# ThomasZiegler/RS-aware-differential-SfM

Measured on AMD Instinct MI355X. Metric: Mpixels/sec RS depth+pose solve, 1280x720 pair, higher is better.
Workload: dtype f64

## Files before the change

### include/rsdsfm.h

```cpp
#ifndef RSDSFM_H
#define RSDSFM_H

#include <stddef.h>
#include <stdint.h>

#ifdef __cplusplus
extern "C" {
#endif

#define RSDSFM_OK 0
#define RSDSFM_ERR_INVALID (-1)
#define RSDSFM_ERR_HIP (-2)
#define RSDSFM_ERR_NO_DEVICE (-3)
#define RSDSFM_ERR_NUMERIC (-4)
#define RSDSFM_ERR_PENDING (-5)
#define RSDSFM_ERR_PEER (-6)

#define RSDSFM_DEPTH_CLOSED_FORM 0
#define RSDSFM_DEPTH_CERES_LM 1

#define RSDSFM_K_COMPAT 0
#define RSDSFM_K_FIXED 1

#define RSDSFM_FLOW_COMPAT_RANK 0
#define RSDSFM_FLOW_GATHERED 1

#define RSDSFM_BACKPROJECT_RS 0
#define RSDSFM_BACKPROJECT_GS 1

#define RSDSFM_Q5_COMPAT 0
#define RSDSFM_Q5_FIXED 1

#define RSDSFM_TERM_GRADIENT 0
#define RSDSFM_TERM_PARAMETER 1
#define RSDSFM_TERM_FUNCTION 2
#define RSDSFM_TERM_MAX_ITER 3
#define RSDSFM_TERM_FAILURE 4
#define RSDSFM_TERM_MIN_RADIUS 5

typedef struct rsdsfm_ctx rsdsfm_ctx;

typedef struct rsdsfm_lm_summary {
    int32_t num_iterations;
    int32_t num_successful_steps;
    int32_t num_unsuccessful_steps;
    int32_t termination;
    double initial_cost;
    double final_cost;
    double final_radius;
} rsdsfm_lm_summary;

typedef struct rsdsfm_ransac_out {
    int64_t num_inliers;
    int32_t best_trial;
    int32_t _pad;
    double w[3], v[3], k;
    double inlier_error;
    int64_t* inlier_idx;
    double* inliers;
    double* alpha;
    double* alpha_k;
    uint8_t* mask;
    double* inv_depth;
    int64_t* trial_count;
    double* trial_err;
    double* trial_vel;
    int32_t* trial_steps;
} rsdsfm_ransac_out;

int rsdsfm_create(rsdsfm_ctx** ctx, int device, void* stream_or_null);
void rsdsfm_destroy(rsdsfm_ctx* ctx);
const char* rsdsfm_last_error(const rsdsfm_ctx* ctx);
const char* rsdsfm_version(void);
int rsdsfm_fused_arithmetic(void);
int rsdsfm_synchronize(rsdsfm_ctx* ctx);
int rsdsfm_set_depth_variant(rsdsfm_ctx* ctx, int variant);
int rsdsfm_set_ransac_speculation(rsdsfm_ctx* ctx, int k0);
int rsdsfm_set_ransac_math(rsdsfm_ctx* ctx, int mode);
int rsdsfm_ransac_restarts(rsdsfm_ctx* ctx, int64_t* count);
int rsdsfm_set_lm_arithmetic(rsdsfm_ctx* ctx, int mode);
int rsdsfm_lma_restarts(rsdsfm_ctx* ctx, int64_t* count, int32_t* last_guards_or_null);
int rsdsfm_refine_restarts(rsdsfm_ctx* ctx, int64_t* runs, int64_t* restarts, int64_t* resolves_or_null, int32_t* last_guard_or_null);
int rsdsfm_set_refine_arithmetic(rsdsfm_ctx* ctx, int mode);
int rsdsfm_lma_count_only(rsdsfm_ctx* ctx, int64_t* runs, int64_t* lazy_runs_or_null);
int rsdsfm_depth_restarts(rsdsfm_ctx* ctx, int64_t* count);
int rsdsfm_set_refine_stage(rsdsfm_ctx* ctx, int mode);
int rsdsfm_set_profiling(rsdsfm_ctx* ctx, int on);
int rsdsfm_profile_last_ms(rsdsfm_ctx* ctx, const char* what, double* ms);
const char* rsdsfm_kernel_name(const char* entry_point);

int rsdsfm_get_alpha(rsdsfm_ctx* ctx, const double* flow_px2n, int64_t n, double h, double gamma, double* alpha_n);
int rsdsfm_get_alpha_k(rsdsfm_ctx* ctx, const double* q_px2n, const double* flow_px2n, int64_t n, double h,
                       double gamma, double* alpha_k_n);
int rsdsfm_calculate_velocities(rsdsfm_ctx* ctx, const double* q_18xT, const double* u_18xT,
                                const double* alpha_9xT, const double* alpha_k_9xT, int32_t count,
                                int use_alpha_k, int k_sign_mode, double* w_3xT, double* v_3xT, double* k_T);
int rsdsfm_estimate_inverse_depths(rsdsfm_ctx* ctx, const double* q2n, const double* u2n, int64_t n,
                                   const double v[3], const double w[3], double k, const double* alpha_n,
                                   const double* alpha_k_n, int depth_mode, double* inv_depth_n,
                                   rsdsfm_lm_summary* summary_or_null);
int rsdsfm_ransac(rsdsfm_ctx* ctx, const double* q2n, const double* u2n, const double* alpha_n,
                  const double* alpha_k_n, int64_t n, int use_alpha_k, int32_t iterations, double tolerance,
                  const int32_t* samples_9xT_or_null, uint64_t seed, int depth_mode, int k_sign_mode,
                  rsdsfm_ransac_out* out);
int rsdsfm_refine(rsdsfm_ctx* ctx, const double* flow2n, int64_t n_flow, int64_t m, const double* inliers_3m,
                  const double* alpha_m, const double* alpha_k_m, const int64_t* inlier_idx_or_null,
                  const double v_in[3], const double w_in[3], double k_in, int const_acceleration,
                  int flow_index_mode, double* inliers_out_3m, double v_out[3], double w_out[3], double* k_out,
                  rsdsfm_lm_summary* summary_or_null);
int rsdsfm_last_ransac_tag(rsdsfm_ctx* ctx, uint64_t* tag, int64_t* cache_hits_or_null);
int rsdsfm_refine_from_ransac(rsdsfm_ctx* ctx, uint64_t ransac_tag, const double* flow2n, int64_t n_flow, int64_t m, const double* inliers_3m,
                              const double* alpha_m, const double* alpha_k_m, const int64_t* inlier_idx_or_null, const double v_in[3],
                              const double w_in[3], double k_in, int const_acceleration, int flow_index_mode, double* inliers_out_3m,
                              double v_out[3], double w_out[3], double* k_out, rsdsfm_lm_summary* summary_or_null);
#define RSDSFM_REFINE_TRACE_COLS 8
#define RSDSFM_TRACE_REJECTED 0.0
#define RSDSFM_TRACE_ACCEPTED 1.0
#define RSDSFM_TRACE_INVALID 2.0
#define RSDSFM_TRACE_PARAMETER_TOL 3.0
#define RSDSFM_TRACE_FUNCTION_TOL 4.0
#define RSDSFM_TRACE_ACCEPTED_GRADIENT_TOL 5.0
int rsdsfm_set_refine_trace(rsdsfm_ctx* ctx, int32_t rows);
int rsdsfm_get_refine_trace(rsdsfm_ctx* ctx, double* trace_rows_x_8, int32_t rows);
int rsdsfm_flatten(rsdsfm_ctx* ctx, const double* flow_img_rows_cols_2, int32_t rows, int32_t cols, double fx,
                   double fy, double cx, double cy, double gamma, double flow_threshold, double* q2n,
                   double* u2n, double* alpha_n, double* alpha_k_n, int64_t* n_out);
int rsdsfm_depth_map(rsdsfm_ctx* ctx, double* inliers_3m_inout, int64_t m, double v_inout[3], double fx,
                     double fy, double cx, double cy, int32_t rows, int32_t cols,
                     double* depth_map_colmajor, int32_t* xs_or_null, int32_t* ys_or_null, int* flipped);
int rsdsfm_pose_table(rsdsfm_ctx* ctx, const double v[3], const double w[3], double k, double gamma,
                      int32_t rows, double* R_rows9, double* t_rows3);

int rsdsfm_estimate_inverse_depths_dev(rsdsfm_ctx* ctx, const double* d_q2n, const double* d_u2n, int64_t n,
                                       const double v[3], const double w[3], double k, const double* d_alpha_n,
                                       const double* d_alpha_k_n, int depth_mode, double* d_inv_depth_n);
int rsdsfm_flatten_dev(rsdsfm_ctx* ctx, const double* d_flow_img, int32_t rows, int32_t cols, double fx, double fy,
                       double cx, double cy, double gamma, double flow_threshold, double* d_q2n, double* d_u2n,
                       double* d_alpha_n, double* d_alpha_k_n, int64_t* n_out);
int rsdsfm_depth_map_dev(rsdsfm_ctx* ctx, double* d_inliers_3m_inout, int64_t m, double v_inout[3], double fx, double fy,
                         double cx, double cy, int32_t rows, int32_t cols, double* d_depth_map_colmajor,
                         int32_t* d_xs_or_null, int32_t* d_ys_or_null, int* flipped);
int rsdsfm_pose_table_dev(rsdsfm_ctx* ctx, const double v[3], const double w[3], double k, double gamma, int32_t rows,
                          double* d_R_rows9, double* d_t_rows3);
typedef struct rsdsfm_frame_params {
    int32_t ransac_trials;
    int32_t use_acceleration_mode;
    int32_t use_refinement;
    int32_t depth_mode;
    int32_t k_sign_mode;
    int32_t flow_index_mode;
    int32_t use_global_shutter_mode;
    int32_t struct_bytes;
    double ransac_tol;
    double flow_threshold;
    uint64_t seed;
} rsdsfm_frame_params;

void rsdsfm_frame_params_init(rsdsfm_frame_params* params);

typedef struct rsdsfm_frame_result {
    int64_t n_points, num_inliers;
    int32_t best_trial, flipped;
    double ransac_w[3], ransac_v[3], ransac_k;
    double w[3], v[3], k;
// ... 182 lines not shown
```

### rs-aware-differential-sfm_amd/__init__.py

```python
import ctypes as C
import os
import sys

import numpy as np

from . import dist, pipeline, synth

_HERE = os.path.dirname(os.path.abspath(__file__))
LIB_PATH = os.environ.get("RSDSFM_LIB") or os.path.join(_HERE, "librsdsfm_hip.so")
LIB_PATH_FUSED = os.path.join(_HERE, "librsdsfm_hip_fused.so")
HEADER_PATH = os.path.join(os.path.dirname(_HERE), "include", "rsdsfm.h")

OK = 0
ERR_PENDING = -5
DEPTH_CLOSED_FORM, DEPTH_CERES_LM = 0, 1
K_COMPAT, K_FIXED = 0, 1
FLOW_COMPAT_RANK, FLOW_GATHERED = 0, 1
REFINE_TRACE_COLS = 8
TRACE_REJECTED, TRACE_ACCEPTED, TRACE_INVALID, TRACE_PARAMETER_TOL, TRACE_FUNCTION_TOL, TRACE_ACCEPTED_GRADIENT_TOL = 0.0, 1.0, 2.0, 3.0, 4.0, 5.0
TERMINATION = {0: "gradient", 1: "parameter", 2: "function", 3: "max_iter", 4: "failure", 5: "min_radius"}

_libs = {}


# ... 134 lines not shown
    return np.ascontiguousarray(a, dtype=np.float64)


def _p(a):
    return None if a is None else a.ctypes.data_as(C.c_void_p)


def _v3(a):
    return (C.c_double * 3)(*[float(x) for x in a])


def _dp(ptr):
    return C.c_void_p(int(ptr))


class Solver:

    def __init__(self, device=0, stream=None, arith="reference"):
        self.lib = load_library(arith=arith)
        self.arith = arith
        self._ctx = C.c_void_p()
        rc = self.lib.rsdsfm_create(C.byref(self._ctx), int(device), C.c_void_p(stream) if stream else None)
        if rc != OK:
            self._ctx = None
            raise RsdsfmError("rsdsfm_create(device=%d) failed with %d (no usable gfx950 device? there is no CPU fallback)" % (device, rc))

    def close(self):
        if getattr(self, "_ctx", None):
            self.lib.rsdsfm_destroy(self._ctx)
            self._ctx = None

    def __del__(self):
        try:
            self.close()
        except Exception:
            pass

    def __enter__(self):
        return self

    def __exit__(self, *a):
        self.close()

    def _check(self, rc, what):
        if rc != OK:
            msg = self.lib.rsdsfm_last_error(self._ctx)
            raise RsdsfmError("%s failed (%d): %s" % (what, rc, msg.decode() if msg else ""))

    def set_depth_variant(self, variant):
        self._check(self.lib.rsdsfm_set_depth_variant(self._ctx, int(variant)), "rsdsfm_set_depth_variant")

    def set_profiling(self, on):
        self._check(self.lib.rsdsfm_set_profiling(self._ctx, int(bool(on))), "rsdsfm_set_profiling")

    def profile_last_ms(self, what="ransac_lm_round0"):
        ms = C.c_double()
        self._check(self.lib.rsdsfm_profile_last_ms(self._ctx, what.encode(), C.byref(ms)), "rsdsfm_profile_last_ms")
        return ms.value

    def set_refine_stage(self, mode):
        self._check(self.lib.rsdsfm_set_refine_stage(self._ctx, int(mode)), "rsdsfm_set_refine_stage")

    def set_ransac_speculation(self, k0):
        self._check(self.lib.rsdsfm_set_ransac_speculation(self._ctx, int(k0)), "rsdsfm_set_ransac_speculation")

    def set_ransac_math(self, mode):
        self._check(self.lib.rsdsfm_set_ransac_math(self._ctx, int(mode)), "rsdsfm_set_ransac_math")

    def set_lm_arithmetic(self, mode):
        self._check(self.lib.rsdsfm_set_lm_arithmetic(self._ctx, int(mode)), "rsdsfm_set_lm_arithmetic")

    def set_refine_arithmetic(self, mode):
        self._check(self.lib.rsdsfm_set_refine_arithmetic(self._ctx, int(mode)), "rsdsfm_set_refine_arithmetic")

    def refine_restarts(self):
        n, r, sv, g = C.c_int64(0), C.c_int64(0), C.c_int64(0), C.c_int32(0)
        self._check(self.lib.rsdsfm_refine_restarts(self._ctx, C.byref(n), C.byref(r), C.byref(sv), C.byref(g)), "rsdsfm_refine_restarts")
        return dict(runs=n.value, restarts=r.value, resolves=sv.value, last_guard=g.value)

    def lma_restarts(self):
        n, g = C.c_int64(0), C.c_int32(0)
        self._check(self.lib.rsdsfm_lma_restarts(self._ctx, C.byref(n), C.byref(g)), "rsdsfm_lma_restarts")
        return int(n.value), int(g.value)

    def lma_count_only(self):
        a, b = C.c_int64(0), C.c_int64(0)
        self._check(self.lib.rsdsfm_lma_count_only(self._ctx, C.byref(a), C.byref(b)), "rsdsfm_lma_count_only")
        return int(a.value), int(b.value)

    def ransac_restarts(self):
        n = C.c_int64()
        self._check(self.lib.rsdsfm_ransac_restarts(self._ctx, C.byref(n)), "rsdsfm_ransac_restarts")
        return n.value

    def depth_restarts(self):
        n = C.c_int64()
        self._check(self.lib.rsdsfm_depth_restarts(self._ctx, C.byref(n)), "rsdsfm_depth_restarts")
        return int(n.value)

    def synchronize(self):
        self._check(self.lib.rsdsfm_synchronize(self._ctx), "rsdsfm_synchronize")

    def get_alpha(self, flow_px, h, gamma):
        flow_px = _f64(flow_px)
        n = flow_px.shape[0]
        out = np.empty(n)
        self._check(self.lib.rsdsfm_get_alpha(self._ctx, _p(flow_px), C.c_int64(n), C.c_double(h), C.c_double(gamma), _p(out)), "rsdsfm_get_alpha")
        return out

    def get_alpha_k(self, q_px, flow_px, h, gamma):
        q_px, flow_px = _f64(q_px), _f64(flow_px)
        n = flow_px.shape[0]
        out = np.empty(n)
        self._check(self.lib.rsdsfm_get_alpha_k(self._ctx, _p(q_px), _p(flow_px), C.c_int64(n), C.c_double(h), C.c_double(gamma), _p(out)), "rsdsfm_get_alpha_k")
        return out

    def calculate_velocities(self, q, u, alpha, alpha_k, use_alpha_k=False, k_sign_mode=K_COMPAT):
        q, u, alpha, alpha_k = _f64(q), _f64(u), _f64(alpha), _f64(alpha_k)
        single = q.ndim == 2
        T = 1 if single else q.shape[0]
        w, v, k = np.empty((T, 3)), np.empty((T, 3)), np.empty(T)
        self._check(self.lib.rsdsfm_calculate_velocities(self._ctx, _p(q), _p(u), _p(alpha), _p(alpha_k), C.c_int32(T), int(use_alpha_k), int(k_sign_mode), _p(w), _p(v), _p(k)), "rsdsfm_calculate_velocities")
        return (w[0], v[0], float(k[0])) if single else (w, v, k)

    def ransac(self, q, u, alpha, alpha_k, use_alpha_k, iterations, tolerance, samples=None, seed=0, depth_mode=DEPTH_CERES_LM, k_sign_mode=K_COMPAT, outputs=None):
        q, u, alpha, alpha_k = _f64(q), _f64(u), _f64(alpha), _f64(alpha_k)
        n, T = q.shape[0], int(iterations)
        smp = None if samples is None else np.ascontiguousarray(samples, dtype=np.int32).reshape(-1)
        reuse = outputs is not None
        if reuse and outputs.get("_shape") == (n, T):
            bufs = outputs["_bufs"]
        else:
            bufs = dict(
                inlier_idx=np.zeros(n, dtype=np.int64), inliers=np.zeros((n, 3)), alpha=np.zeros(n), alpha_k=np.zeros(n),
                mask=np.zeros(n, dtype=np.uint8), inv_depth=np.zeros(n), trial_count=np.zeros(max(T, 1), dtype=np.int64),
                trial_err=np.zeros(max(T, 1)), trial_vel=np.zeros((max(T, 1), 7)), trial_steps=np.zeros(max(T, 1), dtype=np.int32),
            )
            if reuse:
                outputs["_shape"], outputs["_bufs"] = (n, T), bufs
        out = RansacOut()
        for name, arr in bufs.items():
            if not reuse or "only" not in outputs or name in outputs["only"]:
                setattr(out, name, arr.ctypes.data)
        self._check(self.lib.rsdsfm_ransac(self._ctx, _p(q), _p(u), _p(alpha), _p(alpha_k), C.c_int64(n), int(use_alpha_k), C.c_int32(T), C.c_double(tolerance), _p(smp), C.c_uint64(seed), int(depth_mode), int(k_sign_mode), C.byref(out)), "rsdsfm_ransac")
        m = int(out.num_inliers)
        tag, hits = C.c_uint64(0), C.c_int64(0)
        self._check(self.lib.rsdsfm_last_ransac_tag(self._ctx, C.byref(tag), C.byref(hits)), "rsdsfm_last_ransac_tag")
        return dict(
            tag=int(tag.value),
            num_inliers=m, best_trial=int(out.best_trial), w=np.array(out.w[:]), v=np.array(out.v[:]), k=float(out.k),
            inlier_error=float(out.inlier_error), inlier_idx=bufs["inlier_idx"][:m] if reuse else bufs["inlier_idx"][:m].copy(),
            inliers=bufs["inliers"][:m] if reuse else bufs["inliers"][:m].copy(), alpha=bufs["alpha"][:m] if reuse else bufs["alpha"][:m].copy(),
            alpha_k=bufs["alpha_k"][:m] if reuse else bufs["alpha_k"][:m].copy(), mask=bufs["mask"], inv_depth=bufs["inv_depth"],
            trial_count=bufs["trial_count"][:T], trial_err=bufs["trial_err"][:T], trial_vel=bufs["trial_vel"][:T],
            trial_steps=bufs["trial_steps"][:T],
        )

    def estimate_inverse_depths(self, q, u, v, w, k, alpha, alpha_k, mode=DEPTH_CERES_LM):
        q, u, alpha, alpha_k = _f64(q), _f64(u), _f64(alpha), _f64(alpha_k)
        n = q.shape[0]
        rho = np.empty(n)
        sm = LmSummary()
        self._check(self.lib.rsdsfm_estimate_inverse_depths(self._ctx, _p(q), _p(u), C.c_int64(n), _v3(v), _v3(w), C.c_double(k), _p(alpha), _p(alpha_k), int(mode), _p(rho), C.byref(sm)), "rsdsfm_estimate_inverse_depths")
        return rho, sm.as_dict()

    def estimate_inverse_depth(self, q, v, w, flow, k, alpha, alpha_k, mode=DEPTH_CERES_LM):
# ... 852 lines not shown
```

### rs-aware-differential-sfm_amd/csrc/capi.hip

```cpp
#include <string.h>

#include <algorithm>
#include <new>
#include <vector>

#include <chrono>
#include <thread>

#include "rsdsfm_internal.hpp"

namespace rsdsfm {

int fail(Ctx* c, int code, const char* msg) {
    if (c) c->err = msg;
    return code;
}

int ensure_stage(Ctx* c, size_t bytes) {
    c->stage_gen += 1;
    if (bytes <= c->stage_bytes) return RSDSFM_OK;
    RSDSFM_HIP_CHECK(c, hipStreamSynchronize(c->stream));
    if (c->d_stage) RSDSFM_HIP_CHECK(c, hipFree(c->d_stage));
    c->d_stage = nullptr;
    c->stage_bytes = 0;
// ... 241 lines not shown
    if (rows < 0 || rows > 4096) return fail(c, RSDSFM_ERR_INVALID, "refine trace: 0 <= rows <= 4096");
    if (rows != c->refine_trace_rows) {
        RSDSFM_HIP_CHECK(c, hipStreamSynchronize(c->stream));
        if (c->d_refine_trace) RSDSFM_HIP_CHECK(c, hipFree(c->d_refine_trace));
        c->d_refine_trace = nullptr;
        c->refine_trace_rows = 0;
        if (rows > 0) {
            RSDSFM_HIP_CHECK(c, hipMalloc((void**)&c->d_refine_trace, (size_t)rows * kRefineTraceCols * sizeof(double)));
            c->refine_trace_rows = rows;
        }
    }
    if (c->d_refine_trace)
        RSDSFM_HIP_CHECK(c, hipMemsetAsync(c->d_refine_trace, 0xFF, (size_t)rows * kRefineTraceCols * sizeof(double), c->stream));
    return RSDSFM_OK;
}

int rsdsfm_get_refine_trace(rsdsfm_ctx* ctx, double* out, int32_t rows) {
    CTX_OR_FAIL(ctx);
    if (!out || rows < 1) return fail(c, RSDSFM_ERR_INVALID, "refine trace: null output or rows < 1");
    if (!c->d_refine_trace) return fail(c, RSDSFM_ERR_INVALID, "no refine trace: call rsdsfm_set_refine_trace(ctx, rows) before the refinement");
    if (rows > c->refine_trace_rows) return fail(c, RSDSFM_ERR_INVALID, "refine trace: more rows requested than rsdsfm_set_refine_trace reserved");
    RSDSFM_HIP_CHECK(c, hipMemcpyAsync(out, c->d_refine_trace, (size_t)rows * kRefineTraceCols * sizeof(double), hipMemcpyDeviceToHost, c->stream));
    RSDSFM_HIP_CHECK(c, hipStreamSynchronize(c->stream));
    return RSDSFM_OK;
}

int rsdsfm_set_ransac_speculation(rsdsfm_ctx* ctx, int k0) {
    CTX_OR_FAIL(ctx);
    if (k0 != 0 && k0 != 2 && k0 != KMAX) return fail(c, RSDSFM_ERR_INVALID, "ransac speculation depth must be 0 (automatic, default), 2 or 3");
    c->ransac_k0 = k0;
    return RSDSFM_OK;
}

int rsdsfm_set_ransac_math(rsdsfm_ctx* ctx, int mode) {
    CTX_OR_FAIL(ctx);
    if (mode < 0 || mode > 1) return fail(c, RSDSFM_ERR_INVALID, "ransac math: 0 = in-range function cores with restart (default), 1 = standard functions");
    c->ransac_math_mode = mode;
    return RSDSFM_OK;
}

int rsdsfm_ransac_restarts(rsdsfm_ctx* ctx, int64_t* count) {
    CTX_OR_FAIL(ctx);
    if (!count) return fail(c, RSDSFM_ERR_INVALID, "ransac restarts: null output");
    int64_t total = c->ransac_restarts;
    for (rsdsfm_ctx* lane : c->lanes) total += lane->c.ransac_restarts;
    *count = total;
    return RSDSFM_OK;
}

int rsdsfm_set_lm_arithmetic(rsdsfm_ctx* ctx, int mode) {
    CTX_OR_FAIL(ctx);
    if (mode < 0 || mode > 2)
        return fail(c, RSDSFM_ERR_INVALID, "LM arithmetic: 0 = analytic trajectory with guards (default), 1 = iterate by iterate, 2 = 0 with the frame solve's count-only pass forced");
    c->lm_arithmetic = mode == 1 ? 1 : 0;
    c->lma_count_only_force = mode == 2;
    c->lma_hold = c->lma_unique_run = 0;
    dist_reset_hold(c);
    for (rsdsfm_ctx* lane : c->lanes)
        lane->c.lm_arithmetic = c->lm_arithmetic, lane->c.lma_count_only_force = c->lma_count_only_force, lane->c.lma_hold = lane->c.lma_unique_run = 0;
    return RSDSFM_OK;
}

int rsdsfm_lma_count_only(rsdsfm_ctx* ctx, int64_t* runs, int64_t* lazy_runs) {
    CTX_OR_FAIL(ctx);
    if (!runs) return fail(c, RSDSFM_ERR_INVALID, "lma count only: null output");
    int64_t a = c->lma_count_only_runs, b = c->lma_lazy_runs;
    for (rsdsfm_ctx* lane : c->lanes) a += lane->c.lma_count_only_runs, b += lane->c.lma_lazy_runs;
    *runs = a;
    if (lazy_runs) *lazy_runs = b;
    return RSDSFM_OK;
}

int rsdsfm_lma_restarts(rsdsfm_ctx* ctx, int64_t* count, int32_t* last_guards) {
    CTX_OR_FAIL(ctx);
    if (!count) return fail(c, RSDSFM_ERR_INVALID, "lma restarts: null output");
    int64_t total = c->lma_restarts;
    int guards = c->lma_last_guard;
    for (rsdsfm_ctx* lane : c->lanes) total += lane->c.lma_restarts, guards |= lane->c.lma_last_guard;
    *count = total;
    if (last_guards) *last_guards = guards;
    return RSDSFM_OK;
}

int rsdsfm_set_refine_arithmetic(rsdsfm_ctx* ctx, int mode) {
    CTX_OR_FAIL(ctx);
    if (mode != 0 && mode != 1) return fail(c, RSDSFM_ERR_INVALID, "refine arithmetic: 0 = radius-factorised (default), 1 = iterate by iterate");
    c->refine_arithmetic = mode;
    for (rsdsfm_ctx* lane : c->lanes) lane->c.refine_arithmetic = mode;
    return RSDSFM_OK;
}

int rsdsfm_refine_restarts(rsdsfm_ctx* ctx, int64_t* runs, int64_t* restarts, int64_t* resolves_or_null, int32_t* last_guard_or_null) {
    CTX_OR_FAIL(ctx);
    if (!runs || !restarts) return fail(c, RSDSFM_ERR_INVALID, "refine restarts: null output");
    int64_t n = c->refine_rf_runs, r = c->refine_rf_restarts, s = c->refine_rf_resolves;
    int guard = c->refine_rf_last_guard;
    for (rsdsfm_ctx* lane : c->lanes) {
        n += lane->c.refine_rf_runs, r += lane->c.refine_rf_restarts, s += lane->c.refine_rf_resolves;
        if (lane->c.refine_rf_last_guard) guard = lane->c.refine_rf_last_guard;
    }
    *runs = n, *restarts = r;
    if (resolves_or_null) *resolves_or_null = s;
    if (last_guard_or_null) *last_guard_or_null = guard;
    return RSDSFM_OK;
}

int rsdsfm_depth_restarts(rsdsfm_ctx* ctx, int64_t* count) {
    CTX_OR_FAIL(ctx);
    if (!count) return fail(c, RSDSFM_ERR_INVALID, "depth restarts: null output");
    *count = c->depth_restarts;
    return RSDSFM_OK;
}

int rsdsfm_set_true_flow_search(rsdsfm_ctx* ctx, int mode) {
    CTX_OR_FAIL(ctx);
    if (mode < 0 || mode > 2) return fail(c, RSDSFM_ERR_INVALID, "true-flow search mode: 0 = automatic, 1 = exhaustive, 2 = interval-pruned");
    c->true_flow_exhaustive = mode;
    return RSDSFM_OK;
}

const char* rsdsfm_kernel_name(const char* entry_point) {
    if (!entry_point) return "";
    if (!strcmp(entry_point, "estimate_inverse_depths_lm")) return RSDSFM_FUSED ? "depth_lm_kernel<1, false>" : "depth_lm_kernel<1, true>";
    if (!strcmp(entry_point, "estimate_inverse_depths_closed_form")) return "depth_closed_form_kernel";
    return "";
}

int rsdsfm_estimate_inverse_depths_dev(rsdsfm_ctx* ctx, const double* d_q, const double* d_u, int64_t n,
                                       const double v[3], const double w[3], double k, const double* d_alpha,
                                       const double* d_alpha_k, int depth_mode, double* d_rho) {
    CTX_OR_FAIL(ctx);
    if (n < 0 || !v || !w) return fail(c, RSDSFM_ERR_INVALID, "bad arguments");
    if (n > 0 && (!d_q || !d_u || !d_alpha || !d_alpha_k || !d_rho)) return fail(c, RSDSFM_ERR_INVALID, "null device pointer");
    Pose pose;
    memcpy(pose.v, v, sizeof(pose.v));
    memcpy(pose.w, w, sizeof(pose.w));
    pose.k = k;
    if (depth_mode == RSDSFM_DEPTH_CLOSED_FORM) return depth_closed_form_launch(c, d_q, d_u, d_alpha, d_alpha_k, n, pose, d_rho);
    if (depth_mode != RSDSFM_DEPTH_CERES_LM) return fail(c, RSDSFM_ERR_INVALID, "unknown depth_mode");
    if (c->depth_variant == 2) {
        int rcf = depth_lm_fused_launch(c, d_q, d_u, d_alpha, d_alpha_k, n, pose, d_rho);
        if (rcf != RSDSFM_OK) return rcf;
        rcf = depth_lm_launch(c, d_q, d_u, d_alpha, d_alpha_k, n, pose, d_rho, 1);
        c->lm_issued_k = 2;
        c->lm_issued_d = 1;
        return rcf;
    }
    if (depth_lma_allowed(c, n)) {
        Ctx* cs1[1] = {c};
        const double *q1[1] = {d_q}, *u1[1] = {d_u}, *a1[1] = {d_alpha}, *ak1[1] = {d_alpha_k};
        double* r1[1] = {d_rho};
        int rc0 = depth_lma_batch_launch(cs1, 1, q1, u1, a1, ak1, &n, &pose, r1);
        c->lm_issued_k = 1;
        c->lm_issued_d = 1;
        return rc0;
    }
    if (c->depth_variant == 0) {
        int rc0 = depth_lm_launch(c, d_q, d_u, d_alpha, d_alpha_k, n, pose, d_rho, 0, true);
        if (rc0 != RSDSFM_OK) return rc0;
        rc0 = depth_lm_decide_apply_launch(c, d_q, d_u, d_alpha, d_alpha_k, n, pose, d_rho);
        c->lm_issued_k = 1;
        c->lm_issued_d = 1;
        return rc0;
    }
    int rc = depth_lm_launch(c, d_q, d_u, d_alpha, d_alpha_k, n, pose, d_rho, 0);
    if (rc != RSDSFM_OK) return rc;
// ... 254 lines not shown
```

### rs-aware-differential-sfm_amd/csrc/frame_host.hip

```cpp
#include <stdlib.h>
#include <string.h>

#include <atomic>

#include <algorithm>
#include <new>

#include "rsdsfm_internal.hpp"
#include "sequence_host.hpp"

namespace rsdsfm {

static std::atomic<int> g_frames_in_flight[64];
int frames_in_flight(const Ctx* c) { return g_frames_in_flight[c->device & 63].load(std::memory_order_relaxed); }

int alpha_ones_launch(Ctx* c, double* d_alpha, int64_t n);
int flatten_device(Ctx* c, const double* d_img, int32_t rows, int32_t cols, int32_t col0, double fx, double fy, double cx, double cy, double gamma,
                   double thr, double* d_q, double* d_u, double* d_alpha, double* d_alpha_k, int64_t* n_out);

struct FrameRun {
    rsdsfm_frame_job job;
    rsdsfm_frame_params prm;
    size_t N = 0;
    int64_t n = 0;
// ... 86 lines not shown
    F->d_in_a = fa.take<double>(N);
    F->d_in_ak = fa.take<double>(N);
    F->d_inl = fa.take<double>(3 * N);
    F->d_inl_ref = fa.take<double>(3 * N);
    F->d_idx = fa.take<int64_t>(N);
    F->d_mask = fa.take<uint8_t>(N);
    F->d_ys = fa.take<int32_t>(N);
    F->d_zpartials = fa.take<double>(1024);
    F->d_zheader = fa.take<double>(8);
    F->d_refine_ws = fa.take<char>(refine_workspace_bytes(c, (int64_t)N, true));
    int64_t* d_flat_counts = fa.take<int64_t>(ncells);
    int64_t* d_flat_offsets = fa.take<int64_t>(ncells + 2048);

    int rc = ensure_pinned(c, ransac_pinned_bytes(prm->ransac_trials));
    if (rc != RSDSFM_OK) return rc;
    int64_t n = (int64_t)N;
    F->side_flatten = false;
    if (c->frame_dense_hint) {
        *count_host(c) = -1;
        int side = prm->ransac_trials > 0 ? c->frame_side_flatten : 0;
        if (side == 3 && prm->ransac_trials > c->num_cus * 2) side = 0;
        F->dense_in_launch = false;
        if (side) {
            F->side_flatten = true;
            F->direct = Minimal9Direct();
            F->direct.img = J.d_flow_img, F->direct.rows = rows, F->direct.cols = cols, F->direct.alpha_ones = prm->use_global_shutter_mode ? 1 : 0;
            F->direct.fx = fx, F->direct.fy = fy, F->direct.cx = cx, F->direct.cy = cy, F->direct.gamma = gamma;
        }
        if (side == 3) {
            if (!c->d_flat_counters) {
                RSDSFM_HIP_CHECK(c, hipMalloc(reinterpret_cast<void**>(&c->d_flat_counters), 2 * sizeof(unsigned long long)));
                RSDSFM_HIP_CHECK(c, hipMemsetAsync(c->d_flat_counters, 0, 2 * sizeof(unsigned long long), c->stream));
            }
            F->dense = DenseFlatten();
            F->dense.thr = prm->flow_threshold;
            F->dense.d_q = F->d_q, F->dense.d_u = F->d_u, F->dense.d_alpha = F->d_a, F->dense.d_alpha_k = F->d_ak;
            F->dense.d_counters = c->d_flat_counters;
            F->dense.total_out = count_host(c);
            F->dense_in_launch = true;
        } else if (side == 2) {
            F->join = [c, F, d_flat_counts, d_flat_offsets]() -> int {
                const rsdsfm_frame_job& J2 = F->job;
                int rc2 = flatten_launch(c, J2.d_flow_img, J2.rows, J2.cols, 0, J2.fx, J2.fy, J2.cx, J2.cy, J2.gamma, F->prm.flow_threshold, F->d_q, F->d_u, F->d_a,
                                         F->d_ak, d_flat_counts, d_flat_offsets, count_host(c), nullptr);
                if (rc2 == RSDSFM_OK && F->prm.use_global_shutter_mode) rc2 = alpha_ones_launch(c, F->d_a, (int64_t)F->N);
                return rc2;
            };
        } else if (side == 1) {
            rc = ensure_side_stream(c);
            if (rc != RSDSFM_OK) return rc;
            RSDSFM_HIP_CHECK(c, hipEventRecord(c->ev_fork, c->stream));
            RSDSFM_HIP_CHECK(c, hipStreamWaitEvent(c->aux_stream, c->ev_fork, 0));
            {
                StreamSwap on_side(c, c->aux_stream);
                rc = flatten_launch(c, J.d_flow_img, rows, cols, 0, fx, fy, cx, cy, gamma, prm->flow_threshold, F->d_q, F->d_u, F->d_a, F->d_ak,
                                    d_flat_counts, d_flat_offsets, count_host(c), nullptr);
                if (rc == RSDSFM_OK && prm->use_global_shutter_mode) rc = alpha_ones_launch(c, F->d_a, n);
            }
            if (rc != RSDSFM_OK) return rc;
            RSDSFM_HIP_CHECK(c, hipEventRecord(c->ev_join, c->aux_stream));
            F->join = [c]() -> int {
                RSDSFM_HIP_CHECK(c, hipStreamWaitEvent(c->stream, c->ev_join, 0));
                return RSDSFM_OK;
            };
        } else {
            rc = flatten_enqueue(c, J.d_flow_img, rows, cols, fx, fy, cx, cy, gamma, prm->flow_threshold, F->d_q, F->d_u, F->d_a, F->d_ak, count_host(c));
            if (rc != RSDSFM_OK) return rc;
        }
    } else {
        rc = flatten_device(c, J.d_flow_img, rows, cols, 0, fx, fy, cx, cy, gamma, prm->flow_threshold, F->d_q, F->d_u, F->d_a, F->d_ak, &n);
        if (rc != RSDSFM_OK) return rc;
        *count_host(c) = n;
    }
    if (prm->use_global_shutter_mode && !F->side_flatten) {
        rc = alpha_ones_launch(c, F->d_a, n);
        if (rc != RSDSFM_OK) return rc;
    }
    F->n = n;
    memset(&F->ro, 0, sizeof(F->ro));
    F->ro.inlier_idx = F->d_idx;
    F->ro.inliers = F->d_inl;
    F->ro.alpha = F->d_in_a;
    F->ro.alpha_k = F->d_in_ak;
    F->ro.mask = F->d_mask;
    F->m_known = -1;
    F->tail = [c, F](const RefineBuffers& B) -> int {
        const rsdsfm_frame_job& J2 = F->job;
        const RefineState* st = B.state;
        const int64_t m_arg = F->m_known >= 0 ? F->m_known : F->n;
        const int64_t* m_dev = F->m_known >= 0 ? nullptr : &st->m;
        PoseTableOut pt;
        if (J2.d_R_rows9_or_null && J2.d_t_rows3_or_null)
            pt.R = J2.d_R_rows9_or_null, pt.t = J2.d_t_rows3_or_null, pt.rows = J2.rows, pt.gamma = J2.gamma, pt.wk_dev = st->p + 3;
        if (B.claim.on)
            return depth_map_decided_launch(c, F->d_inl_ref, m_arg, F->d_zpartials, refine_finish_grid(c, B), B, J2.d_depth_map_colmajor, F->d_zheader,
                                            header_host(c), st->p, m_dev, &pt);
        return depth_map_slab_launch(c, F->d_inl_ref, m_arg, F->d_zpartials, refine_finish_grid(c, B), m_arg, nullptr, J2.fx, J2.fy, J2.cx, J2.cy, J2.rows,
                                     0, J2.cols, J2.d_depth_map_colmajor, nullptr, F->d_ys, F->d_zheader, header_host(c), st->p, m_dev, &pt);
    };
    F->claim = FinishClaim();
    if (c->frame_tail == 0) {
        F->claim.on = true;
        F->claim.fx = J.fx, F->claim.fy = J.fy, F->claim.cx = J.cx, F->claim.cy = J.cy;
        F->claim.rows = rows, F->claim.cols = cols;
        F->claim.ys = F->d_ys;
    }
    F->spec_tail = [c, F](const RansacBest* d_best) -> int {
        return refine_begin(c, F->d_u, F->n, F->n, F->d_inl, F->d_in_a, F->d_in_ak, F->d_idx, nullptr, nullptr, 0.0, F->prm.use_acceleration_mode,
                            F->prm.flow_index_mode, F->d_inl_ref, &F->tail, d_best, F->d_refine_ws, &F->refine, state_host(c), F->d_zpartials, false,
                            &F->claim);
    };
    F->refinement_enqueued = false;
    F->ahead = prm->use_refinement && c->ransac_spec_miss < 2;
    F->open = true;
    g_frames_in_flight[c->device & 63].fetch_add(1, std::memory_order_relaxed);
    F->counted = true;
    F->rc_begin = ransac_begin(c, F->d_q, F->d_u, F->d_a, F->d_ak, n, prm->use_acceleration_mode, prm->ransac_trials, prm->ransac_tol, nullptr, J.seed,
                               prm->depth_mode, prm->k_sign_mode, &F->ro, prm->use_refinement ? &F->spec_tail : nullptr, &F->refinement_enqueued, &F->ransac,
                               F->side_flatten ? &F->direct : nullptr, F->side_flatten && !F->dense_in_launch ? &F->join : nullptr,
                               F->dense_in_launch ? &F->dense : nullptr, F->ahead, true,
                               F->claim.on && prm->use_refinement ? refine_flag_words(F->d_refine_ws) : nullptr);
    return RSDSFM_OK;
}

int frame_finish(Ctx* c, FrameRun* F, rsdsfm_frame_result* res) {
    if (!F->open) return fail(c, RSDSFM_ERR_INVALID, "no frame solve in flight");
    F->open = false;
    FrameInFlightEnd in_flight_end_{c, F};
    const rsdsfm_frame_job& J = F->job;
    const rsdsfm_frame_params* prm = &F->prm;
    memset(res, 0, sizeof(*res));
    int rc = F->rc_begin;
    if (rc == RSDSFM_OK) rc = ransac_finish(c, &F->ransac);
    if (rc != RSDSFM_OK) RSDSFM_HIP_CHECK(c, hipStreamSynchronize(c->stream));
    if (F->side_flatten && c->aux_stream) RSDSFM_HIP_CHECK(c, hipStreamSynchronize(c->aux_stream));
    int64_t n = F->n;
    if (*count_host(c) < 0) {
        c->frame_dense_hint = 1;
        return rc != RSDSFM_OK ? rc : fail(c, RSDSFM_ERR_NUMERIC, "frame solve: the point count did not arrive");
    }
    bool counted = true;
    if (*count_host(c) != n) {
        if (F->dense_in_launch) {
            int64_t n_real = 0;
            rc = flatten_device(c, J.d_flow_img, J.rows, J.cols, 0, J.fx, J.fy, J.cx, J.cy, J.gamma, prm->flow_threshold, F->d_q, F->d_u, F->d_a, F->d_ak, &n_real);
            if (rc == RSDSFM_OK && prm->use_global_shutter_mode) rc = alpha_ones_launch(c, F->d_a, n_real);
            if (rc != RSDSFM_OK) return rc;
            *count_host(c) = n_real;
        }
        n = *count_host(c);
        F->n = n;
        F->refinement_enqueued = false;
        counted = false;
        rc = ransac_begin(c, F->d_q, F->d_u, F->d_a, F->d_ak, n, prm->use_acceleration_mode, prm->ransac_trials, prm->ransac_tol, nullptr, J.seed,
                          prm->depth_mode, prm->k_sign_mode, &F->ro, prm->use_refinement ? &F->spec_tail : nullptr, &F->refinement_enqueued, &F->ransac, nullptr, nullptr,
                          nullptr, F->ahead, true,
                               F->claim.on && prm->use_refinement ? refine_flag_words(F->d_refine_ws) : nullptr);
        if (rc == RSDSFM_OK) rc = ransac_finish(c, &F->ransac);
        counted = rc == RSDSFM_OK;
    }
    c->frame_dense_hint = n == (int64_t)F->N ? 1 : 0;
    if (rc != RSDSFM_OK) return rc;
    if (counted) ransac_commit_hints(c, F->ransac);
    const rsdsfm_ransac_out& ro = F->ro;
    res->n_points = n;
    res->num_inliers = ro.num_inliers;
    res->best_trial = ro.best_trial;
// ... 67 lines not shown
    if (!p) return;
    memset(p, 0, sizeof(*p));
    p->ransac_trials = 5;
    p->use_acceleration_mode = 0;
    p->use_refinement = 1;
    p->depth_mode = RSDSFM_DEPTH_CERES_LM;
    p->k_sign_mode = RSDSFM_K_COMPAT;
    p->flow_index_mode = RSDSFM_FLOW_COMPAT_RANK;
    p->use_global_shutter_mode = 0;
    p->struct_bytes = (int32_t)sizeof(rsdsfm_frame_params);
    p->ransac_tol = 0.05;
    p->flow_threshold = 1e-10;
    p->seed = 1;
}

int rsdsfm_solve_frame_dev(rsdsfm_ctx* ctx, const double* d_flow_img, int32_t rows, int32_t cols, double fx, double fy, double cx,
                           double cy, double gamma, const rsdsfm_frame_params* prm, double* d_depth_map, double* d_R_rows9,
                           double* d_t_rows3, rsdsfm_frame_result* res) {
    if (!ctx) return RSDSFM_ERR_INVALID;
    Ctx* c = &ctx->c;
    DeviceGuard device_guard_(c);
    if (!prm || !res) return fail(c, RSDSFM_ERR_INVALID, "bad arguments");
    FrameRun* F = frame_run_of(c);
    if (!F) return fail(c, RSDSFM_ERR_INVALID, "out of host memory");
    F->prm = *prm;
    F->job = rsdsfm_frame_job{d_flow_img, rows, cols, fx, fy, cx, cy, gamma, d_depth_map, d_R_rows9, d_t_rows3, prm->seed};
    int rc = frame_begin(c, F);
    if (rc != RSDSFM_OK) return rc;
    return frame_finish(c, F, res);
}

int rsdsfm_set_sequence_lanes(rsdsfm_ctx* ctx, int32_t lanes) {
    if (!ctx) return RSDSFM_ERR_INVALID;
    Ctx* c = &ctx->c;
    DeviceGuard device_guard_(c);
    if (lanes < 0 || lanes > 16) return fail(c, RSDSFM_ERR_INVALID, "lanes must be 0 (default) .. 16");
    c->seq_lanes = lanes;
    return RSDSFM_OK;
}

int rsdsfm_set_frame_tail(rsdsfm_ctx* ctx, int mode) {
    if (!ctx) return RSDSFM_ERR_INVALID;
    if (mode < 0 || mode > 1) return fail(&ctx->c, RSDSFM_ERR_INVALID, "mode must be 0 (short launch tail) or 1 (stage-by-stage launches)");
    ctx->c.frame_tail = mode;
    return RSDSFM_OK;
}

int rsdsfm_set_frame_side_flatten(rsdsfm_ctx* ctx, int mode) {
    if (!ctx) return RSDSFM_ERR_INVALID;
    if (mode < 0 || mode > 3) return fail(&ctx->c, RSDSFM_ERR_INVALID, "mode must be 0 (flatten first), 1 (flatten on a second stream), 2 (flatten behind the minimal solver) or 3 (flatten inside the solver's launch)");
    ctx->c.frame_side_flatten = mode;
    return RSDSFM_OK;
}

}

namespace rsdsfm {

int sequence_lane_count(const Ctx* c, int count) { return std::max(1, std::min<int>(count, c->seq_lanes > 0 ? c->seq_lanes : kSequenceLanesDefault)); }

int solve_frames_run(Ctx* c, const rsdsfm_frame_job* jobs, int32_t count, const rsdsfm_frame_params* prm, rsdsfm_frame_result* results, const PairHook* hook) {
    const int L = sequence_lane_count(c, count);
    while ((int)c->lanes.size() < L - 1) {
        rsdsfm_ctx* lane = nullptr;
        int rc = rsdsfm_create(&lane, c->device, nullptr);
        if (rc != RSDSFM_OK) return fail(c, rc, "could not create a sequence lane");
        c->lanes.push_back(lane);
    }
    auto lane_ctx = [&](int l) -> Ctx* { return l == 0 ? c : &c->lanes[(size_t)l - 1]->c; };
    if (L > 1) {
        if (!c->ev_seq) RSDSFM_HIP_CHECK(c, hipEventCreateWithFlags(&c->ev_seq, hipEventDisableTiming));
        RSDSFM_HIP_CHECK(c, hipEventRecord(c->ev_seq, c->stream));
    }
    for (int l = 1; l < L; ++l) {
        Ctx* lc = lane_ctx(l);
        RSDSFM_HIP_CHECK(c, hipStreamWaitEvent(lc->stream, c->ev_seq, 0));
        lc->ransac_k0 = c->ransac_k0;
        lc->ransac_math_mode = c->ransac_math_mode;
        lc->lm_arithmetic = c->lm_arithmetic;
        lc->refine_arithmetic = c->refine_arithmetic;
        lc->lma_count_only_force = c->lma_count_only_force;
        lc->frame_side_flatten = c->frame_side_flatten;
        lc->frame_tail = c->frame_tail;
        lc->refine_stage_mode = c->refine_stage_mode;
    }
    for (int l = 0; l < L; ++l) lane_ctx(l)->refine_stage_separate = L > 1;
    int first_error = RSDSFM_OK;
    int in_flight[16];
    for (int l = 0; l < 16; ++l) in_flight[l] = -1;
    auto finish_lane = [&](int l) {
        const int i = in_flight[l];
        if (i < 0) return;
        in_flight[l] = -1;
        Ctx* lc = lane_ctx(l);
        int rc = frame_finish(lc, static_cast<FrameRun*>(lc->frame_run), &results[i]);
        if (rc != RSDSFM_OK && first_error == RSDSFM_OK) {
            first_error = rc;
            if (lc != c) c->err = "pair " + std::to_string(i) + ": " + lc->err;
        }
        if (rc == RSDSFM_OK && hook && first_error == RSDSFM_OK) {
            rc = (*hook)(lc, i, static_cast<FrameRun*>(lc->frame_run)->job, results[i]);
            if (rc != RSDSFM_OK) {
                first_error = rc;
                c->err = "pair " + std::to_string(i) + ": " + std::string(lc->err);
            }
        }
    };
    for (int i = 0; i < count && first_error == RSDSFM_OK; ++i) {
        const int l = i % L;
        finish_lane(l);
        if (first_error != RSDSFM_OK) break;
        Ctx* lc = lane_ctx(l);
        FrameRun* F = frame_run_of(lc);
        if (!F) {
            first_error = fail(c, RSDSFM_ERR_INVALID, "out of host memory");
            break;
        }
        F->prm = *prm;
        F->job = jobs[i];
        int rc = frame_begin(lc, F);
        if (rc != RSDSFM_OK) {
            first_error = rc;
            if (lc != c) c->err = "pair " + std::to_string(i) + ": " + lc->err;
            break;
        }
        in_flight[l] = i;
    }
    for (;;) {
        int best = -1;
        for (int l = 0; l < L; ++l)
            if (in_flight[l] >= 0 && (best < 0 || in_flight[l] < in_flight[best])) best = l;
        if (best < 0) break;
        finish_lane(best);
    }
    for (int l = 0; l < L; ++l) lane_ctx(l)->refine_stage_separate = false;
    return first_error;
}

}

extern "C" {

int rsdsfm_solve_frames_dev(rsdsfm_ctx* ctx, const rsdsfm_frame_job* jobs, int32_t count, const rsdsfm_frame_params* prm, rsdsfm_frame_result* results) {
    if (!ctx) return RSDSFM_ERR_INVALID;
    Ctx* c = &ctx->c;
    DeviceGuard device_guard_(c);
    if (count < 0 || !prm || (count > 0 && (!jobs || !results))) return fail(c, RSDSFM_ERR_INVALID, "bad arguments");
    if (count == 0) return RSDSFM_OK;
    return solve_frames_run(c, jobs, count, prm, results, nullptr);
}

int rsdsfm_set_refine_stage(rsdsfm_ctx* ctx, int mode) {
    if (!ctx) return RSDSFM_ERR_INVALID;
    Ctx* c = &ctx->c;
    if (mode < 0 || mode > 2) return fail(c, RSDSFM_ERR_INVALID, "refine stage: 0 (automatic), 1 (in the next pass's prologue) or 2 (a launch of its own)");
    c->refine_stage_mode = mode;
    return RSDSFM_OK;
}

}
```

### rs-aware-differential-sfm_amd/csrc/lma_stages.hpp

```cpp
#pragma once

#include "lma_common.hpp"

namespace rsdsfm {

constexpr int kLB = 256;

struct PixIn {
    double x, y, ux, uy, al, ak;
};
__device__ __forceinline__ PixIn load_pix(const double2* __restrict__ q, const double2* __restrict__ u, const double* __restrict__ alpha,
                                          const double* __restrict__ alpha_k, unsigned i) {
    const unsigned o16 = i << 4, o8 = i << 3;
    const double2 qq = *reinterpret_cast<const double2*>(reinterpret_cast<const char*>(q) + o16);
    const double2 uu = *reinterpret_cast<const double2*>(reinterpret_cast<const char*>(u) + o16);
    PixIn p;
    p.x = qq.x, p.y = qq.y, p.ux = uu.x, p.uy = uu.y;
    p.al = *reinterpret_cast<const double*>(reinterpret_cast<const char*>(alpha) + o8);
    p.ak = *reinterpret_cast<const double*>(reinterpret_cast<const char*>(alpha_k) + o8);
    return p;
}

__device__ __forceinline__ void lma_rows_stage(const double* __restrict__ partials, int nblocks, int T, int t, const double2* __restrict__ q,
                                               const double2* __restrict__ u, const double* __restrict__ alpha, const double* __restrict__ alpha_k,
                                               const Pose& pose, const LmaCand& cd, const int* __restrict__ irr_count,
                                               const int* __restrict__ irr_list, double* s_row) {
    __shared__ double s_red3[768];
    __shared__ int s_list[kLmaListCap], s_sorted[kLmaListCap];
    constexpr int LBATCH = 64;
    __shared__ double s_x[LBATCH][2 + 5 * kLmaKP + 2 * kLmaNC + 2 + 1];
    const int tid = threadIdx.x;
    const int raw = irr_count[t];
    {
        static_assert(768 % kLmaSlots == 0 && 768 % kLB == 0, "the stride keeps every thread on its slots");
        const double* __restrict__ base = partials + (int64_t)t * nblocks * kLmaSlots;
        const int total = nblocks * kLmaSlots;
        double acc[3] = {0.0, 0.0, 0.0};
        bool mx[3];
#pragma unroll
        for (int m = 0; m < 3; ++m) mx[m] = ((tid + kLB * m) % kLmaSlots) == kLmaG;
        constexpr int UB = 20;
        for (int f0 = 0; f0 < total; f0 += UB * 768) {
            double vv[UB][3];
#pragma unroll
            for (int j = 0; j < UB; ++j)
#pragma unroll
                for (int m = 0; m < 3; ++m) {
                    const int f = f0 + j * 768 + m * kLB + tid;
                    vv[j][m] = f < total ? base[f] : 0.0;
                }
#pragma unroll
            for (int j = 0; j < UB; ++j)
#pragma unroll
                for (int m = 0; m < 3; ++m) acc[m] = mx[m] ? fmax(acc[m], vv[j][m]) : acc[m] + vv[j][m];
        }
#pragma unroll
        for (int m = 0; m < 3; ++m) s_red3[m * kLB + tid] = acc[m];
        __syncthreads();
        if (tid < kLmaSlots) {
            double r = s_red3[tid];
            for (int e = tid + kLmaSlots; e < 768; e += kLmaSlots) r = tid == kLmaG ? fmax(r, s_red3[e]) : r + s_red3[e];
            if (tid < 6) s_row[tid] = r;
            else s_row[kLmaRowScore + (tid - 6)] = r;
        }
        if (tid >= 6 && tid < kLmaRowScore) s_row[tid] = 0.0;
    }
    const int nl = min(raw, kLmaListCap);
    for (int i = tid; i < nl; i += kLB) s_list[i] = irr_list[(int64_t)t * kLmaListCap + i];
    __syncthreads();
    for (int i = tid; i < nl; i += kLB) {
        const int mine = s_list[i];
        int rank = 0;
        for (int j = 0; j < nl; ++j) rank += s_list[j] < mine ? 1 : 0;
        s_sorted[rank] = mine;
    }
    __syncthreads();
    if (tid == 0 && raw > kLmaListCap) s_row[7] = 1.0;
    if (nl == 0) return;
    const double two_over = 2.0 / (2.0 + pose.k);
    const LmaPlan& plan = cd.plan;
    constexpr int XW = 2 + 5 * kLmaKP + 2 * kLmaNC + 2;
    for (int base = 0; base < nl; base += LBATCH) {
        const int e = base + tid;
        double* xr = s_x[tid < LBATCH ? tid : 0];
        if (tid >= LBATCH) {
        } else if (e < nl) {
            const int64_t i = s_sorted[e];
            const double2 qq = q[i], uu = u[i];
            PixIn px;
            px.x = qq.x, px.y = qq.y, px.ux = uu.x, px.uy = uu.y, px.al = alpha[i], px.ak = alpha_k[i];
            const LmaPx v = lma_pixel(px.x, px.y, px.ux, px.uy, px.al, px.ak, pose, two_over);
            LmxWalk wk;
            lmx_walk(px.x, px.y, px.ux, px.uy, px.al, px.ak, pose, two_over, plan, kLmaKP, wk);
            xr[0] = v.clamped ? wk.c0 : 0.0;
            xr[1] = v.clamped ? wk.g0 : 0.0;
#pragma unroll
            for (int k = 0; k < kLmaKP; ++k) {
                xr[2 + 5 * k + 0] = v.clamped ? wk.m[k] : 0.0;
                xr[2 + 5 * k + 1] = v.clamped ? wk.s2[k] : 0.0;
                xr[2 + 5 * k + 2] = v.clamped ? wk.c[k] : 0.0;
                xr[2 + 5 * k + 3] = v.clamped ? wk.x2[k] : 0.0;
                xr[2 + 5 * k + 4] = v.clamped ? wk.g[k] : 0.0;
            }
#pragma unroll
            for (int c = 0; c < kLmaNC; ++c) {
                double dc = 0.0, de = 0.0;
                if (c < cd.nc) {
                    bool in_a;
                    double err_a;
                    lma_score(v, cd.phi2[c], cd.tol2, in_a, err_a);
                    const double ex = point_error(px.x, px.y, px.ux, px.uy, px.al, px.ak, pose, two_over, wk.rho[cd.steps[c]]);
                    const bool in_x = ex < cd.tol;
                    dc = (in_x ? 1.0 : 0.0) - (in_a ? 1.0 : 0.0);
                    de = cd.count_only ? 0.0 : (in_x ? ex : 0.0) - err_a;
                }
                xr[2 + 5 * kLmaKP + 2 * c] = dc;
                xr[2 + 5 * kLmaKP + 2 * c + 1] = de;
            }
            xr[XW - 2] = v.clamped ? v.a : 0.0;
            xr[XW - 1] = v.clamped ? 1.0 : 0.0;
        } else {
            for (int j = 0; j < XW; ++j) xr[j] = 0.0;
        }
        __syncthreads();
        if (tid < XW) {
            const int cntb = min(LBATCH, nl - base);
            const bool is_max = tid == 1 || (tid >= 2 && tid < 2 + 5 * kLmaKP && ((tid - 2) % 5) == 4);
            double r = 0.0;
            for (int j = 0; j < cntb; ++j) r = is_max ? fmax(r, s_x[j][tid]) : r + s_x[j][tid];
            if (tid < 2) s_row[kLmaRowX0 + tid] = is_max ? fmax(s_row[kLmaRowX0 + tid], r) : s_row[kLmaRowX0 + tid] + r;
            else if (tid < 2 + 5 * kLmaKP) s_row[kLmaRowXk + (tid - 2)] = is_max ? fmax(s_row[kLmaRowXk + (tid - 2)], r) : s_row[kLmaRowXk + (tid - 2)] + r;
            else if (tid < XW - 2) s_row[kLmaRowScore + (tid - 2 - 5 * kLmaKP)] += r;
            else if (tid == XW - 2) s_row[0] -= r;
            else {
                s_row[3] -= r;
                s_row[6] += r;
            }
        }
        __syncthreads();
    }
}

__device__ __forceinline__ bool lma_band(double x, double thr) { return fabs(x - thr) <= kLmaBand * fabs(thr); }

__device__ __forceinline__ int lma_decide(const double* row, int64_t n, const LmaCand& cd, const LmaPlan& plan, bool nan_pose, LmScal& st, double* hist, bool& scored,
                                          double& count, double& err, double* phi_out = nullptr) {
    const double A = row[0], B = row[1], C = row[2], D = row[3], E = row[4], G = row[5];
    const bool listed_walk = row[6] != 0.0;
    int fallback = 0;
    if (row[7] != 0.0) fallback = 8;
    if (__builtin_isinf(A) || __builtin_isinf(B) || __builtin_isinf(C) || __builtin_isinf(D) || __builtin_isinf(E) || __builtin_isinf(G)) fallback = 1;
    st.status = 1;
    st.restart = 0;
    st.n_hist = 0;
    st.K = 0;
    st.write_which = 0;
    st.iteration = 0;
    st.num_successful = 0;
    st.num_unsuccessful = 0;
    st.invalid_run = 0;
    st.termination = -1;
    st.rho_holds = -1;
    st.launches = 1;
    st.next_launch = 1;
    st.predict = 0;
    st.radius = kInitialRadius;
    st.decrease_factor = 2.0;
    double phi = 1.0;
    double XC = row[kLmaRowX0], Xg = row[kLmaRowX0 + 1];
    double cost = 0.5 * ((A + B) + XC), x_norm = sqrt((double)n);
    double gmax = fmax(G, Xg);
    st.initial_cost = cost;
    bool on_plan = true;
    if (lma_band(gmax, kGradientTol)) fallback = 2;
    if (n == 0 || gmax <= kGradientTol) st.termination = RSDSFM_TERM_GRADIENT;
    while (st.termination < 0 && !fallback) {
        if (st.iteration >= kMaxIter) {
            st.termination = RSDSFM_TERM_MAX_ITER;
            break;
        }
        if (st.radius <= kMinRadius) {
            st.termination = RSDSFM_TERM_MIN_RADIUS;
            break;
        }
        st.iteration += 1;
        const int kk = st.n_hist;
        on_plan = on_plan && kk < kLmaKP && st.radius == plan.radius[kk];
        if (listed_walk && !on_plan && B == B) {
            fallback = 9;
            break;
        }
        double psi, phic;
        if (on_plan) psi = plan.psi[kk], phic = plan.phi[kk + 1];
        else lma_phi_step(st.radius, phi, psi, phic);
        const double p2 = phi * phi, pc2 = phic * phic;
        const double* xk = row + kLmaRowXk + 5 * (kk < kLmaKP ? kk : 0);
        const double XM = listed_walk ? xk[0] : 0.0, XS = listed_walk ? xk[1] : 0.0, XCc = listed_walk ? xk[2] : 0.0;
        const double XX = listed_walk ? xk[3] : 0.0, Xgc = listed_walk ? xk[4] : 0.0;
        const double model_change = __builtin_fma(B * p2, psi * (1.0 - 0.5 * psi), XM);
        const double stepsq = __builtin_fma(C * p2, psi * psi, XS);
        if (!(model_change > 0.0)) {
            if (model_change == model_change) {
                fallback = 3;
                break;
            }
            st.num_unsuccessful += 1;
            st.invalid_run += 1;
            if (st.invalid_run >= kMaxInvalid) {
                st.termination = RSDSFM_TERM_FAILURE;
                break;
            }
            st.radius *= 0.5;
            continue;
        }
        if (model_change < 1e-25 * cost) {
            fallback = 3;
            break;
        }
        st.invalid_run = 0;
        const double step_norm = sqrt(stepsq);
        const double ptol = kParameterTol * (x_norm + kParameterTol);
        if (lma_band(step_norm, ptol)) {
            fallback = 4;
            break;
        }
        if (step_norm <= ptol) {
            st.termination = RSDSFM_TERM_PARAMETER;
            break;
        }
        const double cost_change = 0.5 * __builtin_fma(B, p2 - pc2, XC - XCc);
        if (lma_band(fabs(cost_change), kFunctionTol * cost)) {
            fallback = 5;
            break;
        }
        if (fabs(cost_change) <= kFunctionTol * cost) {
            st.termination = RSDSFM_TERM_FUNCTION;
            break;
        }
        const double rel = cost_change / model_change;
        if (!(rel > 0.95)) {
            fallback = 6;
            break;
        }
        hist[st.n_hist] = st.radius;
        st.n_hist += 1;
        phi = phic;
        XC = XCc;
        Xg = Xgc;
        cost = 0.5 * (__builtin_fma(B, pc2, A) + XC);
        x_norm = sqrt(__builtin_fma(C, pc2, __builtin_fma(2.0 * E, phi, D)) + XX);
        gmax = fmax(G * phi, Xg);
        st.radius = radius_accept(st.radius, rel);
        st.decrease_factor = 2.0;
        st.num_successful += 1;
        if (lma_band(gmax, kGradientTol)) {
            fallback = 2;
            break;
        }
        if (gmax <= kGradientTol) st.termination = RSDSFM_TERM_GRADIENT;
    }
    st.cost = cost;
    st.rho_holds = -1;
    if (phi_out) *phi_out = phi;
    scored = false;
    count = err = 0.0;
    if (fallback) return fallback;
    if (nan_pose) {
        scored = true;
        return 0;
    }
    const double phi2 = phi * phi;
    for (int c = 0; c < cd.nc; ++c)
        if (cd.steps[c] == st.n_hist && cd.phi2[c] == phi2) {
            count = row[kLmaRowScore + 2 * c];
            err = row[kLmaRowScore + 2 * c + 1];
            scored = true;
        }
    return 0;
}

}
```

### rs-aware-differential-sfm_amd/csrc/ransac_host.hip

```cpp
#include <stdio.h>
#include <stdlib.h>
#include <string.h>

#include <algorithm>
#include <vector>

#include "rsdsfm_internal.hpp"

namespace rsdsfm {

namespace {


inline uint64_t splitmix64(uint64_t& state) {
    uint64_t z = (state += 0x9E3779B97F4A7C15ULL);
    z = (z ^ (z >> 30)) * 0xBF58476D1CE4E5B9ULL;
    z = (z ^ (z >> 27)) * 0x94D049BB133111EBULL;
    return z ^ (z >> 31);
}

void sample_indices(int64_t n, int T, uint64_t seed, std::vector<int32_t>& out) {
    struct Slot {
        int64_t key;
        int32_t val;
        uint32_t gen;
    };
    thread_local std::vector<Slot> table;
    thread_local uint32_t gen = 0;
    size_t cap = 64;
    while (cap < (size_t)T * 18 * 4) cap <<= 1;
    if (table.size() != cap || gen == 0xFFFFFFFFu) {
        table.assign(cap, Slot{-1, 0, 0});
        gen = 0;
    }
    gen += 1;
    Slot* tb = table.data();
    const uint32_t g = gen;
    auto slot = [&](int64_t i) -> size_t {
        size_t h = (size_t)(((uint64_t)i * 0x9E3779B97F4A7C15ull) >> 20) & (cap - 1);
        while (tb[h].gen == g && tb[h].key != i) h = (h + 1) & (cap - 1);
        return h;
    };
    auto get = [&](int64_t i) -> int32_t {
        const size_t h = slot(i);
        return tb[h].gen == g ? tb[h].val : (int32_t)i;
    };
    auto put = [&](int64_t i, int32_t v) {
        const size_t h = slot(i);
        tb[h].key = i;
        tb[h].val = v;
        tb[h].gen = g;
    };
    out.resize((size_t)T * 9);
    uint64_t st = seed;
    for (int t = 0; t < T; ++t) {
        int64_t n_temp = n;
        for (int j = 0; j < 9; ++j) {
            const int64_t r = (int64_t)(splitmix64(st) % (uint64_t)n_temp);
            const int32_t a = get(n_temp - 1), b = get(r);
            put(n_temp - 1, b);
            put(r, a);
            out[(size_t)t * 9 + j] = b;
            n_temp--;
        }
    }
}

}

void sample_indices(int64_t n, int T, uint64_t seed, int32_t* out) {
    std::vector<int32_t> v;
    sample_indices(n, T, seed, v);
    if (!v.empty()) memcpy(out, v.data(), sizeof(int32_t) * v.size());
}

size_t ransac_pinned_bytes(int T) {
    const size_t Tn = (size_t)std::max(T, 1);
    return sizeof(RansacBest) + 8 * sizeof(int) + sizeof(double) * 2 * Tn + sizeof(double) * 8 * Tn + sizeof(LmState) * Tn + 64 +
           sizeof(int32_t) * Tn * 9 + kPinnedTail;
}

namespace {

enum RansacPc { kPcStart = 0, kPcBatchBegin, kPcRoundEnqueue, kPcRoundWait, kPcAfterRounds, kPcScore, kPcFinal, kPcFinalWait, kPcDone };

int lma_start_over(Ctx* c, RansacRun& R, int guards) {
    R.analytic = false;
    R.lma_restarted = true;
    R.lma_guard |= guards;
    R.tie_margin = -kLmaTie;
    R.not_one_step = 0;
    R.final_done = R.spec_scored = R.tail_enqueued = R.spec_final = false;
    RSDSFM_HIP_CHECK(c, hipMemsetAsync(R.zero_begin, 0, R.zero_bytes, c->stream));
    R.b0 = 0;
    R.pc = kPcBatchBegin;
    return RSDSFM_OK;
}

int ransac_advance(Ctx* c, RansacRun& R, bool yield_at_wait) {
    rsdsfm_ransac_out* out = R.out;
    const int T = R.T, Tn = R.Tn, batch = R.batch, depth_mode = R.depth_mode;
    const int64_t n = R.n;
    const double tol = R.tol;
    int rc = RSDSFM_OK;
    for (;;) {
        switch (R.pc) {
            case kPcStart: {
                const bool zero_in_minimal9 = T > 0 && R.zero_bytes % 8 == 0 && (reinterpret_cast<uintptr_t>(R.zero_begin) & 7) == 0;
                if (!zero_in_minimal9) RSDSFM_HIP_CHECK(c, hipMemsetAsync(R.zero_begin, 0, R.zero_bytes, c->stream));
                if (T > 0) {
                    memcpy(R.h_samples_pinned, R.samples.data(), sizeof(int32_t) * (size_t)T * 9);
                    Minimal9Direct dir = R.direct ? *R.direct : Minimal9Direct();
                    R.core_epoch = 0;
                    if (R.core_math && depth_mode == RSDSFM_DEPTH_CERES_LM && T <= c->num_cus * 2 && c->d_core_flag) {
                        c->core_epoch = c->core_epoch >= 0x3fffffff ? 1 : c->core_epoch + 1;
                        dir.core_flag = c->d_core_flag;
                        dir.core_epoch = R.core_epoch = c->core_epoch;
                    }
                    if (R.direct && R.dense && T <= c->num_cus * 2)
                        rc = minimal9_flatten_launch(c, R.h_samples_pinned, T, R.use_alpha_k, R.k_sign_mode, R.d_hyp, zero_in_minimal9 ? R.zero_begin : nullptr,
                                                     zero_in_minimal9 ? R.zero_bytes : 0, dir, R.dense->thr, R.dense->d_q, R.dense->d_u, R.dense->d_alpha,
                                                     R.dense->d_alpha_k, R.dense->d_counters, R.dense->total_out);
                    else
                        rc = minimal9_launch(c, R.d_q, R.d_u, R.d_a, R.d_ak, R.h_samples_pinned, T, R.use_alpha_k, R.k_sign_mode, R.d_hyp,
                                             zero_in_minimal9 ? R.zero_begin : nullptr, zero_in_minimal9 ? R.zero_bytes : 0, &dir);
                    if (rc != RSDSFM_OK) return rc;
                    if (R.after_minimal9) {
                        rc = (*R.after_minimal9)();
                        if (rc != RSDSFM_OK) return rc;
                    }
                }
                R.b0 = 0;
                R.pc = kPcBatchBegin;
                break;
            }
            case kPcBatchBegin: {
                if (R.b0 >= T) {
                    R.pc = kPcFinal;
                    break;
                }
                R.B = std::min(batch, T - R.b0);
                R.need_score = true;
                if (depth_mode == RSDSFM_DEPTH_CERES_LM) {
                    if (R.b0 > 0)
                        RSDSFM_HIP_CHECK(c, hipMemsetAsync(R.d_flags, 0, (size_t)(reinterpret_cast<char*>(R.d_irr_count + R.batch) - reinterpret_cast<char*>(R.d_flags)), c->stream));
                    R.round = 0;
                    R.pc = kPcRoundEnqueue;
                } else {
                    R.pc = kPcScore;
                }
                break;
            }
            case kPcRoundEnqueue: {
                const int b0 = R.b0, B = R.B, round = R.round;
                bool flags_via_pick = false;
                if (round > 4 * kMaxIter) return fail(c, RSDSFM_ERR_NUMERIC, "LM state machines did not terminate");
                if (R.analytic && round == 0) {
                    rc = ransac_lma_launch(c, R.d_q, R.d_u, R.d_a, R.d_ak, n, R.d_hyp + (size_t)b0 * 8, B, R.d_states + b0, R.d_partials, R.d_flags,
                                           R.d_scored + b0, R.d_tcount + b0, R.d_terr + b0, tol, R.lma_cand, 2, R.d_irr_count, R.d_irr_list, R.d_unscored,
                                           nullptr, R.core_epoch ? c->d_core_flag : nullptr, R.core_epoch, R.count_only);
                } else {
                    rc = ransac_lm_round_launch(c, R.d_q, R.d_u, R.d_a, R.d_ak, n, R.d_hyp + (size_t)b0 * 8, B, R.d_states + b0, R.d_partials, R.d_flags,
                                                R.d_scored + b0, R.d_tcount + b0, R.d_terr + b0, round, tol, R.k0, R.fused_base, R.core_math,
                                                R.core_epoch ? c->d_core_flag : nullptr, R.core_epoch, R.d_unscored);
                }
                if (rc != RSDSFM_OK) return rc;
                if (round == 0 && B == T) {
                    const PickLazy lazy = R.count_only ? PickLazy{R.d_scored, R.d_unscored, R.d_flags + 1} : PickLazy();
                    if (c->ransac_score_idle < kScoreIdleLimit) {
                        if (R.count_only) {
                            rc = ransac_pick_launch(c, R.d_tcount, R.d_terr, T, R.d_hyp, R.d_best, nullptr, R.d_flags, nullptr, 0, nullptr, 0, 0, nullptr, 0.0, lazy);
                            if (rc != RSDSFM_OK) return rc;
                        }
                        rc = ransac_score_launch(c, R.d_q, R.d_u, R.d_a, R.d_ak, n, R.d_hyp, T, R.d_states, depth_mode, tol, R.d_scored, R.d_partials,
                                                 R.d_tcount, R.d_terr, R.d_unscored, R.d_flags + 1);
                        if (rc != RSDSFM_OK) return rc;
                        R.spec_scored = true;
                    }
                    rc = ransac_pick_launch(c, R.d_tcount, R.d_terr, T, R.d_hyp, R.d_best, R.h_best, R.d_flags, R.h_running, R.spec_scored ? 1 : 0,
                                            nullptr, 0, 0, nullptr, R.tie_margin, lazy);
                    if (rc != RSDSFM_OK) return rc;
                    flags_via_pick = true;
                    rc = ransac_final_launch(c, R.d_q, R.d_u, R.d_a, R.d_ak, n, R.d_best, R.d_states, depth_mode, tol, R.d_rho, R.d_mask, R.d_bcounts,
                                             R.d_boffs, out->inlier_idx, out->inliers, out->alpha, out->alpha_k, R.h_best, R.refine_flag_words);
                    if (rc != RSDSFM_OK) return rc;
                    R.final_done = true;
                    R.spec_final = true;
                    if (R.spec_tail && R.tail_ahead) {
                        rc = (*R.spec_tail)(R.d_best);
                        if (rc != RSDSFM_OK) return rc;
                        R.tail_enqueued = true;
                    }
                }
                if (!flags_via_pick) RSDSFM_HIP_CHECK(c, hipMemcpyAsync(R.h_running, R.d_flags, sizeof(int) * 8, hipMemcpyDeviceToHost, c->stream));
                R.pc = kPcRoundWait;
                if (yield_at_wait) return RSDSFM_OK;
                break;
            }
            case kPcRoundWait: {
                yield_at_wait = false;
                if (int rcs = sync_stream(c, "ransac_finish line 244")) return rcs;
                const int* h_running = R.h_running;
                if (R.round == 0 && R.analytic && (h_running[3] & 16) != 0) R.lma_guard |= h_running[3] >> 8;
                if (R.round == 0 && R.analytic && (h_running[3] & 6) != 0 && !((h_running[3] & 1) && R.core_math)) {
                    rc = lma_start_over(c, R, (h_running[3] >> 8) | ((h_running[3] & 4) ? (1 << 7) : 0));
                    if (rc != RSDSFM_OK) return rc;
                    break;
                }
                if (R.round == 0 && R.core_math && (h_running[3] & 1) != 0) {
                    R.core_math = false;
                    R.restarted = true;
                    R.not_one_step = 0;
                    R.final_done = R.spec_scored = R.tail_enqueued = R.spec_final = false;
                    R.dense = nullptr;
                    R.after_minimal9 = nullptr;
                    R.pc = kPcStart;
                    break;
                }
                if (R.round == 0) {
                    R.not_one_step += h_running[2];
                    if (R.b0 == 0) {
                        int best = 0;
                        for (int a2 = 1; a2 <= 3; ++a2)
                            if (h_running[4 + a2] > (best ? h_running[4 + best] : 0)) best = a2;
                        if (best) R.fused_base_next = best;
                        int second = 0;
                        for (int a2 = 1; a2 <= 3; ++a2)
                            if (a2 != best && h_running[4 + a2] > (second ? h_running[4 + second] : 0)) second = a2;
                        if (best) {
                            R.lma_cand_next[0] = best;
                            R.lma_cand_next[1] = second ? second : (best > 1 ? best - 1 : 2);
                        }
                    }
                }
                if (h_running[0] == 0) {
                    R.pc = kPcAfterRounds;
                } else {
                    R.final_done = false;
                    R.round += 1;
                    R.pc = kPcRoundEnqueue;
                }
                break;
            }
            case kPcAfterRounds: {
                R.need_score = R.h_running[1] > 0;
                if (R.B == T) R.score_hint_next = R.need_score ? 1 : 0;
                if (R.need_score && R.final_done && R.spec_scored && !R.h_best->lazy_pending) R.need_score = false;
                if (R.need_score) R.final_done = false;
                R.pc = kPcScore;
                break;
            }
            case kPcScore: {
                if (R.need_score) {
                    rc = ransac_score_launch(c, R.d_q, R.d_u, R.d_a, R.d_ak, n, R.d_hyp + (size_t)R.b0 * 8, R.B, R.d_states + R.b0, depth_mode, tol,
                                             depth_mode == RSDSFM_DEPTH_CERES_LM ? R.d_scored + R.b0 : nullptr, R.d_partials, R.d_tcount + R.b0,
                                             R.d_terr + R.b0, depth_mode == RSDSFM_DEPTH_CERES_LM ? R.d_unscored : nullptr, R.d_flags + 1);
                    if (rc != RSDSFM_OK) return rc;
                }
                R.b0 += batch;
                R.pc = kPcBatchBegin;
                break;
            }
            case kPcFinal: {
                if (!R.final_done) {
                    R.tail_enqueued = false;
                    R.spec_final = false;
                    rc = ransac_pick_launch(c, R.d_tcount, R.d_terr, T, R.d_hyp, R.d_best, R.h_best, nullptr, nullptr, 0, nullptr, 0, 0, nullptr, R.tie_margin,
                                            R.count_only ? PickLazy{R.d_scored, R.d_unscored, R.d_flags + 1} : PickLazy());
                    if (rc != RSDSFM_OK) return rc;
                    rc = ransac_final_launch(c, R.d_q, R.d_u, R.d_a, R.d_ak, n, R.d_best, R.d_states, depth_mode, tol, R.d_rho, R.d_mask, R.d_bcounts,
                                             R.d_boffs, out->inlier_idx, out->inliers, out->alpha, out->alpha_k, R.h_best, R.refine_flag_words);
                    if (rc != RSDSFM_OK) return rc;
                }
                if (R.spec_tail && !R.tail_enqueued) {
                    rc = (*R.spec_tail)(R.d_best);
                    if (rc != RSDSFM_OK) return rc;
                    R.tail_enqueued = true;
                }
                if (T > 0 && out->trial_count) RSDSFM_HIP_CHECK(c, hipMemcpyAsync(R.h_tcount, R.d_tcount, sizeof(double) * T, hipMemcpyDeviceToHost, c->stream));
                if (T > 0 && out->trial_err) RSDSFM_HIP_CHECK(c, hipMemcpyAsync(R.h_terr, R.d_terr, sizeof(double) * T, hipMemcpyDeviceToHost, c->stream));
                if (T > 0 && out->trial_vel) RSDSFM_HIP_CHECK(c, hipMemcpyAsync(R.h_hyp, R.d_hyp, sizeof(double) * 8 * T, hipMemcpyDeviceToHost, c->stream));
                if (T > 0 && out->trial_steps && depth_mode == RSDSFM_DEPTH_CERES_LM)
                    RSDSFM_HIP_CHECK(c, hipMemcpyAsync(R.h_states, R.d_states, sizeof(LmState) * T, hipMemcpyDeviceToHost, c->stream));
                R.pc = kPcFinalWait;
                if (yield_at_wait) return RSDSFM_OK;
                break;
            }
            case kPcFinalWait: {
                if (int rcs = sync_stream(c, "ransac_finish line 345")) return rcs;
                const RansacBest* h_best = R.h_best;
#ifdef RSDSFM_DEBUG_HOOKS
                if (getenv("RSDSFM_RANSAC_DEBUG")) fprintf(stderr, "[ransac] final wait: lazy_pending %d undecided %d flags %d %d %d %d hist %d %d %d %d spec_scored %d spec_final %d tail %d idle %d\n", h_best->lazy_pending, h_best->undecided, R.h_running[0], R.h_running[1], R.h_running[2], R.h_running[3], R.h_running[4], R.h_running[5], R.h_running[6], R.h_running[7], (int)R.spec_scored, (int)R.spec_final, (int)R.tail_enqueued, c->ransac_score_idle);
#endif
                if (R.count_only && h_best->lazy_pending) {
                    if (++R.lazy_rounds > T + 2) return fail(c, RSDSFM_ERR_NUMERIC, "lazy error sums did not settle");
                    R.final_done = R.tail_enqueued = R.spec_final = false;
                    R.need_score = true;
                    R.score_hint_next = 1;
                    R.b0 = 0;
                    R.B = T;
                    R.pc = kPcScore;
                    break;
                }
                if (R.analytic && h_best->lma_tie) {
                    rc = lma_start_over(c, R, 1 << 7);
                    if (rc != RSDSFM_OK) return rc;
                    break;
                }
                R.lma_tie_seen = h_best->lma_tie != 0;
                R.shared_best = h_best->shared_best;
                if (h_best->num_inliers != h_best->num_inliers_scan) {
                    if (R.analytic) {
                        rc = lma_start_over(c, R, 1 << 10);
                        if (rc != RSDSFM_OK) return rc;
                        break;
                    }
                    return fail(c, RSDSFM_ERR_NUMERIC, "inlier count mismatch between scoring and compaction");
                }
                out->num_inliers = h_best->num_inliers;
                out->best_trial = h_best->best_trial;
                memcpy(out->w, &h_best->hyp[0], 3 * sizeof(double));
                memcpy(out->v, &h_best->hyp[3], 3 * sizeof(double));
                out->k = h_best->hyp[6];
                out->inlier_error = h_best->inlier_error;
                for (int t = 0; t < T; ++t) {
                    if (out->trial_count) out->trial_count[t] = (int64_t)R.h_tcount[t];
                    if (out->trial_err) out->trial_err[t] = R.h_terr[t];
                    if (out->trial_vel) memcpy(out->trial_vel + (size_t)7 * t, R.h_hyp + (size_t)8 * t, 7 * sizeof(double));
                    if (out->trial_steps) out->trial_steps[t] = depth_mode == RSDSFM_DEPTH_CERES_LM ? R.h_states[t].num_successful : 1;
                }
                if (R.spec_tail_held) *R.spec_tail_held = R.tail_enqueued;
                R.hints_ready = true;
                R.pc = kPcDone;
                (void)Tn;
                return RSDSFM_OK;
            }
            default:
                return RSDSFM_OK;
        }
    }
}

}

void ransac_commit_hints(Ctx* c, const RansacRun& R) {
    if (!R.hints_ready || R.depth_mode != RSDSFM_DEPTH_CERES_LM || R.T <= 0) return;
    if (R.fused_base_next) c->ransac_fused_base = R.fused_base_next;
    if (R.score_hint_next >= 0) c->ransac_score_idle = R.score_hint_next ? 0 : std::min(c->ransac_score_idle + 1, kScoreIdleLimit);
    c->ransac_not_one_step = R.not_one_step;
    c->ransac_spec_miss = R.spec_final ? 0 : std::min(c->ransac_spec_miss + 1, 2);
    if (R.count_only) c->lma_count_only_runs += 1, c->lma_lazy_runs += (R.lazy_rounds > 0 || R.shared_best > 1) ? 1 : 0;
    if (R.lazy_rounds > 0 || R.shared_best > 1) c->lma_unique_run = 0;
    else if (R.shared_best == 1) c->lma_unique_run = std::min(c->lma_unique_run + 1, 2);
    if (R.lma_guard) c->lma_last_guard = R.lma_guard, c->lma_handed_over += 1;
    if (R.lma_restarted) {
        c->lma_hold = 16;
        c->lma_restarts += 1;
        c->lma_last_guard = R.lma_guard;
    } else if (c->lma_hold > 0 && !R.analytic) {
        c->lma_hold = R.lma_tie_seen ? 16 : c->lma_hold - 1;
    }
    if (R.restarted) {
        c->ransac_standard_math = 16;
        c->ransac_restarts += 1;
    } else if (c->ransac_standard_math > 0) {
        c->ransac_standard_math -= 1;
    }
}

int ransac_begin(Ctx* c, const double* d_q, const double* d_u, const double* d_a, const double* d_ak, int64_t n, int use_alpha_k, int T,
                 double tol, const int32_t* h_samples, uint64_t seed, int depth_mode, int k_sign_mode, rsdsfm_ransac_out* out,
                 const RansacSpecTail* spec_tail, bool* spec_tail_held, RansacRun* run, const Minimal9Direct* direct,
                 const std::function<int()>* after_minimal9, const DenseFlatten* dense, bool tail_ahead, bool count_only, int* refine_flag_words) {
    RansacRun& R = *run;
    R = RansacRun();
    R.tail_ahead = tail_ahead;
    R.core_math = c->ransac_math_mode == 0 && c->ransac_standard_math == 0;
    R.analytic = depth_mode == RSDSFM_DEPTH_CERES_LM && T > 0 && c->lm_arithmetic == 0 && c->lma_hold == 0;
    R.tie_margin = depth_mode != RSDSFM_DEPTH_CERES_LM || c->lm_arithmetic != 0 ? 0.0 : (R.analytic ? kLmaTie : -kLmaTie);
    R.lma_cand[0] = c->lma_cand[0], R.lma_cand[1] = c->lma_cand[1];
    R.count_only = count_only && R.analytic && T <= kRansacBatch && (c->lma_unique_run >= 2 || c->lma_count_only_force);
    if (R.count_only) R.tie_margin = 0.0;
    R.refine_flag_words = refine_flag_words;
    if (spec_tail_held) *spec_tail_held = false;
    if (!out) return fail(c, RSDSFM_ERR_INVALID, "null out");
    if (n < 9) return fail(c, RSDSFM_ERR_INVALID, "ransac needs at least 9 points (the reference would compute rand() % 0)");
    if (T < 0) return fail(c, RSDSFM_ERR_INVALID, "negative iterations");
    if (depth_mode != RSDSFM_DEPTH_CLOSED_FORM && depth_mode != RSDSFM_DEPTH_CERES_LM) return fail(c, RSDSFM_ERR_INVALID, "unknown depth_mode");
    if (n > (int64_t)INT32_MAX) return fail(c, RSDSFM_ERR_INVALID, "n exceeds the int32 sample index range");
    if (T > 0) {
        if (h_samples) {
            R.samples.assign(h_samples, h_samples + (size_t)T * 9);
            for (int32_t s : R.samples)
                if (s < 0 || s >= n) return fail(c, RSDSFM_ERR_INVALID, "sample index out of range");
        } else {
            sample_indices(n, T, seed, R.samples);
        }
    }
    const int Tn = std::max(T, 1);
    const int batch = std::min(Tn, kRansacBatch);
    const size_t partials_doubles = std::max<size_t>((size_t)ransac_lm_partials_doubles(c, n, batch), (size_t)ransac_lma_partials_doubles(c, n, batch));
    size_t need = Arena::need(sizeof(double) * Tn * 8) + Arena::need(sizeof(int) * batch) + Arena::need(sizeof(int) * ransac_lma_list_ints(batch)) +
                  Arena::need(sizeof(LmState) * Tn) + Arena::need(sizeof(double) * partials_doubles) +
                  Arena::need(sizeof(int) * 8) + 2 * Arena::need(sizeof(int) * Tn) + 2 * Arena::need(sizeof(double) * Tn) + Arena::need(sizeof(RansacBest)) +
                  2 * Arena::need(sizeof(int64_t) * 2048) + Arena::need(sizeof(double) * (size_t)n) + Arena::need((size_t)n) + 4096;
    int rc = ensure_ws(c, need);
    if (rc != RSDSFM_OK) return rc;
    Arena ws(c->d_ws);
    R.d_hyp = ws.take<double>((size_t)Tn * 8);
    R.zero_begin = ws.base + ws.off;
    R.d_states = ws.take<LmState>(Tn);
    R.d_scored = ws.take<int>(Tn);
    R.d_flags = ws.take<int>(8);
    R.d_irr_count = ws.take<int>(batch);
    R.zero_bytes = (size_t)((ws.base + ws.off) - R.zero_begin);
    R.d_irr_list = ws.take<int>(ransac_lma_list_ints(batch));
    R.d_unscored = ws.take<int>(batch);
    R.d_partials = ws.take<double>(partials_doubles);
    R.d_tcount = ws.take<double>(Tn);
    R.d_terr = ws.take<double>(Tn);
    R.d_best = ws.take<RansacBest>(1);
    R.d_bcounts = ws.take<int64_t>(2048);
    R.d_boffs = ws.take<int64_t>(2048);
    R.d_rho = out->inv_depth ? out->inv_depth : ws.take<double>((size_t)n);
    R.d_mask = out->mask ? out->mask : ws.take<uint8_t>((size_t)n);

    rc = ensure_pinned(c, ransac_pinned_bytes(T));
    if (rc != RSDSFM_OK) return rc;
    if (!c->d_core_flag) {
        RSDSFM_HIP_CHECK(c, hipMalloc(reinterpret_cast<void**>(&c->d_core_flag), 64));
        RSDSFM_HIP_CHECK(c, hipMemsetAsync(c->d_core_flag, 0, 64, c->stream));
    }
    char* hp = static_cast<char*>(c->h_pinned);
    R.h_best = reinterpret_cast<RansacBest*>(hp);
    R.h_running = reinterpret_cast<int*>(hp + sizeof(RansacBest));
    R.h_tcount = reinterpret_cast<double*>(hp + sizeof(RansacBest) + 32);
    R.h_terr = R.h_tcount + Tn;
    R.h_hyp = R.h_terr + Tn;
    R.h_states = reinterpret_cast<LmState*>(R.h_hyp + (size_t)8 * Tn);
    R.h_samples_pinned = reinterpret_cast<int32_t*>(R.h_states + Tn);

    R.d_q = d_q, R.d_u = d_u, R.d_a = d_a, R.d_ak = d_ak;
    R.n = n, R.T = T, R.Tn = Tn, R.batch = batch, R.tol = tol, R.depth_mode = depth_mode, R.use_alpha_k = use_alpha_k, R.k_sign_mode = k_sign_mode;
    R.out = out, R.spec_tail = spec_tail, R.spec_tail_held = spec_tail_held;
    R.direct = direct, R.after_minimal9 = after_minimal9, R.dense = dense;
    R.k0 = c->ransac_k0 != 0 ? c->ransac_k0 : (c->ransac_not_one_step == 0 ? 2 : (int)KMAX);
    R.fused_base = R.k0 == 2 ? 1 : std::min(std::max(c->ransac_fused_base, 1), (int)KMAX);
    R.pc = kPcStart;
    return ransac_advance(c, R, true);
}

int ransac_finish(Ctx* c, RansacRun* run) { return ransac_advance(c, *run, false); }

int ransac_device(Ctx* c, const double* d_q, const double* d_u, const double* d_a, const double* d_ak, int64_t n,
                  int use_alpha_k, int T, double tol, const int32_t* h_samples, uint64_t seed, int depth_mode,
                  int k_sign_mode, rsdsfm_ransac_out* out, const RansacSpecTail* spec_tail, bool* spec_tail_held) {
    RansacRun run;
    int rc = ransac_begin(c, d_q, d_u, d_a, d_ak, n, use_alpha_k, T, tol, h_samples, seed, depth_mode, k_sign_mode, out, spec_tail, spec_tail_held,
                          &run, nullptr, nullptr);
    if (rc == RSDSFM_OK) rc = ransac_finish(c, &run);
    if (rc == RSDSFM_OK) ransac_commit_hints(c, run);
    return rc;
}

}

using namespace rsdsfm;

extern "C" {

int rsdsfm_calculate_velocities(rsdsfm_ctx* ctx, const double* q, const double* u, const double* alpha, const double* alpha_k,
                                int32_t count, int use_alpha_k, int k_sign_mode, double* w, double* v, double* k) {
    if (!ctx) return RSDSFM_ERR_INVALID;
    Ctx* c = &ctx->c;
    DeviceGuard device_guard_(c);
    if (count < 0 || (count > 0 && (!q || !u || !alpha || !alpha_k || !w || !v || !k))) return fail(c, RSDSFM_ERR_INVALID, "bad arguments");
    if (count == 0) return RSDSFM_OK;
    const size_t T = (size_t)count;
    int rc = ensure_stage(c, 2 * Arena::need(144 * T) + 2 * Arena::need(72 * T) + Arena::need(64 * T));
    if (rc != RSDSFM_OK) return rc;
    Arena sa(c->d_stage);
    double* d_q = sa.take<double>(18 * T);
    double* d_u = sa.take<double>(18 * T);
    double* d_a = sa.take<double>(9 * T);
    double* d_ak = sa.take<double>(9 * T);
    double* d_h = sa.take<double>(8 * T);
    RSDSFM_HIP_CHECK(c, hipMemcpyAsync(d_q, q, 144 * T, hipMemcpyHostToDevice, c->stream));
    RSDSFM_HIP_CHECK(c, hipMemcpyAsync(d_u, u, 144 * T, hipMemcpyHostToDevice, c->stream));
    RSDSFM_HIP_CHECK(c, hipMemcpyAsync(d_a, alpha, 72 * T, hipMemcpyHostToDevice, c->stream));
    RSDSFM_HIP_CHECK(c, hipMemcpyAsync(d_ak, alpha_k, 72 * T, hipMemcpyHostToDevice, c->stream));
    rc = minimal9_launch(c, d_q, d_u, d_a, d_ak, nullptr, count, use_alpha_k, k_sign_mode, d_h);
    if (rc != RSDSFM_OK) return rc;
    std::vector<double> h(8 * T);
    RSDSFM_HIP_CHECK(c, hipMemcpyAsync(h.data(), d_h, 64 * T, hipMemcpyDeviceToHost, c->stream));
    RSDSFM_HIP_CHECK(c, hipStreamSynchronize(c->stream));
    int worst = 0;
    for (size_t t = 0; t < T; ++t) {
        memcpy(w + 3 * t, &h[8 * t], 3 * sizeof(double));
        memcpy(v + 3 * t, &h[8 * t + 3], 3 * sizeof(double));
        k[t] = h[8 * t + 6];
        if (h[8 * t + 7] != 0.0) worst = (int)h[8 * t + 7];
    }
    if (worst != 0) return fail(c, RSDSFM_ERR_NUMERIC, worst == -1 ? "no real eigenvalue k for at least one hypothesis" : "singular system in the k estimation");
    return RSDSFM_OK;
}

int rsdsfm_ransac_dev(rsdsfm_ctx* ctx, const double* d_q, const double* d_u, const double* d_alpha, const double* d_alpha_k,
                      int64_t n, int use_alpha_k, int32_t iterations, double tolerance, const int32_t* samples, uint64_t seed,
// ... 76 lines not shown
```

### rs-aware-differential-sfm_amd/csrc/ransac_kernels.hip

```cpp
#include <algorithm>

#include "device_math.hpp"
#include "lm_common.hpp"
#include "rsdsfm_internal.hpp"

namespace rsdsfm {

namespace {

constexpr int kRB = 256;
constexpr int kRP = RSDSFM_FUSED ? 5 : 6;
constexpr int kFused = 1;
constexpr int kTiledFusedBase = 2;
constexpr int NSR = NS + 2 * kFused;
constexpr int kNSum = NSR - (KMAX + 1);
constexpr int kTStride = 65;

template <int K0>
struct R0Shape {
    static constexpr int NSk = 3 + 5 * K0;
    static constexpr int F = kFused;
    static constexpr int nsum = NSk - (K0 + 1) + 2 * F;
};
static_assert(R0Shape<KMAX>::nsum == kNSum, "full shape uses every sum slot");

template <int BIDX, bool CORE = false>
struct ScoreHook {
    double x, y, ux, uy, al, ak, two_over, tol;
    const Pose* pose;
    double* sc;
    uint32_t* worst = nullptr;
    __device__ __forceinline__ void operator()(int j, double rho, const PixelModel& m) const {
        if (j == BIDX) {
#if RSDSFM_FUSED
            (void)m;
            const double e = point_error(x, y, ux, uy, al, ak, *pose, two_over, rho);
#else
            const double e = CORE ? point_error_from_model_core(m, rho, *worst) : point_error_from_model(m, rho);
#endif
            if (e < tol) {
                sc[0] += 1.0;
                sc[1] += e;
            }
        }
    }
};

struct Tile {
    double x[kRP], y[kRP], ux[kRP], uy[kRP], al[kRP], ak[kRP];
    bool ok[kRP];
};

__device__ __forceinline__ void load_tile(Tile& t, const double2* __restrict__ q, const double2* __restrict__ u,
                                          const double* __restrict__ alpha, const double* __restrict__ alpha_k,
                                          int64_t base, int64_t n) {
#pragma unroll
    for (int j = 0; j < kRP; ++j) {
        const int64_t i = base + threadIdx.x + (int64_t)j * kRB;
        t.ok[j] = i < n;
        const int64_t ii = t.ok[j] ? i : n - 1;
        const double2 qq = q[ii], uu = u[ii];
        t.x[j] = qq.x;
        t.y[j] = qq.y;
        t.ux[j] = uu.x;
        t.uy[j] = uu.y;
        t.al[j] = alpha[ii];
        t.ak[j] = alpha_k[ii];
    }
}

__device__ __forceinline__ bool is_nan_bits(double x) {
    const uint32_t h = (uint32_t)__double2hiint(x) & 0x7FFFFFFFu;
    return h > 0x7FF00000u || (h == 0x7FF00000u && __double2loint(x) != 0);
}
__device__ __forceinline__ bool pose_has_nan(const Pose& p) {
    return ((int)is_nan_bits(p.w[0]) | (int)is_nan_bits(p.w[1]) | (int)is_nan_bits(p.w[2]) | (int)is_nan_bits(p.v[0]) | (int)is_nan_bits(p.v[1]) |
            (int)is_nan_bits(p.v[2]) | (int)is_nan_bits(p.k)) != 0;
}

#define RSDSFM_LOAD_POSE(pose, hyp, t)                       \
    Pose pose;                                               \
    {                                                        \
        const double* h_ = (hyp) + (int64_t)(t) * 8;          \
        pose.w[0] = h_[0], pose.w[1] = h_[1], pose.w[2] = h_[2]; \
        pose.v[0] = h_[3], pose.v[1] = h_[4], pose.v[2] = h_[5]; \
        pose.k = h_[6];                                      \
// ... 517 lines not shown
        rows[(int64_t)t * 2 + 1] = ((s_red[0][1] + s_red[1][1]) + s_red[2][1]) + s_red[3][1];
    }
}

__device__ __forceinline__ void pick_best_trial(const double* __restrict__ trial_count, const double* __restrict__ trial_err, int T,
                                                int lane, int& bi, double& best_count, double& best_err) {
    best_count = -1.0, best_err = 0.0;
    bi = -1;
    for (int t0 = 0; t0 < T; t0 += 64) {
        const int t = t0 + lane;
        const double cl = t < T ? trial_count[t] : 0.0, el = t < T ? trial_err[t] : 0.0;
        const int nt = T - t0 < 64 ? T - t0 : 64;
        for (int j = 0; j < nt; ++j) {
            const double c = lane_value(cl, j), e = lane_value(el, j);
            if (c > best_count || (c == best_count && e < best_err)) {
                best_count = c;
                best_err = e;
                bi = t0 + j;
            }
        }
    }
}

__global__ __launch_bounds__(64) void ransac_pick_kernel(const double* __restrict__ trial_count, const double* __restrict__ trial_err, int T,
                                                        const double* __restrict__ hyp, RansacBest* best, RansacBest* best_host,
                                                        const int* __restrict__ flags, int* __restrict__ flags_host, int scored_ahead,
                                                        const double* __restrict__ cnt_rt = nullptr, int cnt_stride = 0, int nranks = 0,
                                                        int64_t* __restrict__ m_all = nullptr, double tie_margin = 0.0, PickLazy lazy = PickLazy()) {
    if (blockIdx.x != 0) return;
    const int lane = threadIdx.x;
    int undecided = (flags && (flags[0] != 0 || (flags[1] > 0 && !scored_ahead) || flags[3] != 0)) ? 1 : 0;
    double best_count, best_err;
    int bi;
    pick_best_trial(trial_count, trial_err, T, lane, bi, best_count, best_err);
    int tie = 0;
    if (tie_margin != 0.0 && bi >= 0 && best_count > 0.0 && !(flags && (flags[0] != 0 || (flags[1] > 0 && !scored_ahead)))) {
        const double tm = fabs(tie_margin);
        for (int t0 = 0; t0 < T; t0 += 64) {
            const int t = t0 + lane;
            const bool hit = t < T && t != bi && trial_count[t] == best_count && fabs(trial_err[t] - best_err) <= tm * best_count;
            if (__builtin_amdgcn_ballot_w64(hit) != 0) tie = 1;
        }
    }
    if (tie_margin > 0.0) undecided |= tie;
    int pending = 0, list_n = 0, ns = 0;
    if (bi >= 0 && best_count > 0.0 && !(flags && (flags[0] != 0 || (flags[1] > 0 && !scored_ahead) || flags[3] != 0))) {
        int nco = 0;
        for (int t0 = 0; t0 < T; t0 += 64) {
            const int t = t0 + lane;
            const bool hit = t < T && trial_count[t] == best_count;
            ns += __builtin_popcountll(__builtin_amdgcn_ballot_w64(hit));
            nco += __builtin_popcountll(__builtin_amdgcn_ballot_w64(hit && lazy.scored && lazy.scored[t] == 2));
        }
        if (ns > 1 && nco > 0) {
            int base = 0;
            for (int t0 = 0; t0 < T; t0 += 64) {
                const int t = t0 + lane;
                const bool co = t < T && trial_count[t] == best_count && lazy.scored[t] == 2;
                const unsigned long long mk = __builtin_amdgcn_ballot_w64(co);
                if (co) {
                    lazy.list[base + __builtin_popcountll(mk & ((1ull << lane) - 1ull))] = t;
                    lazy.scored[t] = 0;
                }
                base += __builtin_popcountll(mk);
            }
            if (lane == 0) *lazy.list_count = nco;
            pending = 1;
            list_n = nco;
            undecided = 1;
        }
    }
    if (flags_host && lane < 8) flags_host[lane] = (lane == 1 && pending) ? list_n : (flags[lane] | ((lane == 3 && tie && tie_margin > 0.0) ? 4 : 0));
    if (m_all)
        for (int r = lane; r < nranks; r += 64) m_all[r] = bi >= 0 ? (int64_t)cnt_rt[(int64_t)r * cnt_stride + bi] : 0;
    const double h = (lane < 8 && bi >= 0) ? hyp[(int64_t)bi * 8 + lane] : 0.0;
    if (lane < 8) best->hyp[lane] = h;
    if (lane < 8 && best_host) best_host->hyp[lane] = h;
    if (lane == 0) {
        best->best_trial = bi;
        best->undecided = undecided;
        best->lma_tie = tie;
        best->lazy_pending = pending;
        best->shared_best = ns;
        best->num_inliers = bi >= 0 ? (int64_t)best_count : 0;
        best->inlier_error = best_err;
        if (best_host) {
            best_host->best_trial = bi;
            best_host->undecided = undecided;
            best_host->lma_tie = tie;
            best_host->lazy_pending = pending;
            best_host->shared_best = ns;
            best_host->num_inliers = bi >= 0 ? (int64_t)best_count : 0;
            best_host->inlier_error = best_err;
        }
    }
}

__global__ __launch_bounds__(kRB) void ransac_final_kernel(const double2* __restrict__ q, const double2* __restrict__ u,
                                                          const double* __restrict__ alpha,
                                                          const double* __restrict__ alpha_k, int64_t n, int64_t chunk,
                                                          const RansacBest* __restrict__ best,
                                                          const LmState* __restrict__ states, int depth_mode, double tol,
                                                          double* __restrict__ rho_out, uint8_t* __restrict__ mask_out,
                                                          int64_t* __restrict__ block_counts) {
    __shared__ LmPlanLds plan;
    __shared__ int s_cnt[kRB / 64];
    const int tid = threadIdx.x, lane = tid & 63, wv = tid >> 6;
    if (best->undecided) return;
    const int bt = best->best_trial;
    Pose pose;
    pose.w[0] = best->hyp[0], pose.w[1] = best->hyp[1], pose.w[2] = best->hyp[2];
    pose.v[0] = best->hyp[3], pose.v[1] = best->hyp[4], pose.v[2] = best->hyp[5];
    pose.k = best->hyp[6];
    if (depth_mode == RSDSFM_DEPTH_CERES_LM && bt >= 0) {
        if (tid == 0) {
            plan.n_hist = states[bt].n_hist;
            plan.K = 0;
            plan.write_which = 0;
        }
        if (tid < kMaxIter) plan.inv_hist[tid] = 1.0 / states[bt].hist[tid];
    }
    __syncthreads();
    const double two_over = 2.0 / (2.0 + pose.k);
    const int64_t i0 = (int64_t)blockIdx.x * chunk;
    const int64_t i1 = (i0 + chunk < n) ? i0 + chunk : n;
    int count = 0;
    for (int64_t i = i0 + tid; i < i1; i += kRB) {
        double2 qq = q[i], uu = u[i];
        const double al = alpha[i], ak = alpha_k[i];
        bool in = false;
        double rho = 0.0;
        if (bt >= 0) {
            rho = hyp_rho(qq.x, qq.y, uu.x, uu.y, al, ak, pose, two_over, depth_mode, plan);
            in = point_error(qq.x, qq.y, uu.x, uu.y, al, ak, pose, two_over, rho) < tol;
        }
        rho_out[i] = rho;
        mask_out[i] = in ? 1 : 0;
        count += in ? 1 : 0;
    }
    for (int off = 32; off >= 1; off >>= 1) count += __shfl_xor(count, off, 64);
    if (lane == 0) s_cnt[wv] = count;
    __syncthreads();
    if (tid == 0) {
        int c = 0;
        for (int w2 = 0; w2 < kRB / 64; ++w2) c += s_cnt[w2];
        block_counts[blockIdx.x] = c;
    }
}

__global__ __launch_bounds__(256) void ransac_scan_kernel(const int64_t* __restrict__ block_counts, int nblocks,
                                                         int64_t* __restrict__ block_offsets, RansacBest* best, RansacBest* best_host) {
    __shared__ int64_t s_part[256];
    const int tid = threadIdx.x;
    const int per = (nblocks + 255) / 256;
    int64_t sum = 0;
    for (int j = 0; j < per; ++j) {
        const int b = tid * per + j;
        if (b < nblocks) sum += block_counts[b];
    }
    s_part[tid] = sum;
    __syncthreads();
    if (tid == 0) {
        int64_t run = 0;
        for (int i = 0; i < 256; ++i) {
            int64_t v = s_part[i];
            s_part[i] = run;
            run += v;
        }
        best->num_inliers_scan = run;
        if (best_host) best_host->num_inliers_scan = run;
    }
    __syncthreads();
    int64_t run = s_part[tid];
    for (int j = 0; j < per; ++j) {
        const int b = tid * per + j;
        if (b < nblocks) {
            block_offsets[b] = run;
            run += block_counts[b];
        }
    }
}

__global__ __launch_bounds__(kRB) void ransac_scatter_kernel(const double2* __restrict__ q, const double* __restrict__ alpha,
                                                            const double* __restrict__ alpha_k, int64_t n, int64_t chunk,
                                                            const double* __restrict__ rho, const uint8_t* __restrict__ mask,
                                                            const int64_t* __restrict__ block_counts, RansacBest* best,
                                                            RansacBest* best_host, int64_t* __restrict__ inlier_idx, double* __restrict__ inliers,
                                                            double* __restrict__ out_alpha, double* __restrict__ out_alpha_k,
                                                            int* __restrict__ zero_words = nullptr) {
    __shared__ int s_wave[kRB / 64];
    __shared__ int64_t s_base;
    if (zero_words && blockIdx.x == 0 && threadIdx.x < (int)(kRefineStateBlockTail / sizeof(int))) zero_words[threadIdx.x] = 0;
    __shared__ int64_t s_pre[kRB / 64], s_all[kRB / 64];
    const int tid = threadIdx.x, lane = tid & 63, wv = tid >> 6;
    const int undecided = best->undecided;
    const int64_t i0 = (int64_t)blockIdx.x * chunk;
    const int64_t i1 = (i0 + chunk < n) ? i0 + chunk : n;
    {
        int64_t pre = 0, all = 0;
        for (int b = tid; b < (int)gridDim.x; b += kRB) {
            const int64_t cnt = block_counts[b];
            all += cnt;
            if (b < (int)blockIdx.x) pre += cnt;
        }
#pragma unroll
        for (int off = 32; off > 0; off >>= 1) {
            pre += __shfl_down(pre, off);
            all += __shfl_down(all, off);
        }
        if (lane == 0) s_pre[wv] = pre, s_all[wv] = all;
        __syncthreads();
        if (tid == 0) {
            int64_t p2 = 0, a2 = 0;
            for (int w2 = 0; w2 < kRB / 64; ++w2) p2 += s_pre[w2], a2 += s_all[w2];
            s_base = p2;
            if (blockIdx.x == 0 && !undecided) {
                best->num_inliers_scan = a2;
                if (best_host) best_host->num_inliers_scan = a2;
            }
        }
    }
    if (undecided) return;
    __syncthreads();
    for (int64_t start = i0; start < i1; start += kRB) {
        const int64_t i = start + tid;
        const bool in = (i < i1) && mask[i] != 0;
        const unsigned long long bal = __ballot(in);
        const int prefix = __popcll(bal & ((1ull << lane) - 1ull));
        if (lane == 0) s_wave[wv] = __popcll(bal);
        __syncthreads();
        int woff = 0, total = 0;
#pragma unroll
        for (int w2 = 0; w2 < kRB / 64; ++w2) {
            const int c = s_wave[w2];
            if (w2 < wv) woff += c;
            total += c;
        }
        if (in) {
            const int64_t o = s_base + woff + prefix;
            double2 qq = q[i];
            if (inlier_idx) inlier_idx[o] = i;
            if (inliers) {
                inliers[3 * o + 0] = qq.x;
                inliers[3 * o + 1] = qq.y;
                inliers[3 * o + 2] = 1.0 / rho[i];
            }
            if (out_alpha) out_alpha[o] = alpha[i];
            if (out_alpha_k) out_alpha_k[o] = alpha_k[i];
        }
        __syncthreads();
        if (tid == 0) s_base += total;
        __syncthreads();
    }
}

int ransac_pixel_grid(const Ctx* c, int64_t n) {
    const int64_t tiles = (n + (int64_t)kRB * kRP - 1) / ((int64_t)kRB * kRP);
    int64_t g = tiles < 1 ? 1 : tiles;
    const int64_t cap = (int64_t)c->num_cus * 4;
    if (g > cap) {
        const int64_t iters = (g + cap - 1) / cap;
        g = (g + iters - 1) / iters;
    }
    return (int)g;
}

static int ransac_lm_groups(const Ctx* c, int grid, int T) {
    const int slots = c->num_cus * 2;
    int g = (8 * slots + grid - 1) / grid;
    g = std::min(g, T / 8);
    return std::max(g, 1);
}

int ransac_lm_partials_doubles(const Ctx* c, int64_t n, int batch) { return ransac_pixel_grid(c, n) * batch * NSR; }

static int lm_launch(Ctx* c, const dim3& g2, int k0, const double* q, const double* u, const double* a, const double* ak, int64_t n,
                     const double* hyp, int T, const LmState* states, double* partials, int round, double tol, int* flags, int fused_base,
                     bool core_math, const int* m9_flag, int m9_epoch, unsigned long long* clk = nullptr) {
    const double2* q2 = reinterpret_cast<const double2*>(q);
    const double2* u2 = reinterpret_cast<const double2*>(u);
    const size_t lds = sizeof(double) * T * NSR;
    const int tiles = (int)g2.x, groups = (int)g2.y;
    const dim3 g1((unsigned)(((tiles + 7) / 8) * 8 * groups));
    const int clk_bid = !clk ? -1 : groups > 1 ? (((tiles + 7) / 8) / 2) * 8 * (groups - 1) : tiles / 2;
#define RSDSFM_LM_LAUNCH(R0, K0, BASE, CORE) \
    hipLaunchKernelGGL((ransac_lm_kernel<R0, K0, BASE, CORE>), g1, dim3(kRB), lds, c->stream, q2, u2, a, ak, n, hyp, T, states, partials, round, tol, flags, tiles, groups, m9_flag, m9_epoch, clk, clk_bid)
    const bool core = core_math && flags != nullptr && !RSDSFM_FUSED;
    (void)core;
#if RSDSFM_FUSED
#define RSDSFM_LM_LAUNCH2(R0, K0, BASE) RSDSFM_LM_LAUNCH(R0, K0, BASE, false)
#else
#define RSDSFM_LM_LAUNCH2(R0, K0, BASE)                 \
    do {                                                \
        if (core) RSDSFM_LM_LAUNCH(R0, K0, BASE, true); \
        else RSDSFM_LM_LAUNCH(R0, K0, BASE, false);     \
    } while (0)
#endif
    if (round != 0)
        RSDSFM_LM_LAUNCH(false, KMAX, 0, false);
    else if (k0 == 2)
        RSDSFM_LM_LAUNCH2(true, 2, 1);
    else if (fused_base == 1)
        RSDSFM_LM_LAUNCH2(true, KMAX, 1);
    else if (fused_base == 3)
        RSDSFM_LM_LAUNCH2(true, KMAX, 3);
    else
        RSDSFM_LM_LAUNCH2(true, KMAX, 2);
#undef RSDSFM_LM_LAUNCH2
#undef RSDSFM_LM_LAUNCH
    RSDSFM_HIP_CHECK(c, hipGetLastError());
    return RSDSFM_OK;
}

int ransac_lm_round_launch(Ctx* c, const double* q, const double* u, const double* a, const double* ak, int64_t n,
                           const double* hyp, int T, LmState* states, double* partials, int* flags, int* scored,
                           double* trial_count, double* trial_err, int round, double tol, int k0, int fused_base, bool core_math,
                           const int* m9_core_flag, int m9_core_epoch, int* unscored_list) {
    const int grid = ransac_pixel_grid(c, n);
    const dim3 g2(grid, ransac_lm_groups(c, grid, T));
    if (k0 != 2) k0 = KMAX;
    if (fused_base < 1 || fused_base > k0) fused_base = std::min(2, k0);
    const bool prof = c->profile && round == 0 && c->ev_prof[0] && c->ev_prof[1];
    if (prof) RSDSFM_HIP_CHECK(c, hipEventRecord(c->ev_prof[0], c->stream));
    int rc = lm_launch(c, g2, k0, q, u, a, ak, n, hyp, T, states, partials, round, tol, flags, fused_base, core_math, round == 0 ? m9_core_flag : nullptr, m9_core_epoch,
                       prof ? c->d_clk_probe : nullptr);
    if (rc != RSDSFM_OK) return rc;
    if (prof) {
        RSDSFM_HIP_CHECK(c, hipEventRecord(c->ev_prof[1], c->stream));
        c->prof_pending = true;
        c->prof_what = 0;
    }
    hipLaunchKernelGGL(ransac_decide_kernel, dim3(T), dim3(256), 0, c->stream, partials, grid, T, 1, states, n, round, k0, flags, flags + 2, scored,
                       trial_count, trial_err, fused_base, flags + 4, unscored_list);
    RSDSFM_HIP_CHECK(c, hipGetLastError());
    return RSDSFM_OK;
// ... 23 lines not shown
    int rc = lm_launch(c, g2, KMAX, q, u, a, ak, n, hyp, T, states, partials, round, tol, core ? core_flags : nullptr, kTiledFusedBase, core,
                       core ? m9_flag : nullptr, m9_epoch);
    if (rc != RSDSFM_OK) return rc;
    hipLaunchKernelGGL(ransac_lm_rows_kernel, dim3(T), dim3(256), 0, c->stream, partials, grid, T, states, round, rows,
                       static_cast<const int*>(core ? core_flags : nullptr));
    RSDSFM_HIP_CHECK(c, hipGetLastError());
    return RSDSFM_OK;
}

int ransac_rows_payload_doubles(int T, bool core_trailer) { return T * NSR + (core_trailer ? 2 : 0); }

int ransac_decide_rows_launch(Ctx* c, const double* rows_all, int nranks, int T, LmState* states, int64_t n_total, int round,
                              int* flags, int* scored, double* trial_count, double* trial_err, bool core_trailer, double* cnt_rt, int cnt_stride) {
    if (cnt_rt && nranks > 256) return fail(c, RSDSFM_ERR_INVALID, "more than 256 ranks");
    RSDSFM_HIP_CHECK(c, hipMemsetAsync(flags, 0, sizeof(int), c->stream));
    hipLaunchKernelGGL(ransac_decide_kernel, dim3(T), dim3(256), 0, c->stream, rows_all, nranks, T, 0, states, n_total, round, (int)KMAX, flags,
                       static_cast<int*>(nullptr), scored, trial_count, trial_err, kTiledFusedBase, static_cast<int*>(nullptr),
                       static_cast<int*>(nullptr), core_trailer ? T * NSR / 2 + 1 : 0, cnt_rt, cnt_stride);
    RSDSFM_HIP_CHECK(c, hipGetLastError());
    return RSDSFM_OK;
}

int ransac_score_rows_launch(Ctx* c, const double* q, const double* u, const double* a, const double* ak, int64_t n,
                             const double* hyp, int T, const LmState* states, int depth_mode, double tol, const int* scored,
                             double* partials, double* rows) {
    const int grid = ransac_pixel_grid(c, n);
    const int groups = ransac_lm_groups(c, grid, T);
    hipLaunchKernelGGL(ransac_score_kernel, dim3(((grid + 7) / 8) * 8 * groups), dim3(kRB), sizeof(double) * T * 2, c->stream,
                       reinterpret_cast<const double2*>(q), reinterpret_cast<const double2*>(u), a, ak, n, hyp, T, states,
                       depth_mode, tol, scored, partials, grid, groups, static_cast<const int*>(nullptr), static_cast<const int*>(nullptr));
    RSDSFM_HIP_CHECK(c, hipGetLastError());
    hipLaunchKernelGGL(ransac_score_rows_kernel, dim3(T), dim3(256), 0, c->stream, partials, grid, T, scored, rows);
    RSDSFM_HIP_CHECK(c, hipGetLastError());
    return RSDSFM_OK;
}

int ransac_score_merge_launch(Ctx* c, const double* rows_all, int nranks, int T, const int* scored, double* trial_count,
                              double* trial_err, double* cnt_rt, int cnt_stride) {
    if (cnt_rt && nranks > 256) return fail(c, RSDSFM_ERR_INVALID, "more than 256 ranks");
    hipLaunchKernelGGL(ransac_reduce_scores_kernel, dim3(T), dim3(256), 0, c->stream, rows_all, nranks, T, scored, trial_count,
                       trial_err, cnt_rt, cnt_stride);
    RSDSFM_HIP_CHECK(c, hipGetLastError());
    return RSDSFM_OK;
}

int ransac_rows_doubles() { return NSR; }

int ransac_pick_launch(Ctx* c, const double* trial_count, const double* trial_err, int T, const double* hyp, RansacBest* best,
                       RansacBest* best_host, const int* d_flags, int* h_flags, int scored_ahead, const double* cnt_rt, int cnt_stride,
                       int nranks, int64_t* m_all, double tie_margin, PickLazy lazy) {
    hipLaunchKernelGGL(ransac_pick_kernel, dim3(1), dim3(64), 0, c->stream, trial_count, trial_err, T, hyp, best, best_host, d_flags, h_flags, scored_ahead,
                       cnt_rt, cnt_stride, nranks, m_all, tie_margin, lazy);
    RSDSFM_HIP_CHECK(c, hipGetLastError());
    return RSDSFM_OK;
}

int ransac_final_launch(Ctx* c, const double* q, const double* u, const double* a, const double* ak, int64_t n,
                        RansacBest* best, const LmState* states, int depth_mode, double tol, double* rho, uint8_t* mask,
                        int64_t* block_counts, int64_t* block_offsets, int64_t* inlier_idx, double* inliers,
                        double* out_alpha, double* out_alpha_k, RansacBest* best_host, int* zero_words) {
    int64_t blocks = (n + kRB - 1) / kRB;
    if (blocks < 1) blocks = 1;
    const int64_t cap = 2048;
    int64_t chunk = kRB;
    if (blocks > cap) {
        chunk = ((blocks + cap - 1) / cap) * kRB;
        blocks = (n + chunk - 1) / chunk;
    }
    hipLaunchKernelGGL(ransac_final_kernel, dim3((int)blocks), dim3(kRB), 0, c->stream, reinterpret_cast<const double2*>(q),
                       reinterpret_cast<const double2*>(u), a, ak, n, chunk, best, states, depth_mode, tol, rho, mask,
                       block_counts);
    RSDSFM_HIP_CHECK(c, hipGetLastError());
    if (inlier_idx || inliers || out_alpha || out_alpha_k) {
        hipLaunchKernelGGL(ransac_scatter_kernel, dim3((int)blocks), dim3(kRB), 0, c->stream, reinterpret_cast<const double2*>(q),
                           a, ak, n, chunk, rho, mask, block_counts, best, best_host, inlier_idx, inliers, out_alpha, out_alpha_k, zero_words);
    } else {
        if (zero_words) RSDSFM_HIP_CHECK(c, hipMemsetAsync(zero_words, 0, kRefineStateBlockTail, c->stream));
        hipLaunchKernelGGL(ransac_scan_kernel, dim3(1), dim3(256), 0, c->stream, block_counts, (int)blocks, block_offsets, best, best_host);
    }
    RSDSFM_HIP_CHECK(c, hipGetLastError());
    return RSDSFM_OK;
}

}
```

### rs-aware-differential-sfm_amd/csrc/ransac_lma_kernels.hip

```cpp
#include <stdlib.h>

#include <algorithm>

#include "lma_common.hpp"
#include "lma_stages.hpp"
#include "rsdsfm_internal.hpp"

namespace rsdsfm {

namespace {

__device__ __forceinline__ bool is_nan_bits2(double x) {
    const uint32_t h = (uint32_t)__double2hiint(x) & 0x7FFFFFFFu;
    return h > 0x7FF00000u || (h == 0x7FF00000u && __double2loint(x) != 0);
}
__device__ __forceinline__ Pose load_pose(const double* __restrict__ hyp, int t) {
    const double* h_ = hyp + (int64_t)t * 8;
    Pose p;
    p.w[0] = h_[0], p.w[1] = h_[1], p.w[2] = h_[2];
    p.v[0] = h_[3], p.v[1] = h_[4], p.v[2] = h_[5];
    p.k = h_[6];
    return p;
}
__device__ __forceinline__ bool pose_nan(const Pose& p) {
// ... 24 lines not shown
    const int len = (int)min(chunk, n - p0);
    const double2* __restrict__ qb = q + p0;
    const double2* __restrict__ ub = u + p0;
    const double* __restrict__ ab = alpha + p0;
    const double* __restrict__ akb = alpha_k + p0;
    double A = 0.0, B = 0.0, C = 0.0, D = 0.0, E = 0.0, G = 0.0;
    int cnt[NC];
    double es[NC];
#pragma unroll
    for (int c = 0; c < NC; ++c) cnt[c] = 0, es[c] = 0.0;
    if (active) {
        const Pose pose = load_pose(hyp, t);
        const double two_over = 2.0 / (2.0 + pose.k);
        auto pixel = [&](const PixIn& px) -> bool {
            const LmaPx v = lma_pixel(px.x, px.y, px.ux, px.uy, px.al, px.ak, pose, two_over);
            A += v.a;
            B += v.ge;
            C = __builtin_fma(v.e0, v.e0, C);
            D = __builtin_fma(v.rhos, v.rhos, D);
            E = __builtin_fma(v.rhos, v.e0, E);
            G = lma_max_abs(G, v.g);
            const double m = lma_margin(v, cd);
            bool listed = v.clamped;
#pragma unroll
            for (int c = 0; c < NC; ++c) {
                const double e2 = __builtin_fma(v.ge, cd.phi2[c], v.a);
                const bool in = e2 < cd.tol2;
                listed = listed || (fabs(e2 - cd.tol2) <= m);
                cnt[c] += in ? 1 : 0;
                if (ERR) {
                    const double err = sqrt_core(lma_max_pos(e2, kLmaSqrtMin));
                    es[c] = __builtin_fma(err, __hiloint2double((in && e2 >= kLmaSqrtMin) ? 0x3FF00000 : 0, 0), es[c]);
                }
            }
            return listed;
        };
        auto push = [&](unsigned i) {
            const int pos = atomicAdd(&irr_count[t], 1);
            if (pos < kLmaListCap) irr_list[(int64_t)t * kLmaListCap + pos] = (int)(p0 + (int64_t)i);
        };
        const int rounds = len / P;
        unsigned i = (unsigned)slot;
        const unsigned uP = (unsigned)P;
        PixIn pa, pb;
        int r = 0;
        if (rounds > 0) pa = load_pix(qb, ub, ab, akb, i);
        for (; r + 1 < rounds; r += 2, i += 2 * uP) {
            pb = load_pix(qb, ub, ab, akb, i + uP);
            const bool la = pixel(pa);
            pa = load_pix(qb, ub, ab, akb, r + 2 < rounds ? i + 2 * uP : i);
            const bool lb = pixel(pb);
            if (la || lb) {
                if (la) push(i);
                if (lb) push(i + uP);
            }
        }
        if (r < rounds) {
            if (pixel(pa)) push(i);
            i += uP;
        }
        if (i < (unsigned)len && pixel(load_pix(qb, ub, ab, akb, i))) push(i);
    }
    s_part[g][0] = A, s_part[g][1] = B, s_part[g][2] = C, s_part[g][3] = D, s_part[g][4] = E, s_part[g][kLmaG] = G;
#pragma unroll
    for (int c = 0; c < kLmaNC; ++c) {
        s_part[g][6 + 2 * c] = c < NC ? (double)cnt[c < NC ? c : 0] : 0.0;
        s_part[g][7 + 2 * c] = c < NC ? es[c < NC ? c : 0] : 0.0;
    }
    __syncthreads();
    for (int o = g; o < Tl * kLmaSlots; o += kLB) {
        const int tt = o / kLmaSlots, sl = o - tt * kLmaSlots;
        double r = s_part[tt][sl];
        for (int s = 1; s < P; ++s) r = sl == kLmaG ? fmax(r, s_part[s * Tg + tt][sl]) : r + s_part[s * Tg + tt][sl];
        partials[((int64_t)(t0 + tt) * nwg + bid) * kLmaSlots + sl] = r;
    }
    if ((int)blockIdx.x == clk_bid && g == 0) {
        clk_probe[2] = __builtin_amdgcn_s_memtime();
        clk_probe[3] = __builtin_amdgcn_s_memrealtime();
    }
}

__device__ __forceinline__ void lma_publish(int t, const LmScal& st, const double* hist_l, int fallback, bool scored, double count, double err,
                                            LmState* states, int* flags, int* __restrict__ scored_out, double* __restrict__ trial_count,
                                            double* __restrict__ trial_err, int* steps_hist, int* __restrict__ unscored_list, int* guard_word, bool count_only) {
    LmState* state = states + t;
    if (fallback) {
        LmScal f = {};
        f.status = 0;
        f.K = KMAX;
        f.termination = -1;
        f.rho_holds = -1;
        f.launches = 0;
        f.next_launch = 1;
        f.radius = kInitialRadius;
        f.decrease_factor = 2.0;
        double r = kInitialRadius;
        for (int j = 0; j < KMAX; ++j) {
            f.cand[j] = r;
            r = radius_accept(r, 1.0);
        }
        *static_cast<LmScal*>(state) = f;
        atomicAdd(&flags[0], 1);
        atomicOr(&flags[3], 16 | (1 << (8 + fallback)));
        (void)guard_word;
        return;
    }
    *static_cast<LmScal*>(state) = st;
    for (int j = 0; j < st.n_hist && j < kMaxIter; ++j) state->hist[j] = hist_l[j];
    if (steps_hist) atomicAdd(&steps_hist[st.n_hist < 1 ? 0 : (st.n_hist > 3 ? 3 : st.n_hist)], 1);
    if (scored) {
        trial_count[t] = count;
        trial_err[t] = err;
        scored_out[t] = count_only ? 2 : 1;
    } else {
        const int pos = atomicAdd(&flags[1], 1);
        if (unscored_list) unscored_list[pos] = t;
    }
}

__global__ __launch_bounds__(kLB) void ransac_lma_rows_decide_kernel(const double* __restrict__ partials, int nblocks, int T, const double2* __restrict__ q,
                                                                    const double2* __restrict__ u, const double* __restrict__ alpha,
                                                                    const double* __restrict__ alpha_k, int64_t n, const double* __restrict__ hyp,
                                                                    const LmaCand cd, const int* __restrict__ irr_count, const int* __restrict__ irr_list,
                                                                    LmState* states, int* flags, int* __restrict__ scored_out, double* __restrict__ trial_count,
                                                                    double* __restrict__ trial_err, int* __restrict__ unscored_list, int* guard_word,
                                                                    const int* __restrict__ m9_core_flag, int m9_core_epoch) {
    __shared__ double s_row[kLmaRow];
    const int t = blockIdx.x;
    if (t == 0 && threadIdx.x == 0 && m9_core_flag && *m9_core_flag == m9_core_epoch) atomicOr(&flags[3], 1);
    lma_rows_stage(partials, nblocks, T, t, q, u, alpha, alpha_k, load_pose(hyp, t), cd, irr_count, irr_list, s_row);
    __syncthreads();
    if (threadIdx.x == 0) {
        LmScal st;
        double hist_l[kMaxIter];
        bool scored;
        double count, err;
        const Pose pose = load_pose(hyp, t);
        const int fb = lma_decide(s_row, n, cd, cd.plan, pose_nan(pose), st, hist_l, scored, count, err);
        lma_publish(t, st, hist_l, fb, scored, count, err, states, flags, scored_out, trial_count, trial_err, flags + 4, unscored_list, guard_word, cd.count_only != 0);
    }
}

__global__ __launch_bounds__(kLB) void ransac_lma_rows_kernel(const double* __restrict__ partials, int nblocks, int T, const double2* __restrict__ q,
                                                             const double2* __restrict__ u, const double* __restrict__ alpha,
                                                             const double* __restrict__ alpha_k, const double* __restrict__ hyp, const LmaCand cd,
                                                             const int* __restrict__ irr_count, const int* __restrict__ irr_list, double* __restrict__ rows) {
    __shared__ double s_row[kLmaRow];
    const int t = blockIdx.x;
    lma_rows_stage(partials, nblocks, T, t, q, u, alpha, alpha_k, load_pose(hyp, t), cd, irr_count, irr_list, s_row);
    __syncthreads();
    if (threadIdx.x < kLmaRow) rows[(int64_t)t * kLmaRow + threadIdx.x] = s_row[threadIdx.x];
}

__global__ __launch_bounds__(64) void ransac_lma_decide_kernel(const double* __restrict__ rows_all, int nranks, int64_t rank_stride, int T, int64_t n_total,
                                                              const double* __restrict__ hyp, const LmaCand cd, LmState* states, int* flags,
                                                              int* __restrict__ scored_out, double* __restrict__ trial_count,
                                                              double* __restrict__ trial_err, int* __restrict__ unscored_list, int* guard_word,
                                                              double* __restrict__ cnt_rt, int cnt_stride, const int* __restrict__ m9_core_flag, int m9_core_epoch) {
    const int t = blockIdx.x * 64 + threadIdx.x;
    if (t == 0 && m9_core_flag && *m9_core_flag == m9_core_epoch) atomicOr(&flags[3], 1);
    if (t >= T) return;
    double row[kLmaRow];
    for (int j = 0; j < kLmaRow; ++j) {
        const bool is_max = j == kLmaG || j == kLmaRowX0 + 1 || (j >= kLmaRowXk && j < kLmaRowScore && ((j - kLmaRowXk) % 5) == 4) || j == 7;
        double r = rows_all[(int64_t)t * kLmaRow + j];
        for (int rk = 1; rk < nranks; ++rk) {
            const double x = rows_all[rk * rank_stride + (int64_t)t * kLmaRow + j];
            r = is_max ? fmax(r, x) : r + x;
        }
        row[j] = r;
    }
    LmScal st;
    double hist_l[kMaxIter];
    bool scored;
    double count, err;
    const Pose pose = load_pose(hyp, t);
    const int fb = lma_decide(row, n_total, cd, cd.plan, pose_nan(pose), st, hist_l, scored, count, err);
    lma_publish(t, st, hist_l, fb, scored, count, err, states, flags, scored_out, trial_count, trial_err, nullptr, unscored_list, guard_word, cd.count_only != 0);
    if (cnt_rt && scored && !fb) {
        int cc = -1;
        for (int c = 0; c < cd.nc; ++c)
            if (cd.steps[c] == st.n_hist) cc = c;
        for (int rk = 0; rk < nranks; ++rk) cnt_rt[(int64_t)rk * cnt_stride + t] = cc >= 0 ? rows_all[rk * rank_stride + (int64_t)t * kLmaRow + kLmaRowScore + 2 * cc] : 0.0;
    }
}

LmaCand lma_candidates(const int* steps, int nc, double tol, bool count_only = false) {
    LmaCand cd;
    const LmaPlan plan = lma_plan();
    cd.plan = plan;
    cd.nc = std::min(std::max(nc, 1), (int)kLmaNC);
    for (int c = 0; c < kLmaNC; ++c) {
        const int s = c < cd.nc ? std::min(std::max(steps[c], 1), kLmaKP - 1) : 1;
        cd.steps[c] = s;
        cd.phi2[c] = plan.phi[s] * plan.phi[s];
    }
    cd.tol = tol;
    cd.tol2 = tol * tol;
    cd.c1 = std::max(0.5 * kLmaEta * tol, kLmaMarginFloor);
    cd.c1x2 = 2.0 * cd.c1;
    cd.count_only = count_only ? 1 : 0;
    return cd;
}

int ransac_lma_group_size(int T, int* groups_out) {
    int best_ng = 1;
    double best_u = 0.0;
    for (int ng = 1; ng <= 8 && ng <= T; ++ng) {
        const int tg = (T + ng - 1) / ng, ngu = (T + tg - 1) / tg;
        const double u = (double)T * (kLB / tg) / ((double)ngu * kLB);
        if (u > best_u + 1e-9) best_u = u, best_ng = ng;
        if (u >= 0.9) {
            best_ng = ng;
            break;
        }
    }
    const int tg = (T + best_ng - 1) / best_ng;
    if (groups_out) *groups_out = (T + tg - 1) / tg;
    return tg;
}

int ransac_lma_grid(const Ctx* c, int64_t n, int T, int64_t* chunk_out, int blocks_per_cu) {
    const int P = std::max(1, kLB / std::max(T, 1));
    if (n <= 0) {
        *chunk_out = P;
        return 1;
    }
    int64_t g = (n + (int64_t)P * 8 - 1) / ((int64_t)P * 8);
    g = std::max<int64_t>(1, std::min<int64_t>(g, (int64_t)c->num_cus * std::max(1, std::min(blocks_per_cu, 8))));
    int64_t chunk = (n + g - 1) / g;
    chunk = ((chunk + P - 1) / P) * P;
    g = std::max<int64_t>(1, (n + chunk - 1) / chunk);
    *chunk_out = chunk;
    return (int)g;
}
int64_t ransac_lma_partials_doubles(const Ctx* c, int64_t n, int batch) {
    const int64_t gmax = std::min<int64_t>((int64_t)c->num_cus * 8, std::max<int64_t>(1, (n + 7) / 8));
    return gmax * batch * kLmaSlots;
}
size_t ransac_lma_list_ints(int batch) { return (size_t)batch * kLmaListCap; }

static int lma_pass_launch(Ctx* c, const double* q, const double* u, const double* a, const double* ak, int64_t n, const double* hyp, int T,
                           const LmaCand& cd, double* partials, int* irr_count, int* irr_list, int* grid_out, unsigned long long* clk = nullptr) {
    static int occ_tab[2][kLmaNC + 1] = {{0, 0, 0, 0}, {0, 0, 0, 0}};
    const int nc = std::min(std::max(cd.nc, 1), (int)kLmaNC);
    int* occ = occ_tab[cd.count_only ? 1 : 0];
    if (occ[nc] == 0) {
        int nb = 0;
        const void* fn = cd.count_only ? (nc == 1 ? reinterpret_cast<const void*>(&ransac_lma_kernel<1, false>) : nc == 2 ? reinterpret_cast<const void*>(&ransac_lma_kernel<2, false>) : reinterpret_cast<const void*>(&ransac_lma_kernel<3, false>))
                                       : (nc == 1 ? reinterpret_cast<const void*>(&ransac_lma_kernel<1, true>) : nc == 2 ? reinterpret_cast<const void*>(&ransac_lma_kernel<2, true>) : reinterpret_cast<const void*>(&ransac_lma_kernel<3, true>));
        if (hipOccupancyMaxActiveBlocksPerMultiprocessor(&nb, fn, kLB, 0) != hipSuccess || nb < 1) nb = 4;
        occ[nc] = nb;
    }
    int64_t chunk;
    static const int grid_override = getenv("RSDSFM_LMA_BLOCKS_PER_CU") ? atoi(getenv("RSDSFM_LMA_BLOCKS_PER_CU")) : 0;
    int groups = 1;
    const int Tg = ransac_lma_group_size(T, &groups);
    const int per_cu = std::max(1, (grid_override > 0 ? grid_override : occ[nc]));
    int nwg = ransac_lma_grid(c, n, Tg, &chunk, per_cu);
    if (groups > 1) {
        const int64_t cap = std::max<int64_t>(1, (int64_t)c->num_cus * std::min(per_cu, 8) / groups);
        if (nwg > cap) {
            const int P = std::max(1, kLB / Tg);
            chunk = (n + cap - 1) / cap;
            chunk = ((chunk + P - 1) / P) * P;
            nwg = (int)std::max<int64_t>(1, (n + chunk - 1) / chunk);
        }
    }
    const int grid = nwg * groups;
    *grid_out = nwg;
    const double2* q2 = reinterpret_cast<const double2*>(q);
    const double2* u2 = reinterpret_cast<const double2*>(u);
    const int clk_bid = clk ? grid / 2 : -1;
#define RSDSFM_LMA_LAUNCH(NC, ERR) \
    hipLaunchKernelGGL((ransac_lma_kernel<NC, ERR>), dim3(grid), dim3(kLB), 0, c->stream, q2, u2, a, ak, n, hyp, T, cd, partials, irr_count, irr_list, chunk, clk, clk_bid, Tg, nwg)
    if (cd.count_only) {
        if (cd.nc == 1) RSDSFM_LMA_LAUNCH(1, false);
        else if (cd.nc == 2) RSDSFM_LMA_LAUNCH(2, false);
        else RSDSFM_LMA_LAUNCH(3, false);
    } else if (cd.nc == 1) RSDSFM_LMA_LAUNCH(1, true);
    else if (cd.nc == 2) RSDSFM_LMA_LAUNCH(2, true);
    else RSDSFM_LMA_LAUNCH(3, true);
#undef RSDSFM_LMA_LAUNCH
    RSDSFM_HIP_CHECK(c, hipGetLastError());
    return RSDSFM_OK;
}

int ransac_lma_launch(Ctx* c, const double* q, const double* u, const double* a, const double* ak, int64_t n, const double* hyp, int T,
                      LmState* states, double* partials, int* flags, int* scored, double* trial_count, double* trial_err, double tol,
                      const int* cand_steps, int ncand, int* irr_count, int* irr_list, int* unscored_list, int* guard_word, const int* m9_core_flag,
                      int m9_core_epoch, bool count_only) {
    if (T < 1 || T > kLB) return fail(c, RSDSFM_ERR_INVALID, "hypothesis batch of the analytic pass exceeds 256");
    const LmaCand cd = lma_candidates(cand_steps, ncand, tol, count_only);
    int grid = 0;
    const bool prof = c->profile && c->ev_prof[0] && c->ev_prof[1];
    if (prof) RSDSFM_HIP_CHECK(c, hipEventRecord(c->ev_prof[0], c->stream));
    int rc = lma_pass_launch(c, q, u, a, ak, n, hyp, T, cd, partials, irr_count, irr_list, &grid, prof ? c->d_clk_probe : nullptr);
    if (rc != RSDSFM_OK) return rc;
    if (prof) {
        RSDSFM_HIP_CHECK(c, hipEventRecord(c->ev_prof[1], c->stream));
        c->prof_pending = true;
        c->prof_what = 0;
    }
    hipLaunchKernelGGL(ransac_lma_rows_decide_kernel, dim3(T), dim3(kLB), 0, c->stream, partials, grid, T, reinterpret_cast<const double2*>(q),
                       reinterpret_cast<const double2*>(u), a, ak, n, hyp, cd, irr_count, irr_list, states, flags, scored, trial_count, trial_err,
                       unscored_list, guard_word, m9_core_flag, m9_core_epoch);
    RSDSFM_HIP_CHECK(c, hipGetLastError());
    return RSDSFM_OK;
}

int ransac_lma_rows_doubles() { return kLmaRow; }
int ransac_lma_rows_launch(Ctx* c, const double* q, const double* u, const double* a, const double* ak, int64_t n, const double* hyp, int T,
                           double* partials, double tol, const int* cand_steps, int ncand, int* irr_count, int* irr_list, double* rows) {
    if (T < 1 || T > kLB) return fail(c, RSDSFM_ERR_INVALID, "hypothesis batch of the analytic pass exceeds 256");
    const LmaCand cd = lma_candidates(cand_steps, ncand, tol);
    int grid = 0;
    int rc = lma_pass_launch(c, q, u, a, ak, n, hyp, T, cd, partials, irr_count, irr_list, &grid);
    if (rc != RSDSFM_OK) return rc;
    hipLaunchKernelGGL(ransac_lma_rows_kernel, dim3(T), dim3(kLB), 0, c->stream, partials, grid, T, reinterpret_cast<const double2*>(q),
                       reinterpret_cast<const double2*>(u), a, ak, hyp, cd, irr_count, irr_list, rows);
    RSDSFM_HIP_CHECK(c, hipGetLastError());
    return RSDSFM_OK;
}
int ransac_lma_decide_rows_launch(Ctx* c, const double* rows_all, int nranks, int64_t rank_stride, int T, int64_t n_total, const double* hyp,
                                  LmState* states, int* flags, int* scored, double* trial_count, double* trial_err, double tol, const int* cand_steps,
                                  int ncand, int* unscored_list, int* guard_word, double* cnt_rt, int cnt_stride, const int* m9_core_flag, int m9_core_epoch) {
    const LmaCand cd = lma_candidates(cand_steps, ncand, tol);
    hipLaunchKernelGGL(ransac_lma_decide_kernel, dim3((T + 63) / 64), dim3(64), 0, c->stream, rows_all, nranks, rank_stride, T, n_total, hyp, cd, states,
                       flags, scored, trial_count, trial_err, unscored_list, guard_word, cnt_rt, cnt_stride, m9_core_flag, m9_core_epoch);
    RSDSFM_HIP_CHECK(c, hipGetLastError());
    return RSDSFM_OK;
}

}
```

### rs-aware-differential-sfm_amd/csrc/rsdsfm_internal.hpp

```cpp
#pragma once

#include <hip/hip_runtime.h>
#include <stdint.h>

#include <functional>
#include <string>
#include <vector>

#include "../../include/rsdsfm.h"

namespace rsdsfm {

constexpr int kMaxIter = 50;
constexpr int kRefineTraceCols = RSDSFM_REFINE_TRACE_COLS;
constexpr double kInitialRadius = 1e4;
constexpr double kMaxRadius = 1e16;
constexpr double kMinRadius = 1e-32;
constexpr double kMinRelDecrease = 1e-3;
constexpr double kMinLmDiag = 1e-6;
constexpr double kMaxLmDiag = 1e32;
constexpr double kFunctionTol = 1e-6;
constexpr double kGradientTol = 1e-10;
static_assert(kGradientTol < 1.0, "the indicator encoding of the gradient-maximum slots needs kGradientTol < 1");
constexpr double kParameterTol = 1e-8;
constexpr int kMaxInvalid = 5;
constexpr double kLmaTie = 1e-11;

constexpr int KMAX = 3;
constexpr int NS = 3 + 5 * KMAX;

struct Pose {
    double v[3];
    double w[3];
    double k;
};

struct LmScal {
    int32_t status;
    int32_t n_hist;
    int32_t K;
    int32_t write_which;
    int32_t iteration;
    int32_t num_successful;
    int32_t num_unsuccessful;
    int32_t invalid_run;
    int32_t termination;
    int32_t rho_holds;
    int32_t launches;
    int32_t next_launch;
    int32_t predict;
    int32_t restart;
    double radius;
    double decrease_factor;
    double cost;
    double initial_cost;
    double cand[KMAX];
};
struct LmState : LmScal {
    double hist[kMaxIter];
};

constexpr size_t kRefineStateBlockTail = 32;
struct RansacBest {
    int32_t best_trial;
    int32_t undecided;
    int64_t num_inliers;
    int64_t num_inliers_scan;
    double inlier_error;
    double hyp[8];
    int32_t lma_tie;
    int32_t shared_best;
    int32_t _pad_shared;
    int32_t lazy_pending;
};
struct PickLazy {
    int* scored = nullptr;
    int* list = nullptr;
    int* list_count = nullptr;
};

constexpr int kScoreIdleLimit = 4;
constexpr int kRansacBatch = 128;

struct Ctx {
    int device = 0;
    hipStream_t stream = nullptr;
    bool own_stream = false;
    std::string err;
    double* d_partials = nullptr;
    unsigned* d_tickets = nullptr;
    LmState* d_lm = nullptr;
    LmState* h_lm = nullptr;
    int lm_issued_k = 0;
    int true_flow_exhaustive = 0;
    int ransac_fused_base = 2;
    int ransac_score_idle = kScoreIdleLimit;
    int refine_iters_hint = -1;
    int ransac_standard_math = 0;
    int* d_core_flag = nullptr;
    int core_epoch = 0;
    int ransac_math_mode = 0;
    int64_t ransac_restarts = 0;
    int lm_arithmetic = 0;
    int lma_hold = 0;
    bool lma_count_only_force = false;
    int64_t lma_count_only_runs = 0, lma_lazy_runs = 0;
    int lma_unique_run = 0;
    int64_t lma_restarts = 0;
    int64_t lma_handed_over = 0;
    int lma_last_guard = 0;
    int* d_lma_list = nullptr;
    int depth_lma_parity = 0;
    int lma_cand[2] = {2, 1};
    int ransac_spec_miss = 0;
    int frame_dense_hint = 1;
    int lm_issued_d = 0;
    int depth_epoch = 0;
    int depth_standard_math = 0;
    int64_t depth_restarts = 0;
    int depth_core_launch = 0;
    int prof_what = 0;
    void* d_stage = nullptr;
    size_t stage_bytes = 0;
    void* d_ws = nullptr;
    size_t ws_bytes = 0;
    void* d_frame = nullptr;
    size_t frame_bytes = 0;
    void* h_pinned = nullptr;
    hipEvent_t ev_ready = nullptr;
    size_t pinned_bytes = 0;
    int num_cus = 256;
    int ransac_k0 = 0;
    int ransac_not_one_step = -1;
    bool profile = false;
    hipEvent_t ev_prof[2] = {nullptr, nullptr};
    unsigned long long* d_clk_probe = nullptr;
    bool prof_pending = false;
    double* d_refine_trace = nullptr;
    int refine_trace_rows = 0;
    int depth_variant = 0;
    void* d_tile = nullptr;
    size_t tile_bytes = 0;
    void* tile_session = nullptr;
    int tile_np = 0;
    void* flow_pair = nullptr;
    void* flow_clip = nullptr;
    int flow_batch = 0;
    void* flow_check = nullptr;
    void* rectify_dense = nullptr;
    unsigned* d_claim[3] = {nullptr, nullptr, nullptr};
    size_t claim_words[3] = {0, 0, 0};
    unsigned claim_epoch[3] = {0, 0, 0};
    void* dist = nullptr;
    void* frame_run = nullptr;
    hipStream_t aux_stream = nullptr;
    hipEvent_t ev_fork = nullptr, ev_join = nullptr, ev_seq = nullptr;
    int frame_side_flatten = 3;
    int frame_tail = 0;
    unsigned long long* d_flat_counters = nullptr;
    int seq_lanes = 0;
    int refine_stage_mode = 0;
    bool refine_stage_separate = false;
    int refine_arithmetic = 0;
    int64_t refine_rf_runs = 0, refine_rf_restarts = 0, refine_rf_resolves = 0;
    int refine_rf_last_guard = 0;
    struct RansacCache {
        uint64_t tag = 0, stage_gen = 0;
        const double *d_u = nullptr, *d_inl = nullptr, *d_alpha = nullptr, *d_alpha_k = nullptr;
        const int64_t* d_idx = nullptr;
        int64_t n = 0, m = 0;
        const void* h_u = nullptr;
        double u_probe[16] = {0};
        double inl_probe[16] = {0};
    } ransac_cache;
    uint64_t stage_gen = 0, ransac_tag_counter = 0;
    int64_t refine_cache_hits = 0;
    std::vector<rsdsfm_ctx*> lanes;
};
constexpr int kSequenceLanesDefault = 3;
void dist_release(Ctx* c);
void dist_reset_hold(Ctx* c);
void frame_release(Ctx* c);
void flow_release(Ctx* c);
void flow_check_release(Ctx* c);
void rectify_dense_release(Ctx* c);

constexpr int kDepthBlock = 256;
constexpr int kDepthMaxBlocks = 512;
constexpr int kDecideBlock = 256;
constexpr int kDepthBatchMax = 8;

#define RSDSFM_HIP_CHECK(ctx, expr)                                                            \
    do {                                                                                       \
        hipError_t _e = (expr);                                                                \
        if (_e != hipSuccess) {                                                                \
            (ctx)->err = std::string(#expr) + ": " + hipGetErrorString(_e);                    \
            return RSDSFM_ERR_HIP;                                                             \
        }                                                                                      \
    } while (0)

struct DeviceGuard {
    int prev = -1;
    bool switched = false;
    explicit DeviceGuard(const Ctx* c) {
        if (hipGetDevice(&prev) == hipSuccess && prev != c->device) switched = hipSetDevice(c->device) == hipSuccess;
    }
    ~DeviceGuard() {
        if (switched) (void)hipSetDevice(prev);
    }
    DeviceGuard(const DeviceGuard&) = delete;
    DeviceGuard& operator=(const DeviceGuard&) = delete;
};

int fail(Ctx* c, int code, const char* msg);
int ensure_stage(Ctx* c, size_t bytes);
struct XferItem {
    void* host;
    const void* dev;
    size_t bytes;
};
struct XferUp {
    void* dev;
    const void* host;
    size_t bytes;
};
int xfer_h2d(Ctx* c, void* d_dst, const void* h_src, size_t bytes);
int xfer_h2d_many(Ctx* c, const XferUp* items, int count);
int xfer_d2h(Ctx* c, void* h_dst, const void* d_src, size_t bytes);
int xfer_d2h_many(Ctx* c, const XferItem* items, int count);
bool xfer_trace_on();
void xfer_trace(const char* label);
void xfer_trace_span(const char* label, double us);
void xfer_trace_dump(const char* what);
int ensure_ws(Ctx* c, size_t bytes);
int sync_stream(Ctx* c, const char* where);
void set_sync_dumper(std::function<void(Ctx*)> f);
int ensure_pinned(Ctx* c, size_t bytes);

struct Arena {
    char* base;
    size_t off = 0;
// ... 25 lines not shown
bool depth_lma_allowed(const Ctx* c, int64_t n);
int depth_lma_batch_launch(Ctx* const* cs, int count, const double* const* q, const double* const* u, const double* const* a,
                           const double* const* ak, const int64_t* n, const Pose* poses, double* const* rho);
int depth_lma_row_doubles();
int depth_lma_shard_launch(Ctx* c, const double* q, const double* u, const double* a, const double* ak, int64_t n, const Pose& pose, double* rho, double* d_row);
int depth_lma_shard_finish_launch(Ctx* c, const double* q, const double* u, const double* a, const double* ak, int64_t n, const Pose& pose, double* rho,
                                  const double* d_rows_all, int nranks, int64_t n_total);

}

namespace rsdsfm {
int alpha_launch(Ctx* c, const double* flow_px, int64_t n, double h, double gamma, double* alpha);
int alpha_k_launch(Ctx* c, const double* q_px, const double* flow_px, int64_t n, double h, double gamma, double* alpha_k);
int depth_map_device(Ctx* c, double* d_inl, int64_t m, double v_inout[3], double fx, double fy, double cx, double cy, int32_t rows, int32_t cols,
                     double* d_depth_map, int32_t* d_xs, int32_t* d_ys, int* flipped, const double* w_or_null, double k, double gamma,
                     double* d_R_rows9, double* d_t_rows3);
struct PoseTableOut {
    double* R = nullptr;
    double* t = nullptr;
    int rows = 0;
    double gamma = 0.0;
    const double* wk_dev = nullptr;
};
int pose_table_launch(Ctx* c, const Pose& pose, double gamma, int rows, double* R, double* t, const double* v_dev = nullptr,
                      const double* wk_dev = nullptr);
int64_t flatten_cells(int rows, int cols);
int flatten_launch(Ctx* c, const double* d_img, int rows, int cols, int col0, double fx, double fy, double cx, double cy,
                   double gamma, double thr, double* d_q, double* d_u, double* d_alpha, double* d_alpha_k, int64_t* d_counts,
                   int64_t* d_offsets, int64_t* d_total, hipEvent_t total_ready = nullptr);
int depth_map_launch(Ctx* c, double* d_inl, int64_t m, const double v[3], double fx, double fy, double cx, double cy, int rows,
                     int cols, double* d_depth_map, int32_t* d_xs, int32_t* d_ys, double* d_header, double* d_partials,
                     double* h_header = nullptr, const double* v_dev = nullptr, const int64_t* m_dev = nullptr,
                     const PoseTableOut* pt = nullptr);
int depth_map_slab_launch(Ctx* c, double* d_inl, int64_t m, const double* d_zsums, int nz, int64_t m_total, const double v[3],
                          double fx, double fy, double cx, double cy, int rows, int col0, int ncols, double* d_depth_map,
                          int32_t* d_xs, int32_t* d_ys, double* d_header, double* h_header = nullptr, const double* v_dev = nullptr,
                          const int64_t* m_dev = nullptr, const PoseTableOut* pt = nullptr);
int claim_map_acquire(Ctx* c, int which, size_t npix, unsigned** map, unsigned* tag, unsigned* mask);
int claim_map_reserve(Ctx* c, int which, size_t words);
int zsum_row_launch(Ctx* c, const double* d_inl, int64_t m, double* d_partials, double* d_out);
}

namespace rsdsfm {
struct Minimal9Direct {
    const double* img = nullptr;
    int rows = 0, cols = 0, alpha_ones = 0;
    double fx = 0, fy = 0, cx = 0, cy = 0, gamma = 0;
    int* core_flag = nullptr;
    int core_epoch = 0;
    double* probe = nullptr;
};
int minimal9_launch(Ctx* c, const double* q, const double* u, const double* alpha, const double* alpha_k,
                    const int32_t* samples, int T, int use_alpha_k, int k_sign_mode, double* hyp_out, void* zero_begin = nullptr,
                    size_t zero_bytes = 0, const Minimal9Direct* direct = nullptr);
struct DenseFlatten {
    double thr = 0.0;
    double *d_q = nullptr, *d_u = nullptr, *d_alpha = nullptr, *d_alpha_k = nullptr;
    unsigned long long* d_counters = nullptr;
    int64_t* total_out = nullptr;
};
int minimal9_flatten_launch(Ctx* c, const int32_t* samples, int T, int use_alpha_k, int k_sign_mode, double* hyp_out, void* zero_begin, size_t zero_bytes,
                            const Minimal9Direct& direct, double thr, double* d_q, double* d_u, double* d_alpha, double* d_alpha_k,
                            unsigned long long* d_counters, int64_t* total_out);
}

namespace rsdsfm {
int ransac_pixel_grid(const Ctx* c, int64_t n);
int ransac_lm_partials_doubles(const Ctx* c, int64_t n, int batch);
int ransac_lm_round_launch(Ctx* c, const double* q, const double* u, const double* a, const double* ak, int64_t n,
                           const double* hyp, int T, LmState* states, double* partials, int* flags, int* scored,
                           double* trial_count, double* trial_err, int round, double tol, int k0, int fused_base, bool core_math,
                           const int* m9_core_flag = nullptr, int m9_core_epoch = 0, int* unscored_list = nullptr);
int ransac_score_launch(Ctx* c, const double* q, const double* u, const double* a, const double* ak, int64_t n,
                        const double* hyp, int T, const LmState* states, int depth_mode, double tol, const int* scored,
                        double* partials, double* trial_count, double* trial_err, const int* unscored_list = nullptr, const int* unscored_count = nullptr);
int ransac_pick_launch(Ctx* c, const double* trial_count, const double* trial_err, int T, const double* hyp, RansacBest* best,
                       RansacBest* best_host = nullptr, const int* d_flags = nullptr, int* h_flags = nullptr, int scored_ahead = 0,
                       const double* cnt_rt = nullptr, int cnt_stride = 0, int nranks = 0, int64_t* m_all = nullptr, double tie_margin = 0.0,
                       PickLazy lazy = PickLazy());
int ransac_final_launch(Ctx* c, const double* q, const double* u, const double* a, const double* ak, int64_t n,
                        RansacBest* best, const LmState* states, int depth_mode, double tol, double* rho, uint8_t* mask,
                        int64_t* block_counts, int64_t* block_offsets, int64_t* inlier_idx, double* inliers,
                        double* out_alpha, double* out_alpha_k, RansacBest* best_host = nullptr, int* zero_words = nullptr);
int ransac_rows_doubles();
int ransac_lm_rows_launch(Ctx* c, const double* q, const double* u, const double* a, const double* ak, int64_t n,
                          const double* hyp, int T, const LmState* states, double* partials, int round, double tol, double* rows,
                          int* core_flags = nullptr, const int* m9_flag = nullptr, int m9_epoch = 0);
int ransac_rows_payload_doubles(int T, bool core_trailer);
int ransac_decide_rows_launch(Ctx* c, const double* rows_all, int nranks, int T, LmState* states, int64_t n_total, int round,
                              int* flags, int* scored, double* trial_count, double* trial_err, bool core_trailer = false,
                              double* cnt_rt = nullptr, int cnt_stride = 0);
int ransac_score_rows_launch(Ctx* c, const double* q, const double* u, const double* a, const double* ak, int64_t n,
                             const double* hyp, int T, const LmState* states, int depth_mode, double tol, const int* scored,
                             double* partials, double* rows);
int ransac_score_merge_launch(Ctx* c, const double* rows_all, int nranks, int T, const int* scored, double* trial_count,
                              double* trial_err, double* cnt_rt = nullptr, int cnt_stride = 0);
void sample_indices(int64_t n, int T, uint64_t seed, int32_t* out);
int64_t ransac_lma_partials_doubles(const Ctx* c, int64_t n, int batch);
size_t ransac_lma_list_ints(int batch);
int ransac_lma_launch(Ctx* c, const double* q, const double* u, const double* a, const double* ak, int64_t n, const double* hyp, int T,
                      LmState* states, double* partials, int* flags, int* scored, double* trial_count, double* trial_err, double tol,
                      const int* cand_steps, int ncand, int* irr_count, int* irr_list, int* unscored_list, int* guard_word,
                      const int* m9_core_flag = nullptr, int m9_core_epoch = 0, bool count_only = false);
int ransac_lma_rows_doubles();
int ransac_lma_rows_launch(Ctx* c, const double* q, const double* u, const double* a, const double* ak, int64_t n, const double* hyp, int T,
                           double* partials, double tol, const int* cand_steps, int ncand, int* irr_count, int* irr_list, double* rows);
int ransac_lma_decide_rows_launch(Ctx* c, const double* rows_all, int nranks, int64_t rank_stride, int T, int64_t n_total, const double* hyp,
                                  LmState* states, int* flags, int* scored, double* trial_count, double* trial_err, double tol, const int* cand_steps,
                                  int ncand, int* unscored_list, int* guard_word, double* cnt_rt, int cnt_stride, const int* m9_core_flag = nullptr,
                                  int m9_core_epoch = 0);
}

namespace rsdsfm {
struct RefineState {
    int32_t np, cur, iteration, invalid_run, num_successful, num_unsuccessful, termination, solve_ok;
    double p[7], pc[7], sp[7], yp[7];
    double radius, decrease_factor, cost, initial_cost, x_norm, gmax, stepsq_p;
    int64_t m;
    int32_t grid;
    int32_t need_schur;
    double zsum;
    int32_t slots;
    int32_t spec_miss_run;
    int32_t pending_apply;
    int32_t rf;
    double dp[7];
    double p0[7];
    int32_t rf_guard, rf_resolves;
};
constexpr int kTermRestartExact = 64;
struct FinishClaim {
    bool on = false;
    double fx = 0.0, fy = 0.0, cx = 0.0, cy = 0.0;
    int rows = 0, cols = 0;
    int32_t* ys = nullptr;
    unsigned* owner = nullptr;
    unsigned tag = 0, mask = 0;
};
struct RefineBuffers {
    const double* flow;
    int64_t n_flow, m;
    bool m_on_device = false;
    const double* inl;
    const double* alpha;
    const double* alpha_k;
    const int64_t* inlier_idx;
    int flow_index_mode;
    RefineState* state;
    double* uu;
    double* beta;
    double* rho_a;
    double* rho_b;
    double* srho;
    double* partials;
    int* bad_index;
    RefineState* state_host = nullptr;
    double* zpartials = nullptr;
    const RansacBest* best_dev = nullptr;
    FinishClaim claim;
    bool want_zsum = false;
};
size_t ransac_pinned_bytes(int T);
typedef std::function<int(const RansacBest*)> RansacSpecTail;
struct RansacRun {
    int pc = 0;
    const double *d_q = nullptr, *d_u = nullptr, *d_a = nullptr, *d_ak = nullptr;
    int64_t n = 0;
    int T = 0, Tn = 1, batch = 1, depth_mode = 0, use_alpha_k = 0, k_sign_mode = 0, k0 = 0, fused_base = 0;
    double tol = 0.0;
    rsdsfm_ransac_out* out = nullptr;
    const RansacSpecTail* spec_tail = nullptr;
    bool* spec_tail_held = nullptr;
    int core_epoch = 0;
    int* d_unscored = nullptr;
    bool core_math = true;
    bool analytic = false;
    bool lma_restarted = false;
    int* refine_flag_words = nullptr;
    bool count_only = false;
    int lazy_rounds = 0;
    int shared_best = 0;
    double tie_margin = 0.0;
    int lma_guard = 0;
    bool lma_tie_seen = false;
    int lma_cand[2] = {2, 1}, lma_cand_next[2] = {0, 0};
    int *d_irr_count = nullptr, *d_irr_list = nullptr;
    bool restarted = false;
    bool tail_ahead = true;
    const Minimal9Direct* direct = nullptr;
    const DenseFlatten* dense = nullptr;
    const std::function<int()>* after_minimal9 = nullptr;
    std::vector<int32_t> samples;
    double *d_hyp = nullptr, *d_partials = nullptr, *d_tcount = nullptr, *d_terr = nullptr, *d_rho = nullptr;
    char* zero_begin = nullptr;
    size_t zero_bytes = 0;
    LmState* d_states = nullptr;
    int *d_scored = nullptr, *d_flags = nullptr;
    RansacBest* d_best = nullptr;
    int64_t *d_bcounts = nullptr, *d_boffs = nullptr;
    uint8_t* d_mask = nullptr;
    RansacBest* h_best = nullptr;
    int* h_running = nullptr;
    double *h_tcount = nullptr, *h_terr = nullptr, *h_hyp = nullptr;
    LmState* h_states = nullptr;
    int32_t* h_samples_pinned = nullptr;
    int b0 = 0, B = 0, round = 0;
    bool need_score = true, final_done = false, spec_scored = false, tail_enqueued = false, spec_final = false;
    int not_one_step = 0, fused_base_next = 0, score_hint_next = -1;
    bool hints_ready = false;
};
int ransac_begin(Ctx* c, const double* d_q, const double* d_u, const double* d_a, const double* d_ak, int64_t n, int use_alpha_k, int T,
                 double tol, const int32_t* h_samples, uint64_t seed, int depth_mode, int k_sign_mode, rsdsfm_ransac_out* out,
                 const RansacSpecTail* spec_tail, bool* spec_tail_held, RansacRun* run, const Minimal9Direct* direct,
                 const std::function<int()>* after_minimal9, const DenseFlatten* dense = nullptr, bool tail_ahead = true, bool count_only = false,
                 int* refine_flag_words = nullptr);
int ransac_finish(Ctx* c, RansacRun* run);
void ransac_commit_hints(Ctx* c, const RansacRun& run);
int flatten_enqueue(Ctx* c, const double* d_img, int32_t rows, int32_t cols, double fx, double fy, double cx, double cy, double gamma,
                    double thr, double* d_q, double* d_u, double* d_alpha, double* d_alpha_k, int64_t* h_total);
typedef std::function<int(const RefineBuffers&)> RefineTail;
int refine_finish_grid(const Ctx* c, const RefineBuffers& B);
int depth_map_decided_launch(Ctx* c, double* d_inl, int64_t m, const double* d_zsums, int nz, const RefineBuffers& B, double* d_depth_map,
                             double* d_header, double* h_header, const double* v_dev, const int64_t* m_dev, const PoseTableOut* pt);
struct RefineRun {
    RefineBuffers B;
    int np = 6, launched = 0, chunk = 5, hint_prev = -1;
    bool rf = false;
    double* d_inl_out = nullptr;
    const RefineTail* tail = nullptr;
    RefineState* hs = nullptr;
    bool prefetch = false, prefetched = false;
    bool tail_done = false;
};
constexpr size_t kPinnedTail = 1024;
size_t refine_workspace_bytes(const Ctx* c, int64_t m, bool m_on_device);
int refine_begin(Ctx* c, const double* d_flow, int64_t n_flow, int64_t m, const double* d_inl, const double* d_alpha,
                 const double* d_alpha_k, const int64_t* d_inlier_idx, const double v_in[3], const double w_in[3], double k_in,
                 int const_acceleration, int flow_index_mode, double* d_inl_out, const RefineTail* tail, const RansacBest* d_best,
                 void* ws_base, RefineRun* run, RefineState* hs_prefetch, double* d_zpartials, bool exact = false,
                 const FinishClaim* claim = nullptr);
constexpr int kRcRefineRestartExact = 1;
int refine_device(Ctx* c, const double* d_flow, int64_t n_flow, int64_t m, const double* d_inl, const double* d_alpha,
                  const double* d_alpha_k, const int64_t* d_inlier_idx, const double v_in[3], const double w_in[3], double k_in,
                  int const_acceleration, int flow_index_mode, double* d_inl_out, double v_out[3], double w_out[3], double* k_out,
                  rsdsfm_lm_summary* summary, const RefineTail* tail, double* d_zpartials, bool exact = false, const FinishClaim* claim = nullptr);
int refine_enqueue_chunk(Ctx* c, RefineRun* run);
int frames_in_flight(const Ctx* c);
int refine_poll(Ctx* c, RefineRun* run, double v_out[3], double w_out[3], double* k_out, rsdsfm_lm_summary* summary);
int refine_partials_doubles(const Ctx* c, int64_t m);
int refine_partials_doubles_cap(const Ctx* c);
int refine_state_from_best_launch(Ctx* c, const RansacBest* d_best, const RefineBuffers& B, int np);
int* refine_flag_words(void* ws_base);
inline int refine_trace_reset(Ctx* c) {
    if (!c->d_refine_trace) return RSDSFM_OK;
    return hipMemsetAsync(c->d_refine_trace, 0xFF, (size_t)c->refine_trace_rows * kRefineTraceCols * sizeof(double), c->stream) == hipSuccess ? RSDSFM_OK : RSDSFM_ERR_HIP;
}
int refine_init_launch(Ctx* c, const RefineBuffers& B, int np);
int refine_rf_pass_launch(Ctx* c, const RefineBuffers& B, int np, int g, int g_first, const double* rows_all_prev, int nranks, int64_t m_total,
                          const int64_t* m_total_dev, bool publish = false);
int refine_rf_apply_launch(Ctx* c, const RefineBuffers& B, int np, int g, bool to_published, const double* rows_all, int nranks, int64_t m_total,
                           const int64_t* m_total_dev);
int refine_rf_row_launch(Ctx* c, const RefineBuffers& B, int np, int g, double* row);
int refine_rf_row_doubles(int np);
void refine_rf_debug_dump(Ctx* c, const RefineBuffers& B);
int refine_rf_read_stamps(Ctx* c, unsigned long long out[16]);
int refine_rf_extra_doubles();
int refine_partials_half_doubles(const Ctx* c);
int refine_state_doubles();
inline int* refine_rf_counters(const RefineBuffers& B) { return B.bad_index + 4; }
// ... 27 lines not shown
```

Measured before the change: 1729.

## Compact RANSAC inliers in one pass reusing the analytic LM pass's per-block counts

```diff
diff --git a/include/rsdsfm.h b/include/rsdsfm.h
--- a/include/rsdsfm.h
+++ b/include/rsdsfm.h
@@ -80,6 +80,8 @@
 int rsdsfm_ransac_restarts(rsdsfm_ctx* ctx, int64_t* count);
 int rsdsfm_set_lm_arithmetic(rsdsfm_ctx* ctx, int mode);
 int rsdsfm_lma_restarts(rsdsfm_ctx* ctx, int64_t* count, int32_t* last_guards_or_null);
+int rsdsfm_set_ransac_compaction(rsdsfm_ctx* ctx, int mode);
+int rsdsfm_ransac_compaction(rsdsfm_ctx* ctx, int64_t* one_pass, int64_t* fell_back, int32_t* reasons_or_null);
 int rsdsfm_refine_restarts(rsdsfm_ctx* ctx, int64_t* runs, int64_t* restarts, int64_t* resolves_or_null, int32_t* last_guard_or_null);
 int rsdsfm_set_refine_arithmetic(rsdsfm_ctx* ctx, int mode);
 int rsdsfm_lma_count_only(rsdsfm_ctx* ctx, int64_t* runs, int64_t* lazy_runs_or_null);
diff --git a/rs-aware-differential-sfm_amd/__init__.py b/rs-aware-differential-sfm_amd/__init__.py
--- a/rs-aware-differential-sfm_amd/__init__.py
+++ b/rs-aware-differential-sfm_amd/__init__.py
@@ -240,6 +240,14 @@
         n, g = C.c_int64(0), C.c_int32(0)
         self._check(self.lib.rsdsfm_lma_restarts(self._ctx, C.byref(n), C.byref(g)), "rsdsfm_lma_restarts")
         return int(n.value), int(g.value)
+
+    def set_ransac_compaction(self, mode):
+        self._check(self.lib.rsdsfm_set_ransac_compaction(self._ctx, int(mode)), "rsdsfm_set_ransac_compaction")
+
+    def ransac_compaction(self):
+        a, b, g = C.c_int64(0), C.c_int64(0), C.c_int32(0)
+        self._check(self.lib.rsdsfm_ransac_compaction(self._ctx, C.byref(a), C.byref(b), C.byref(g)), "rsdsfm_ransac_compaction")
+        return int(a.value), int(b.value), int(g.value)
 
     def lma_count_only(self):
         a, b = C.c_int64(0), C.c_int64(0)
diff --git a/rs-aware-differential-sfm_amd/csrc/capi.hip b/rs-aware-differential-sfm_amd/csrc/capi.hip
--- a/rs-aware-differential-sfm_amd/csrc/capi.hip
+++ b/rs-aware-differential-sfm_amd/csrc/capi.hip
@@ -347,6 +347,26 @@
     return RSDSFM_OK;
 }
 
+int rsdsfm_set_ransac_compaction(rsdsfm_ctx* ctx, int mode) {
+    CTX_OR_FAIL(ctx);
+    if (mode != 0 && mode != 1) return fail(c, RSDSFM_ERR_INVALID, "ransac compaction: 0 = one pass on the pixel pass's counts (default), 1 = the two kernels");
+    c->ransac_compaction = mode;
+    for (rsdsfm_ctx* lane : c->lanes) lane->c.ransac_compaction = mode;
+    return RSDSFM_OK;
+}
+
+int rsdsfm_ransac_compaction(rsdsfm_ctx* ctx, int64_t* one_pass, int64_t* fell_back, int32_t* reasons_or_null) {
+    CTX_OR_FAIL(ctx);
+    if (!one_pass || !fell_back) return fail(c, RSDSFM_ERR_INVALID, "ransac compaction: null output");
+    int64_t a = c->compact_runs, b = c->compact_fallbacks;
+    int reasons = c->compact_reasons;
+    for (rsdsfm_ctx* lane : c->lanes) a += lane->c.compact_runs, b += lane->c.compact_fallbacks, reasons |= lane->c.compact_reasons;
+    *one_pass = a;
+    *fell_back = b;
+    if (reasons_or_null) *reasons_or_null = reasons;
+    return RSDSFM_OK;
+}
+
 int rsdsfm_set_refine_arithmetic(rsdsfm_ctx* ctx, int mode) {
     CTX_OR_FAIL(ctx);
     if (mode != 0 && mode != 1) return fail(c, RSDSFM_ERR_INVALID, "refine arithmetic: 0 = radius-factorised (default), 1 = iterate by iterate");
diff --git a/rs-aware-differential-sfm_amd/csrc/frame_host.hip b/rs-aware-differential-sfm_amd/csrc/frame_host.hip
--- a/rs-aware-differential-sfm_amd/csrc/frame_host.hip
+++ b/rs-aware-differential-sfm_amd/csrc/frame_host.hip
@@ -192,7 +192,6 @@
     F->ro.inliers = F->d_inl;
     F->ro.alpha = F->d_in_a;
     F->ro.alpha_k = F->d_in_ak;
-    F->ro.mask = F->d_mask;
     F->m_known = -1;
     F->tail = [c, F](const RefineBuffers& B) -> int {
         const rsdsfm_frame_job& J2 = F->job;
@@ -426,6 +425,7 @@
         lc->lma_count_only_force = c->lma_count_only_force;
         lc->frame_side_flatten = c->frame_side_flatten;
         lc->frame_tail = c->frame_tail;
+        lc->ransac_compaction = c->ransac_compaction;
         lc->refine_stage_mode = c->refine_stage_mode;
     }
     for (int l = 0; l < L; ++l) lane_ctx(l)->refine_stage_separate = L > 1;
diff --git a/rs-aware-differential-sfm_amd/csrc/lma_stages.hpp b/rs-aware-differential-sfm_amd/csrc/lma_stages.hpp
--- a/rs-aware-differential-sfm_amd/csrc/lma_stages.hpp
+++ b/rs-aware-differential-sfm_amd/csrc/lma_stages.hpp
@@ -24,7 +24,8 @@
 __device__ __forceinline__ void lma_rows_stage(const double* __restrict__ partials, int nblocks, int T, int t, const double2* __restrict__ q,
                                                const double2* __restrict__ u, const double* __restrict__ alpha, const double* __restrict__ alpha_k,
                                                const Pose& pose, const LmaCand& cd, const int* __restrict__ irr_count,
-                                               const int* __restrict__ irr_list, double* s_row) {
+                                               const int* __restrict__ irr_list, double* s_row, int* __restrict__ listed_out = nullptr,
+                                               int8_t* __restrict__ listed_dc_out = nullptr) {
     __shared__ double s_red3[768];
     __shared__ int s_list[kLmaListCap], s_sorted[kLmaListCap];
     constexpr int LBATCH = 64;
@@ -116,7 +117,9 @@
                 }
                 xr[2 + 5 * kLmaKP + 2 * c] = dc;
                 xr[2 + 5 * kLmaKP + 2 * c + 1] = de;
-            }
+                if (listed_dc_out) listed_dc_out[e * kLmaNC + c] = (int8_t)dc;
+            }
+            if (listed_out) listed_out[e] = (int)i;
             xr[XW - 2] = v.clamped ? v.a : 0.0;
             xr[XW - 1] = v.clamped ? 1.0 : 0.0;
         } else {
@@ -144,7 +147,7 @@
 __device__ __forceinline__ bool lma_band(double x, double thr) { return fabs(x - thr) <= kLmaBand * fabs(thr); }
 
 __device__ __forceinline__ int lma_decide(const double* row, int64_t n, const LmaCand& cd, const LmaPlan& plan, bool nan_pose, LmScal& st, double* hist, bool& scored,
-                                          double& count, double& err, double* phi_out = nullptr) {
+                                          double& count, double& err, double* phi_out = nullptr, int* fused_c_out = nullptr) {
     const double A = row[0], B = row[1], C = row[2], D = row[3], E = row[4], G = row[5];
     const bool listed_walk = row[6] != 0.0;
     int fallback = 0;
@@ -264,6 +267,7 @@
     if (phi_out) *phi_out = phi;
     scored = false;
     count = err = 0.0;
+    if (fused_c_out) *fused_c_out = -1;
     if (fallback) return fallback;
     if (nan_pose) {
         scored = true;
@@ -275,6 +279,7 @@
             count = row[kLmaRowScore + 2 * c];
             err = row[kLmaRowScore + 2 * c + 1];
             scored = true;
+            if (fused_c_out) *fused_c_out = c;
         }
     return 0;
 }
diff --git a/rs-aware-differential-sfm_amd/csrc/ransac_host.hip b/rs-aware-differential-sfm_amd/csrc/ransac_host.hip
--- a/rs-aware-differential-sfm_amd/csrc/ransac_host.hip
+++ b/rs-aware-differential-sfm_amd/csrc/ransac_host.hip
@@ -103,6 +103,22 @@
     const int64_t n = R.n;
     const double tol = R.tol;
     int rc = RSDSFM_OK;
+    auto final_stage = [&]() -> int {
+        R.compact_used = R.compact_allowed && !R.compact_failed && R.analytic && ransac_compact_fits(R.compact);
+        if (R.compact_used)
+            return ransac_compact_launch(c, R.d_q, R.d_u, R.d_a, R.d_ak, n, R.d_best, R.d_states, R.d_lma_partials, R.compact, R.d_irr_count, tol, out->inlier_idx,
+                                         out->inliers, out->alpha, out->alpha_k, R.h_best, R.refine_flag_words);
+        return ransac_final_launch(c, R.d_q, R.d_u, R.d_a, R.d_ak, n, R.d_best, R.d_states, depth_mode, tol, R.d_rho, R.d_mask, R.d_bcounts, R.d_boffs,
+                                   out->inlier_idx, out->inliers, out->alpha, out->alpha_k, R.h_best, R.refine_flag_words);
+    };
+    auto compact_check = [&]() -> bool {
+        const int bits = R.compact_used ? (R.h_best->compact_word & 0xFF) : 0;
+        if (!bits) return true;
+        R.compact_failed = true;
+        R.compact_reason |= bits;
+        R.final_done = R.tail_enqueued = R.spec_final = false;
+        return false;
+    };
     for (;;) {
         switch (R.pc) {
             case kPcStart: {
@@ -156,9 +172,9 @@
                 bool flags_via_pick = false;
                 if (round > 4 * kMaxIter) return fail(c, RSDSFM_ERR_NUMERIC, "LM state machines did not terminate");
                 if (R.analytic && round == 0) {
-                    rc = ransac_lma_launch(c, R.d_q, R.d_u, R.d_a, R.d_ak, n, R.d_hyp + (size_t)b0 * 8, B, R.d_states + b0, R.d_partials, R.d_flags,
+                    rc = ransac_lma_launch(c, R.d_q, R.d_u, R.d_a, R.d_ak, n, R.d_hyp + (size_t)b0 * 8, B, R.d_states + b0, R.d_lma_partials, R.d_flags,
                                            R.d_scored + b0, R.d_tcount + b0, R.d_terr + b0, tol, R.lma_cand, 2, R.d_irr_count, R.d_irr_list, R.d_unscored,
-                                           nullptr, R.core_epoch ? c->d_core_flag : nullptr, R.core_epoch, R.count_only);
+                                           nullptr, R.core_epoch ? c->d_core_flag : nullptr, R.core_epoch, R.count_only, R.compact_allowed ? &R.compact : nullptr);
                 } else {
                     rc = ransac_lm_round_launch(c, R.d_q, R.d_u, R.d_a, R.d_ak, n, R.d_hyp + (size_t)b0 * 8, B, R.d_states + b0, R.d_partials, R.d_flags,
                                                 R.d_scored + b0, R.d_tcount + b0, R.d_terr + b0, round, tol, R.k0, R.fused_base, R.core_math,
@@ -181,8 +197,7 @@
                                             nullptr, 0, 0, nullptr, R.tie_margin, lazy);
                     if (rc != RSDSFM_OK) return rc;
                     flags_via_pick = true;
-                    rc = ransac_final_launch(c, R.d_q, R.d_u, R.d_a, R.d_ak, n, R.d_best, R.d_states, depth_mode, tol, R.d_rho, R.d_mask, R.d_bcounts,
-                                             R.d_boffs, out->inlier_idx, out->inliers, out->alpha, out->alpha_k, R.h_best, R.refine_flag_words);
+                    rc = final_stage();
                     if (rc != RSDSFM_OK) return rc;
                     R.final_done = true;
                     R.spec_final = true;
@@ -262,14 +277,14 @@
                 break;
             }
             case kPcFinal: {
+                if (R.final_done) (void)compact_check();
                 if (!R.final_done) {
                     R.tail_enqueued = false;
                     R.spec_final = false;
                     rc = ransac_pick_launch(c, R.d_tcount, R.d_terr, T, R.d_hyp, R.d_best, R.h_best, nullptr, nullptr, 0, nullptr, 0, 0, nullptr, R.tie_margin,
                                             R.count_only ? PickLazy{R.d_scored, R.d_unscored, R.d_flags + 1} : PickLazy());
                     if (rc != RSDSFM_OK) return rc;
-                    rc = ransac_final_launch(c, R.d_q, R.d_u, R.d_a, R.d_ak, n, R.d_best, R.d_states, depth_mode, tol, R.d_rho, R.d_mask, R.d_bcounts,
-                                             R.d_boffs, out->inlier_idx, out->inliers, out->alpha, out->alpha_k, R.h_best, R.refine_flag_words);
+                    rc = final_stage();
                     if (rc != RSDSFM_OK) return rc;
                 }
                 if (R.spec_tail && !R.tail_enqueued) {
@@ -307,6 +322,10 @@
                     if (rc != RSDSFM_OK) return rc;
                     break;
                 }
+                if (!compact_check()) {
+                    R.pc = kPcFinal;
+                    break;
+                }
                 R.lma_tie_seen = h_best->lma_tie != 0;
                 R.shared_best = h_best->shared_best;
                 if (h_best->num_inliers != h_best->num_inliers_scan) {
@@ -349,6 +368,10 @@
     if (R.score_hint_next >= 0) c->ransac_score_idle = R.score_hint_next ? 0 : std::min(c->ransac_score_idle + 1, kScoreIdleLimit);
     c->ransac_not_one_step = R.not_one_step;
     c->ransac_spec_miss = R.spec_final ? 0 : std::min(c->ransac_spec_miss + 1, 2);
+    if (R.compact_eligible) {
+        if (R.compact_used) c->compact_runs += 1;
+        else c->compact_fallbacks += 1, c->compact_reasons |= R.compact_reason | (!R.analytic ? kCompactNotAnalytic : !R.compact_allowed ? kCompactGeometry : 0);
+    }
     if (R.count_only) c->lma_count_only_runs += 1, c->lma_lazy_runs += (R.lazy_rounds > 0 || R.shared_best > 1) ? 1 : 0;
     if (R.lazy_rounds > 0 || R.shared_best > 1) c->lma_unique_run = 0;
     else if (R.shared_best == 1) c->lma_unique_run = std::min(c->lma_unique_run + 1, 2);
@@ -400,10 +423,17 @@
     const int Tn = std::max(T, 1);
     const int batch = std::min(Tn, kRansacBatch);
     const size_t partials_doubles = std::max<size_t>((size_t)ransac_lm_partials_doubles(c, n, batch), (size_t)ransac_lma_partials_doubles(c, n, batch));
+    const bool wants_compacted = (out->inlier_idx || out->inliers || out->alpha || out->alpha_k) && T > 0 && depth_mode == RSDSFM_DEPTH_CERES_LM;
+    R.compact_eligible = wants_compacted && c->ransac_compaction == 0;
+    R.compact_allowed = R.compact_eligible && R.analytic && Tn <= kRansacBatch && !out->inv_depth && !out->mask;
+    const size_t lma_keep_doubles = R.compact_allowed ? (size_t)ransac_lma_partials_doubles(c, n, batch) : 0;
     size_t need = Arena::need(sizeof(double) * Tn * 8) + Arena::need(sizeof(int) * batch) + Arena::need(sizeof(int) * ransac_lma_list_ints(batch)) +
                   Arena::need(sizeof(LmState) * Tn) + Arena::need(sizeof(double) * partials_doubles) +
                   Arena::need(sizeof(int) * 8) + 2 * Arena::need(sizeof(int) * Tn) + 2 * Arena::need(sizeof(double) * Tn) + Arena::need(sizeof(RansacBest)) +
                   2 * Arena::need(sizeof(int64_t) * 2048) + Arena::need(sizeof(double) * (size_t)n) + Arena::need((size_t)n) + 4096;
+    if (R.compact_allowed)
+        need += Arena::need(sizeof(double) * lma_keep_doubles) + Arena::need(sizeof(int) * ransac_lma_list_ints(batch)) +
+                Arena::need(ransac_lma_list_ints(batch) * kCompactNC) + Arena::need(sizeof(int) * batch);
     int rc = ensure_ws(c, need);
     if (rc != RSDSFM_OK) return rc;
     Arena ws(c->d_ws);
@@ -424,6 +454,13 @@
     R.d_boffs = ws.take<int64_t>(2048);
     R.d_rho = out->inv_depth ? out->inv_depth : ws.take<double>((size_t)n);
     R.d_mask = out->mask ? out->mask : ws.take<uint8_t>((size_t)n);
+    R.d_lma_partials = R.d_partials;
+    if (R.compact_allowed) {
+        R.d_lma_partials = ws.take<double>(lma_keep_doubles);
+        R.compact.listed = ws.take<int>(ransac_lma_list_ints(batch));
+        R.compact.listed_dc = ws.take<int8_t>(ransac_lma_list_ints(batch) * kCompactNC);
+        R.compact.fused_c = ws.take<int>(batch);
+    }
 
     rc = ensure_pinned(c, ransac_pinned_bytes(T));
     if (rc != RSDSFM_OK) return rc;
diff --git a/rs-aware-differential-sfm_amd/csrc/ransac_kernels.hip b/rs-aware-differential-sfm_amd/csrc/ransac_kernels.hip
--- a/rs-aware-differential-sfm_amd/csrc/ransac_kernels.hip
+++ b/rs-aware-differential-sfm_amd/csrc/ransac_kernels.hip
@@ -2,6 +2,7 @@
 
 #include "device_math.hpp"
 #include "lm_common.hpp"
+#include "lma_common.hpp"
 #include "rsdsfm_internal.hpp"
 
 namespace rsdsfm {
@@ -685,6 +686,7 @@
         best->lma_tie = tie;
         best->lazy_pending = pending;
         best->shared_best = ns;
+        best->compact_word = undecided ? kCompactPickUndecided : 0;
         best->num_inliers = bi >= 0 ? (int64_t)best_count : 0;
         best->inlier_error = best_err;
         if (best_host) {
@@ -693,6 +695,7 @@
             best_host->lma_tie = tie;
             best_host->lazy_pending = pending;
             best_host->shared_best = ns;
+            best_host->compact_word = undecided ? kCompactPickUndecided : 0;
             best_host->num_inliers = bi >= 0 ? (int64_t)best_count : 0;
             best_host->inlier_error = best_err;
         }
@@ -854,6 +857,162 @@
         __syncthreads();
         if (tid == 0) s_base += total;
         __syncthreads();
+    }
+}
+
+
+constexpr int kCompactRowsPerThread = 8;
+constexpr int kCompactListPerThread = (kLmaListCap + kRB - 1) / kRB;
+static_assert(kLmaNC == kCompactNC, "LmaCompactIn carries the fused iterates");
+__global__ __launch_bounds__(kRB) void ransac_compact_kernel(const double2* __restrict__ q, const double2* __restrict__ u, const double* __restrict__ alpha,
+                                                            const double* __restrict__ alpha_k, int64_t n, int64_t chunk, int nwg, RansacBest* best,
+                                                            RansacBest* best_host, const LmState* __restrict__ states, const double* __restrict__ partials,
+                                                            const LmaCompactIn in_, const int* __restrict__ irr_count, double tol,
+                                                            int64_t* __restrict__ inlier_idx, double* __restrict__ inliers, double* __restrict__ out_alpha,
+                                                            double* __restrict__ out_alpha_k, int* __restrict__ zero_words) {
+    __shared__ LmPlanLds plan;
+    __shared__ int s_wave[2][kRB / 64];
+    __shared__ int64_t s_sum[3][kRB / 64];
+    const int tid = threadIdx.x, lane = tid & 63, wv = tid >> 6;
+    const int b = (int)blockIdx.x;
+    if (zero_words && b == 0 && tid < (int)(kRefineStateBlockTail / sizeof(int))) zero_words[tid] = 0;
+    if (best->compact_word & kCompactPickUndecided) return;
+    const int bt = best->best_trial;
+    const int64_t picked = best->num_inliers;
+    Pose pose;
+    pose.w[0] = best->hyp[0], pose.w[1] = best->hyp[1], pose.w[2] = best->hyp[2];
+    pose.v[0] = best->hyp[3], pose.v[1] = best->hyp[4], pose.v[2] = best->hyp[5];
+    pose.k = best->hyp[6];
+    const int btc = bt < 0 ? 0 : bt;
+    const int nh = states[btc].n_hist;
+    const int fc = in_.fused_c[btc];
+    const int raw = irr_count[btc];
+    if (tid < kMaxIter) plan.inv_hist[tid] = 1.0 / states[btc].hist[tid];
+    double cv[kCompactRowsPerThread][kLmaNC];
+#pragma unroll
+    for (int j = 0; j < kCompactRowsPerThread; ++j) {
+        const int bj = tid + j * kRB;
+        const double* __restrict__ row = partials + ((int64_t)btc * nwg + (bj < nwg ? bj : 0)) * kLmaSlots + 6;
+#pragma unroll
+        for (int c = 0; c < kLmaNC; ++c) cv[j][c] = row[2 * c];
+    }
+    int lp[kCompactListPerThread];
+    int8_t ld[kCompactListPerThread][kLmaNC];
+#pragma unroll
+    for (int j = 0; j < kCompactListPerThread; ++j) {
+        const int e = tid + j * kRB;
+        const int64_t le = (int64_t)btc * kLmaListCap + (e < kLmaListCap ? e : 0);
+        lp[j] = in_.listed[le];
+#pragma unroll
+        for (int c = 0; c < kLmaNC; ++c) ld[j][c] = in_.listed_dc[le * kLmaNC + c];
+    }
+    int c_sel = -1;
+#pragma unroll
+    for (int c = 0; c < kLmaNC; ++c)
+        if (c < in_.nc && in_.steps[c] == nh) c_sel = c;
+    if (tid == 0) {
+        plan.n_hist = nh;
+        plan.K = 0;
+        plan.write_which = 0;
+    }
+    const int64_t i0 = (int64_t)b * chunk;
+    const int64_t i1 = (i0 + chunk < n) ? i0 + chunk : n;
+    int64_t pre = 0, all = 0, mine = 0;
+#pragma unroll
+    for (int j = 0; j < kCompactRowsPerThread; ++j) {
+        const int bj = tid + j * kRB;
+        double v = 0.0;
+#pragma unroll
+        for (int c = 0; c < kLmaNC; ++c) v = c == c_sel ? cv[j][c] : v;
+        const int64_t cnt = bj < nwg ? (int64_t)v : 0;
+        all += cnt;
+        pre += bj < b ? cnt : 0;
+        mine += bj == b ? cnt : 0;
+    }
+    const int nl = raw < kLmaListCap ? raw : kLmaListCap;
+#pragma unroll
+    for (int j = 0; j < kCompactListPerThread; ++j) {
+        const int e = tid + j * kRB;
+        int d = 0;
+#pragma unroll
+        for (int c = 0; c < kLmaNC; ++c) d = c == c_sel ? (int)ld[j][c] : d;
+        if (e >= nl) d = 0;
+        const int64_t p = lp[j];
+        all += d;
+        pre += p < i0 ? d : 0;
+        mine += (p >= i0 && p < i1) ? d : 0;
+    }
+#pragma unroll
+    for (int off = 32; off > 0; off >>= 1) {
+        pre += __shfl_down(pre, off);
+        all += __shfl_down(all, off);
+        mine += __shfl_down(mine, off);
+    }
+    if (lane == 0) s_sum[0][wv] = pre, s_sum[1][wv] = all, s_sum[2][wv] = mine;
+    __syncthreads();
+    int64_t base = 0, total = 0, predicted = 0;
+#pragma unroll
+    for (int w2 = 0; w2 < kRB / 64; ++w2) base += s_sum[0][w2], total += s_sum[1][w2], predicted += s_sum[2][w2];
+    int reason = 0;
+    if (bt < 0 || c_sel < 0) reason |= kCompactNoIterate;
+    else if (fc != c_sel) reason |= kCompactNotFused;
+    if (raw > kLmaListCap) reason |= kCompactOverflow;
+    if (!reason && total != picked) reason |= kCompactTotal;
+    if (reason) {
+        if (b == 0 && tid == 0) {
+            best->undecided = 1;
+            best->compact_word = reason;
+            if (best_host) best_host->undecided = 1, best_host->compact_word = reason;
+        }
+        return;
+    }
+    if (b == 0 && tid == 0) {
+        best->num_inliers_scan = total;
+        if (best_host) best_host->num_inliers_scan = total;
+    }
+    const double two_over = 2.0 / (2.0 + pose.k);
+    int64_t run = base;
+    int it = 0;
+    for (int64_t start = i0; start < i1; start += kRB, it ^= 1) {
+        const int64_t i = start + tid;
+        bool in = false;
+        double2 qq = make_double2(0.0, 0.0);
+        double al = 0.0, ak = 0.0, rho = 0.0;
+        if (i < i1) {
+            qq = q[i];
+            const double2 uu = u[i];
+            al = alpha[i], ak = alpha_k[i];
+            rho = hyp_rho(qq.x, qq.y, uu.x, uu.y, al, ak, pose, two_over, RSDSFM_DEPTH_CERES_LM, plan);
+            in = point_error(qq.x, qq.y, uu.x, uu.y, al, ak, pose, two_over, rho) < tol;
+        }
+        const unsigned long long bal = __ballot(in);
+        const int prefix = __popcll(bal & ((1ull << lane) - 1ull));
+        if (lane == 0) s_wave[it][wv] = __popcll(bal);
+        __syncthreads();
+        int woff = 0, found = 0;
+#pragma unroll
+        for (int w2 = 0; w2 < kRB / 64; ++w2) {
+            const int cw = s_wave[it][w2];
+            if (w2 < wv) woff += cw;
+            found += cw;
+        }
+        const int64_t o = run + woff + prefix;
+        if (in && o < n) {
+            if (inlier_idx) inlier_idx[o] = i;
+            if (inliers) {
+                inliers[3 * o + 0] = qq.x;
+                inliers[3 * o + 1] = qq.y;
+                inliers[3 * o + 2] = 1.0 / rho;
+            }
+            if (out_alpha) out_alpha[o] = al;
+            if (out_alpha_k) out_alpha_k[o] = ak;
+        }
+        run += found;
+    }
+    if (tid == 0 && run - base != predicted) {
+        best->undecided = 1;
+        best->compact_word = kCompactCount;
+        if (best_host) best_host->undecided = 1, best_host->compact_word = kCompactCount;
     }
 }
 
@@ -1043,4 +1202,16 @@
     return RSDSFM_OK;
 }
 
-}
+bool ransac_compact_fits(const LmaCompactIn& in) { return in.nwg >= 1 && in.nwg <= kCompactRowsPerThread * kRB && in.chunk >= 1 && in.listed && in.listed_dc && in.fused_c; }
+
+int ransac_compact_launch(Ctx* c, const double* q, const double* u, const double* a, const double* ak, int64_t n, RansacBest* best,
+                          const LmState* states, const double* partials, const LmaCompactIn& in, const int* irr_count, double tol,
+                          int64_t* inlier_idx, double* inliers, double* out_alpha, double* out_alpha_k, RansacBest* best_host, int* zero_words) {
+    if (!ransac_compact_fits(in)) return fail(c, RSDSFM_ERR_INVALID, "one-pass compaction: geometry of the pixel pass out of range");
+    hipLaunchKernelGGL(ransac_compact_kernel, dim3(in.nwg), dim3(kRB), 0, c->stream, reinterpret_cast<const double2*>(q), reinterpret_cast<const double2*>(u),
+                       a, ak, n, in.chunk, in.nwg, best, best_host, states, partials, in, irr_count, tol, inlier_idx, inliers, out_alpha, out_alpha_k, zero_words);
+    RSDSFM_HIP_CHECK(c, hipGetLastError());
+    return RSDSFM_OK;
+}
+
+}
diff --git a/rs-aware-differential-sfm_amd/csrc/ransac_lma_kernels.hip b/rs-aware-differential-sfm_amd/csrc/ransac_lma_kernels.hip
--- a/rs-aware-differential-sfm_amd/csrc/ransac_lma_kernels.hip
+++ b/rs-aware-differential-sfm_amd/csrc/ransac_lma_kernels.hip
@@ -130,8 +130,10 @@
 
 __device__ __forceinline__ void lma_publish(int t, const LmScal& st, const double* hist_l, int fallback, bool scored, double count, double err,
                                             LmState* states, int* flags, int* __restrict__ scored_out, double* __restrict__ trial_count,
-                                            double* __restrict__ trial_err, int* steps_hist, int* __restrict__ unscored_list, int* guard_word, bool count_only) {
+                                            double* __restrict__ trial_err, int* steps_hist, int* __restrict__ unscored_list, int* guard_word, bool count_only,
+                                            int* __restrict__ fused_c_out = nullptr, int fused_c = -1) {
     LmState* state = states + t;
+    if (fused_c_out) fused_c_out[t] = (fallback || !scored) ? -1 : fused_c;
     if (fallback) {
         LmScal f = {};
         f.status = 0;
@@ -172,20 +174,24 @@
                                                                     const LmaCand cd, const int* __restrict__ irr_count, const int* __restrict__ irr_list,
                                                                     LmState* states, int* flags, int* __restrict__ scored_out, double* __restrict__ trial_count,
                                                                     double* __restrict__ trial_err, int* __restrict__ unscored_list, int* guard_word,
-                                                                    const int* __restrict__ m9_core_flag, int m9_core_epoch) {
+                                                                    const int* __restrict__ m9_core_flag, int m9_core_epoch, int* __restrict__ listed_out,
+                                                                    int8_t* __restrict__ listed_dc_out, int* __restrict__ fused_c_out) {
     __shared__ double s_row[kLmaRow];
     const int t = blockIdx.x;
     if (t == 0 && threadIdx.x == 0 && m9_core_flag && *m9_core_flag == m9_core_epoch) atomicOr(&flags[3], 1);
-    lma_rows_stage(partials, nblocks, T, t, q, u, alpha, alpha_k, load_pose(hyp, t), cd, irr_count, irr_list, s_row);
+    lma_rows_stage(partials, nblocks, T, t, q, u, alpha, alpha_k, load_pose(hyp, t), cd, irr_count, irr_list, s_row,
+                   listed_out ? listed_out + (int64_t)t * kLmaListCap : nullptr, listed_dc_out ? listed_dc_out + (int64_t)t * kLmaListCap * kLmaNC : nullptr);
     __syncthreads();
     if (threadIdx.x == 0) {
         LmScal st;
         double hist_l[kMaxIter];
         bool scored;
         double count, err;
+        int fused_c = -1;
         const Pose pose = load_pose(hyp, t);
-        const int fb = lma_decide(s_row, n, cd, cd.plan, pose_nan(pose), st, hist_l, scored, count, err);
-        lma_publish(t, st, hist_l, fb, scored, count, err, states, flags, scored_out, trial_count, trial_err, flags + 4, unscored_list, guard_word, cd.count_only != 0);
+        const int fb = lma_decide(s_row, n, cd, cd.plan, pose_nan(pose), st, hist_l, scored, count, err, nullptr, &fused_c);
+        lma_publish(t, st, hist_l, fb, scored, count, err, states, flags, scored_out, trial_count, trial_err, flags + 4, unscored_list, guard_word, cd.count_only != 0,
+                    fused_c_out, fused_c);
     }
 }
 
@@ -289,7 +295,8 @@
 size_t ransac_lma_list_ints(int batch) { return (size_t)batch * kLmaListCap; }
 
 static int lma_pass_launch(Ctx* c, const double* q, const double* u, const double* a, const double* ak, int64_t n, const double* hyp, int T,
-                           const LmaCand& cd, double* partials, int* irr_count, int* irr_list, int* grid_out, unsigned long long* clk = nullptr) {
+                           const LmaCand& cd, double* partials, int* irr_count, int* irr_list, int* grid_out, unsigned long long* clk = nullptr,
+                           int64_t* chunk_out = nullptr) {
     static int occ_tab[2][kLmaNC + 1] = {{0, 0, 0, 0}, {0, 0, 0, 0}};
     const int nc = std::min(std::max(cd.nc, 1), (int)kLmaNC);
     int* occ = occ_tab[cd.count_only ? 1 : 0];
@@ -317,6 +324,7 @@
     }
     const int grid = nwg * groups;
     *grid_out = nwg;
+    if (chunk_out) *chunk_out = chunk;
     const double2* q2 = reinterpret_cast<const double2*>(q);
     const double2* u2 = reinterpret_cast<const double2*>(u);
     const int clk_bid = clk ? grid / 2 : -1;
@@ -337,14 +345,21 @@
 int ransac_lma_launch(Ctx* c, const double* q, const double* u, const double* a, const double* ak, int64_t n, const double* hyp, int T,
                       LmState* states, double* partials, int* flags, int* scored, double* trial_count, double* trial_err, double tol,
                       const int* cand_steps, int ncand, int* irr_count, int* irr_list, int* unscored_list, int* guard_word, const int* m9_core_flag,
-                      int m9_core_epoch, bool count_only) {
+                      int m9_core_epoch, bool count_only, LmaCompactIn* compact) {
     if (T < 1 || T > kLB) return fail(c, RSDSFM_ERR_INVALID, "hypothesis batch of the analytic pass exceeds 256");
     const LmaCand cd = lma_candidates(cand_steps, ncand, tol, count_only);
     int grid = 0;
+    int64_t chunk = 0;
     const bool prof = c->profile && c->ev_prof[0] && c->ev_prof[1];
     if (prof) RSDSFM_HIP_CHECK(c, hipEventRecord(c->ev_prof[0], c->stream));
-    int rc = lma_pass_launch(c, q, u, a, ak, n, hyp, T, cd, partials, irr_count, irr_list, &grid, prof ? c->d_clk_probe : nullptr);
+    int rc = lma_pass_launch(c, q, u, a, ak, n, hyp, T, cd, partials, irr_count, irr_list, &grid, prof ? c->d_clk_probe : nullptr, &chunk);
     if (rc != RSDSFM_OK) return rc;
+    if (compact) {
+        compact->nwg = grid;
+        compact->chunk = chunk;
+        compact->nc = cd.nc;
+        for (int j = 0; j < kLmaNC; ++j) compact->steps[j] = cd.steps[j];
+    }
     if (prof) {
         RSDSFM_HIP_CHECK(c, hipEventRecord(c->ev_prof[1], c->stream));
         c->prof_pending = true;
@@ -352,7 +367,8 @@
     }
     hipLaunchKernelGGL(ransac_lma_rows_decide_kernel, dim3(T), dim3(kLB), 0, c->stream, partials, grid, T, reinterpret_cast<const double2*>(q),
                        reinterpret_cast<const double2*>(u), a, ak, n, hyp, cd, irr_count, irr_list, states, flags, scored, trial_count, trial_err,
-                       unscored_list, guard_word, m9_core_flag, m9_core_epoch);
+                       unscored_list, guard_word, m9_core_flag, m9_core_epoch, compact ? compact->listed : nullptr, compact ? compact->listed_dc : nullptr,
+                       compact ? compact->fused_c : nullptr);
     RSDSFM_HIP_CHECK(c, hipGetLastError());
     return RSDSFM_OK;
 }
diff --git a/rs-aware-differential-sfm_amd/csrc/rsdsfm_internal.hpp b/rs-aware-differential-sfm_amd/csrc/rsdsfm_internal.hpp
--- a/rs-aware-differential-sfm_amd/csrc/rsdsfm_internal.hpp
+++ b/rs-aware-differential-sfm_amd/csrc/rsdsfm_internal.hpp
@@ -70,8 +70,20 @@
     double hyp[8];
     int32_t lma_tie;
     int32_t shared_best;
-    int32_t _pad_shared;
+    int32_t compact_word;
     int32_t lazy_pending;
+};
+constexpr int kCompactNoIterate = 1, kCompactNotFused = 2, kCompactOverflow = 4, kCompactTotal = 8, kCompactCount = 16, kCompactNotAnalytic = 32,
+              kCompactGeometry = 64;
+constexpr int kCompactPickUndecided = 256;
+constexpr int kCompactNC = 3;
+struct LmaCompactIn {
+    int* listed = nullptr;
+    int8_t* listed_dc = nullptr;
+    int* fused_c = nullptr;
+    int nwg = 0;
+    int64_t chunk = 0;
+    int nc = 0, steps[kCompactNC] = {0, 0, 0};
 };
 struct PickLazy {
     int* scored = nullptr;
@@ -157,6 +169,9 @@
     hipEvent_t ev_fork = nullptr, ev_join = nullptr, ev_seq = nullptr;
     int frame_side_flatten = 3;
     int frame_tail = 0;
+    int ransac_compaction = 0;
+    int64_t compact_runs = 0, compact_fallbacks = 0;
+    int compact_reasons = 0;
     unsigned long long* d_flat_counters = nullptr;
     int seq_lanes = 0;
     int refine_stage_mode = 0;
@@ -348,6 +363,10 @@
                         RansacBest* best, const LmState* states, int depth_mode, double tol, double* rho, uint8_t* mask,
                         int64_t* block_counts, int64_t* block_offsets, int64_t* inlier_idx, double* inliers,
                         double* out_alpha, double* out_alpha_k, RansacBest* best_host = nullptr, int* zero_words = nullptr);
+bool ransac_compact_fits(const LmaCompactIn& in);
+int ransac_compact_launch(Ctx* c, const double* q, const double* u, const double* a, const double* ak, int64_t n, RansacBest* best,
+                          const LmState* states, const double* partials, const LmaCompactIn& in, const int* irr_count, double tol,
+                          int64_t* inlier_idx, double* inliers, double* out_alpha, double* out_alpha_k, RansacBest* best_host, int* zero_words);
 int ransac_rows_doubles();
 int ransac_lm_rows_launch(Ctx* c, const double* q, const double* u, const double* a, const double* ak, int64_t n,
                           const double* hyp, int T, const LmState* states, double* partials, int round, double tol, double* rows,
@@ -367,7 +386,7 @@
 int ransac_lma_launch(Ctx* c, const double* q, const double* u, const double* a, const double* ak, int64_t n, const double* hyp, int T,
                       LmState* states, double* partials, int* flags, int* scored, double* trial_count, double* trial_err, double tol,
                       const int* cand_steps, int ncand, int* irr_count, int* irr_list, int* unscored_list, int* guard_word,
-                      const int* m9_core_flag = nullptr, int m9_core_epoch = 0, bool count_only = false);
+                      const int* m9_core_flag = nullptr, int m9_core_epoch = 0, bool count_only = false, LmaCompactIn* compact = nullptr);
 int ransac_lma_rows_doubles();
 int ransac_lma_rows_launch(Ctx* c, const double* q, const double* u, const double* a, const double* ak, int64_t n, const double* hyp, int T,
                            double* partials, double tol, const int* cand_steps, int ncand, int* irr_count, int* irr_list, double* rows);
@@ -451,6 +470,10 @@
     bool lma_tie_seen = false;
     int lma_cand[2] = {2, 1}, lma_cand_next[2] = {0, 0};
     int *d_irr_count = nullptr, *d_irr_list = nullptr;
+    double* d_lma_partials = nullptr;
+    LmaCompactIn compact;
+    bool compact_eligible = false, compact_allowed = false, compact_used = false, compact_failed = false;
+    int compact_reason = 0;
     bool restarted = false;
     bool tail_ahead = true;
     const Minimal9Direct* direct = nullptr;
```

New measurement: 1736 (median of 2 runs). No clear change (+0.4%).
